# karenyang/GCN-VAE

Measured on AMD Instinct MI355X. Metric: edges/sec R-GCN forward+backward, FB15k-237 emb=200, higher is better.
Workload: dtype f32; 1 GPU; FB15k-237-shaped synthetic full graph (BASELINE configs[1]): 14541 entities, 474 directed relation types, E=544230 directed edges on this rank (544230 in the trained graph), 2-layer R-GCN-VAE bdd num_bases=100 emb_dim=200 dropout 0.2, 0 IAF blocks, DistMult decoder on T=220000 triplets per rank, step = fwd + loss(BCE+reg+KL+MMD) + bwd + clip + Adam; edges_per_gpu=544230, trained_graph_edges=544230, nodes=14541, triplets_per_gpu=220000, n_flows=0, gemm_precision=f32, launch=hipgraph, parallelism=single GPU, optimizer=replicated clip + Adam, k1_operands=f32

## Files before the change

gcn-vae_amd/csrc/common.h:

```cpp
#pragma once
#include <hip/hip_runtime.h>
#include <stdint.h>
#include <stdio.h>

#include "../../include/gcnvae.h"

namespace gv {

constexpr int WAVE = 64;

void set_error(const char* fmt, ...);

inline int launch_status(const char* what) {
    hipError_t e = hipGetLastError();
    if (e != hipSuccess) {
        set_error("%s: %s", what, hipGetErrorString(e));
        return (int)e;
    }
    return GV_OK;
}

#define GV_REQUIRE(cond, code, ...)   \
    do {                              \
        if (!(cond)) {                \
// ... 54 lines not shown
    v += dpp_f<DPP_ROW_HALF_MIRROR>(v);
    v += dpp_f<DPP_ROW_MIRROR>(v);
    return v;
}

__device__ __forceinline__ float wave_sum(float v) {
    v = row16_sum(v);
    return (rl_bcast_f(v, 0) + rl_bcast_f(v, 16)) + (rl_bcast_f(v, 32) + rl_bcast_f(v, 48));
}

__device__ __forceinline__ float wave_max(float v) {
    v = fmaxf(v, dpp_f<DPP_QUAD_1032>(v));
    v = fmaxf(v, dpp_f<DPP_QUAD_2301>(v));
    v = fmaxf(v, dpp_f<DPP_ROW_HALF_MIRROR>(v));
    v = fmaxf(v, dpp_f<DPP_ROW_MIRROR>(v));
    return fmaxf(fmaxf(rl_bcast_f(v, 0), rl_bcast_f(v, 16)), fmaxf(rl_bcast_f(v, 32), rl_bcast_f(v, 48)));
}

template <int N>
__device__ __forceinline__ void load_vec(const float* __restrict__ p, float (&d)[N]) {
    if constexpr (N % 4 == 0) {
#pragma unroll
        for (int i = 0; i < N / 4; ++i) {
            float4 t = reinterpret_cast<const float4*>(p)[i];
            d[4 * i] = t.x; d[4 * i + 1] = t.y; d[4 * i + 2] = t.z; d[4 * i + 3] = t.w;
        }
    } else if constexpr (N % 2 == 0) {
#pragma unroll
        for (int i = 0; i < N / 2; ++i) {
            float2 t = reinterpret_cast<const float2*>(p)[i];
            d[2 * i] = t.x; d[2 * i + 1] = t.y;
        }
    } else {
#pragma unroll
        for (int i = 0; i < N; ++i) d[i] = p[i];
    }
}

template <int N>
__device__ __forceinline__ void store_vec(float* __restrict__ p, const float (&s)[N]) {
    if constexpr (N % 4 == 0) {
#pragma unroll
        for (int i = 0; i < N / 4; ++i)
            reinterpret_cast<float4*>(p)[i] = make_float4(s[4 * i], s[4 * i + 1], s[4 * i + 2], s[4 * i + 3]);
    } else if constexpr (N % 2 == 0) {
#pragma unroll
        for (int i = 0; i < N / 2; ++i) reinterpret_cast<float2*>(p)[i] = make_float2(s[2 * i], s[2 * i + 1]);
    } else {
#pragma unroll
        for (int i = 0; i < N; ++i) p[i] = s[i];
    }
}

__device__ __forceinline__ float sum_slices_16x64(const float* __restrict__ part, int ncols, int nsl, int col, float (*sm)[16]) {
    const int cl = threadIdx.x & 15, grp = threadIdx.x >> 4;
    const int per = (nsl + 63) / 64;
    const int s0 = grp * per, s1 = min(nsl, s0 + per);
    float a0 = 0.f, a1 = 0.f, a2 = 0.f, a3 = 0.f;
    if (col < ncols) {
        int s = s0;
        for (; s + 4 <= s1; s += 4) {
            const float v0 = part[(size_t)s * ncols + col], v1 = part[(size_t)(s + 1) * ncols + col];
            const float v2 = part[(size_t)(s + 2) * ncols + col], v3 = part[(size_t)(s + 3) * ncols + col];
            a0 += v0; a1 += v1; a2 += v2; a3 += v3;
        }
        for (; s < s1; ++s) a0 += part[(size_t)s * ncols + col];
    }
    sm[grp][cl] = (a0 + a1) + (a2 + a3);
    __syncthreads();
    float tot = 0.f;
    if (grp == 0) {
#pragma unroll 8
        for (int g = 0; g < 64; ++g) tot += sm[g][cl];
    }
    return tot;
}

__global__ __launch_bounds__(256) inline void k_fill_u32(unsigned* __restrict__ p, unsigned v, long long n) {
    for (long long i = (long long)blockIdx.x * 256 + threadIdx.x; i < n; i += (long long)gridDim.x * 256) p[i] = v;
}
__global__ __launch_bounds__(256) inline void k_copy_u32(unsigned* __restrict__ d, const unsigned* __restrict__ s, long long n) {
    for (long long i = (long long)blockIdx.x * 256 + threadIdx.x; i < n; i += (long long)gridDim.x * 256) d[i] = s[i];
}
inline hipError_t fill_words(void* p, unsigned word, size_t n_bytes, hipStream_t st) {
    const long long n = (long long)(n_bytes / 4);
    if (n == 0) return hipSuccess;
    const unsigned blocks = (unsigned)((n + 255) / 256 > 4096 ? 4096 : (n + 255) / 256);
    hipLaunchKernelGGL(k_fill_u32, dim3(blocks), dim3(256), 0, st, (unsigned*)p, word, n);
    return hipGetLastError();
}
inline hipError_t copy_words(void* d, const void* s, size_t n_bytes, hipStream_t st) {
    const long long n = (long long)(n_bytes / 4);
    if (n == 0) return hipSuccess;
    const unsigned blocks = (unsigned)((n + 255) / 256 > 4096 ? 4096 : (n + 255) / 256);
    hipLaunchKernelGGL(k_copy_u32, dim3(blocks), dim3(256), 0, st, (unsigned*)d, (const unsigned*)s, n);
    return hipGetLastError();
}

__device__ __forceinline__ float apply_act(float v, int act) { return act == GV_ACT_RELU ? fmaxf(v, 0.f) : v; }

__device__ __forceinline__ uint4 philox4x32_10(uint32_t k0, uint32_t k1, uint32_t c0, uint32_t c1, uint32_t c2, uint32_t c3) {
#pragma unroll
    for (int r = 0; r < 10; ++r) {
        const uint32_t hi0 = __umulhi(0xD2511F53u, c0), lo0 = 0xD2511F53u * c0;
        const uint32_t hi1 = __umulhi(0xCD9E8D57u, c2), lo1 = 0xCD9E8D57u * c2;
        const uint32_t n0 = hi1 ^ c1 ^ k0, n1 = lo1, n2 = hi0 ^ c3 ^ k1, n3 = lo0;
        c0 = n0; c1 = n1; c2 = n2; c3 = n3;
        k0 += 0x9E3779B9u; k1 += 0xBB67AE85u;
    }
    return make_uint4(c0, c1, c2, c3);
}


}
```

gcn-vae_amd/csrc/k_gemm.hip:

```cpp
#include <limits.h>
#include <stdlib.h>
#include <string.h>

#include <algorithm>
#include <type_traits>

#include "common.h"
#include "k_riders.h"
#include "k_mc.h"
#include "k_query_args.h"
#include "k_topk.h"

namespace gv {


typedef float f32x16 __attribute__((ext_vector_type(16)));

struct GemmParams {
    const float* a;
    const float* b;
    float* c;
    const float* bias;
    const float* a_mask;
    float* ws;
// ... 218 lines not shown
        k0 = k1;
    }
#pragma unroll
    for (int u = 0; u < NT; ++u) {
        const int col = n0 + wn + 32 * u + l31;
        if (col >= p.n) continue;
        const float bv = (p.bias && p.split_k == 1) ? p.bias[col] : 0.f;
#pragma unroll
        for (int t = 0; t < MT; ++t) {
            if (p.tmask && MT * NT > 1) {
                const int ti = (m0 + wm + 32 * t) >> 6, tj = (n0 + wn + 32 * u) >> 6;
                const int bit = ti * p.tmask_ld + tj;
                if (ti * 64 < p.m && !((p.tmask[bit >> 6] >> (bit & 63)) & 1ull))
#pragma unroll
                    for (int i = 0; i < 16; ++i) acc[t][u][i] = 0.f;
            }
            float old[16];
            const bool acc_old = p.accumulate && p.split_k == 1;
#pragma unroll
            for (int r = 0; r < 16; ++r) {
                const int row = m0 + wm + t * 32 + (r & 3) + 8 * (r >> 2) + 4 * lhi;
                old[r] = 0.f;
                if (acc_old && row < p.m) old[r] = p.c[(size_t)row * p.ldc + col];
            }
            float val[16];
#pragma unroll
            for (int r = 0; r < 16; ++r) {
                float v = acc[t][u][r];
                if (p.split_k == 1) {
                    v = apply_act(v + bv, p.act);
                    v = acc_old ? old[r] + v : v;
                }
                val[r] = v;
            }
#pragma unroll
            for (int r = 0; r < 16; ++r) {
                const int row = m0 + wm + t * 32 + (r & 3) + 8 * (r >> 2) + 4 * lhi;
                if (row >= p.m) continue;
                if (p.split_k > 1) p.ws[((size_t)bz * p.m + row) * p.n + col] = val[r];
                else p.c[(size_t)row * p.ldc + col] = val[r];
            }
        }
    }
}

template <bool TA, bool TB, int MT, int NT, int BK>
__global__ __launch_bounds__(256) void k_gemm_f32(const GemmParams p) {
    gemm_f32_body<TA, TB, MT, NT, BK>(p, blockIdx.x, blockIdx.y, blockIdx.z, gridDim.x, gridDim.y);
}

template <bool TA, bool TB, int MT, int NT, int BK>
__global__ __launch_bounds__(256) __attribute__((amdgpu_waves_per_eu(MT == 2 ? 5 : 7))) void k_gemm_f32_riders(const GemmParams p, const RiderSet rs, const int ntn, const int ntm,
                                                         const int n_riders, const int riders_front) {
    const int tiles = ntn * ntm;
    int b = blockIdx.x;
    if (riders_front) {
        if (b < n_riders) { rider_body(rs, b, n_riders); return; }
        b -= n_riders;
    } else if (b >= tiles) {
        rider_body(rs, b - tiles, n_riders);
        return;
    }
    const int by = b / ntn;
    gemm_f32_body<TA, TB, MT, NT, BK>(p, b - by * ntn, by, 0, ntn, ntm);
}

constexpr int SC_BM = 64, SC_BN = 64, SC_BK = 16, SC_LDA = SC_BM + 1, SC_LDB = SC_BN + 1;

__device__ __forceinline__ f32x16 score_tile(const GemmParams& p, int m0, int n0, float (&ra)[SC_BM * SC_BK / 256],
                                             float (&rb)[SC_BN * SC_BK / 256], float* As, float* Bs) {
    const int lane = threadIdx.x & 63, wid = threadIdx.x >> 6;
    const int wm = (wid >> 1) * 32, wn = (wid & 1) * 32;
    const int l31 = lane & 31, lhi = lane >> 5;
    f32x16 acc;
#pragma unroll
    for (int i = 0; i < 16; ++i) acc[i] = 0.f;
    for (int k0 = 0; k0 < p.k; k0 += SC_BK) {
        stage_a<false, SC_BM, SC_BK>(As, ra);
        stage_b<true, SC_BN, SC_BK>(Bs, rb);
        __syncthreads();
        if (k0 + SC_BK < p.k) {
            load_a<false, SC_BM, SC_BK>(p, m0, k0 + SC_BK, p.k, ra);
            load_b<true, SC_BN, SC_BK>(p, n0, k0 + SC_BK, p.k, rb);
        }
#pragma unroll
        for (int kk = 0; kk < SC_BK; kk += 2)
            acc = __builtin_amdgcn_mfma_f32_32x32x2f32(As[(kk + lhi) * SC_LDA + wm + l31], Bs[(kk + lhi) * SC_LDB + wn + l31],
                                                       acc, 0, 0, 0);
        __syncthreads();
    }
    return acc;
}

template <class LoadA>
__device__ __forceinline__ f32x16 score_tile_with(const GemmParams& p, LoadA load_a_chunk, int n0, float (&ra)[SC_BM * SC_BK / 256],
                                                  float (&rb)[SC_BN * SC_BK / 256], float* As, float* Bs) {
    const int lane = threadIdx.x & 63, wid = threadIdx.x >> 6;
    const int wm = (wid >> 1) * 32, wn = (wid & 1) * 32;
    const int l31 = lane & 31, lhi = lane >> 5;
    f32x16 acc;
#pragma unroll
    for (int i = 0; i < 16; ++i) acc[i] = 0.f;
    for (int k0 = 0; k0 < p.k; k0 += SC_BK) {
        stage_a<false, SC_BM, SC_BK>(As, ra);
        stage_b<true, SC_BN, SC_BK>(Bs, rb);
        __syncthreads();
        if (k0 + SC_BK < p.k) {
            load_a_chunk(k0 + SC_BK, ra);
            load_b<true, SC_BN, SC_BK>(p, n0, k0 + SC_BK, p.k, rb);
        }
#pragma unroll
        for (int kk = 0; kk < SC_BK; kk += 2)
            acc = __builtin_amdgcn_mfma_f32_32x32x2f32(As[(kk + lhi) * SC_LDA + wm + l31], Bs[(kk + lhi) * SC_LDB + wn + l31],
// ... 843 lines not shown
    }
}

constexpr int COLSUM_SLICES = 64;

__global__ __launch_bounds__(256) void k_colsum_part(const float* x, const float* msk, int64_t m, int n, int ld, float* part) {
    __shared__ float sm[4][64];
    const int lane = threadIdx.x & 63, w = threadIdx.x >> 6;
    const int c = blockIdx.x * 64 + lane;
    const int64_t per = (m + gridDim.y - 1) / gridDim.y;
    const int64_t r0 = blockIdx.y * per, r1 = min(m, r0 + per);
    float a0 = 0.f, a1 = 0.f, a2 = 0.f, a3 = 0.f;
    if (c < n) {
        int64_t r = r0 + w;
        if (msk) {
            for (; r + 12 < r1; r += 16) {
                const float v0 = x[r * ld + c], v1 = x[(r + 4) * ld + c], v2 = x[(r + 8) * ld + c], v3 = x[(r + 12) * ld + c];
                const float m0 = msk[r * ld + c], m1 = msk[(r + 4) * ld + c], m2 = msk[(r + 8) * ld + c], m3 = msk[(r + 12) * ld + c];
                a0 += m0 > 0.f ? v0 : 0.f; a1 += m1 > 0.f ? v1 : 0.f; a2 += m2 > 0.f ? v2 : 0.f; a3 += m3 > 0.f ? v3 : 0.f;
            }
            for (; r < r1; r += 4) a0 += msk[r * ld + c] > 0.f ? x[r * ld + c] : 0.f;
        } else {
            for (; r + 12 < r1; r += 16) {
                const float v0 = x[r * ld + c], v1 = x[(r + 4) * ld + c], v2 = x[(r + 8) * ld + c], v3 = x[(r + 12) * ld + c];
                a0 += v0; a1 += v1; a2 += v2; a3 += v3;
            }
            for (; r < r1; r += 4) a0 += x[r * ld + c];
        }
    }
    sm[w][lane] = (a0 + a1) + (a2 + a3);
    __syncthreads();
    if (w == 0 && c < n) part[(size_t)blockIdx.y * n + c] = (sm[0][lane] + sm[1][lane]) + (sm[2][lane] + sm[3][lane]);
}

__global__ __launch_bounds__(256) void k_colsum_final(const float* part, int n, int nsl, float* out, int accumulate) {
    const int c = blockIdx.x * blockDim.x + threadIdx.x;
    if (c >= n) return;
    float a0 = 0.f, a1 = 0.f, a2 = 0.f, a3 = 0.f;
    int s = 0;
    for (; s + 4 <= nsl; s += 4) {
        const float v0 = part[(size_t)s * n + c], v1 = part[(size_t)(s + 1) * n + c];
        const float v2 = part[(size_t)(s + 2) * n + c], v3 = part[(size_t)(s + 3) * n + c];
        a0 += v0; a1 += v1; a2 += v2; a3 += v3;
    }
    for (; s < nsl; ++s) a0 += part[(size_t)s * n + c];
    const float acc = (a0 + a1) + (a2 + a3);
    out[c] = accumulate ? out[c] + acc : acc;
}

__global__ __launch_bounds__(1024) void k_colsum_final_wide(const float* part, int n, int nsl, float* out, int accumulate) {
    __shared__ float sm[64][16];
    const int c = blockIdx.x * 16 + (threadIdx.x & 15);
    const float acc = sum_slices_16x64(part, n, nsl, c, sm);
    if ((threadIdx.x >> 4) == 0 && c < n) out[c] = accumulate ? out[c] + acc : acc;
}

}

using namespace gv;

static int k_chunk_for(int k, int split_k) {
    int per = (k + split_k - 1) / split_k;
    return ((per + 31) / 32) * 32;
}

extern "C" int64_t gv_gemm_workspace_bytes(int m, int n, int k, int split_k) {
    (void)k;
    return split_k > 1 ? (int64_t)split_k * m * n * (int64_t)sizeof(float) : 0;
}

static int gemm_any(bool bf16, int trans_a, int trans_b, int m, int n, int k, const float* a, int lda, const float* b,
                    int ldb, float* c, int ldc, const float* bias, int act, int accumulate, int split_k,
                    const float* a_relu_mask, void* workspace, int64_t workspace_bytes, void* stream, const int32_t* rows_dev = nullptr,
                    const uint64_t* kmask = nullptr, const uint64_t* tmask = nullptr, int tiles_wanted = 0) {
    GV_REQUIRE(m >= 0 && n >= 0 && k >= 0, GV_ERR_SHAPE, "gv_gemm_f32: negative size");
    if (m == 0 || n == 0) return GV_OK;
    GV_REQUIRE(c && (k == 0 || (a && b)), GV_ERR_NULL, "gv_gemm_f32: NULL matrix");
    GV_REQUIRE(lda >= (trans_a ? m : k) && ldb >= (trans_b ? k : n) && ldc >= n, GV_ERR_SHAPE,
               "gv_gemm_f32: leading dimension too small (lda=%d ldb=%d ldc=%d)", lda, ldb, ldc);
    GV_REQUIRE(act == GV_ACT_NONE || act == GV_ACT_RELU, GV_ERR_SHAPE, "gv_gemm_f32: unknown act %d", act);
    if (split_k < 1) split_k = 1;
    if (k == 0) split_k = 1;
    GemmParams p;
    p.a = a; p.b = b; p.c = c; p.bias = bias; p.a_mask = a_relu_mask; p.ws = (float*)workspace;
    p.m = m; p.n = n; p.k = k; p.lda = lda; p.ldb = ldb; p.ldc = ldc;
    p.act = act; p.accumulate = accumulate;
    p.k_chunk = k_chunk_for(k > 0 ? k : 1, split_k);
    split_k = k > 0 ? (k + p.k_chunk - 1) / p.k_chunk : 1;
    p.split_k = split_k;
    p.vec_a = aligned16(a) && (lda % 4 == 0) && (!a_relu_mask || aligned16(a_relu_mask));
    p.vec_b = aligned16(b) && (ldb % 4 == 0);
    p.rows_dev = bf16 ? nullptr : rows_dev;
    GV_REQUIRE(!kmask || (!bf16 && split_k == 1 && k <= 64 * 16), GV_ERR_SHAPE,
               "gv_gemm_f32_sparse: k-chunk words cover fp32 products of k <= 1024 without split-K (k=%d split_k=%d)", k, split_k);
    GV_REQUIRE(!tmask || !bf16, GV_ERR_SHAPE, "gv_gemm_f32_sparse: fp32 only");
    p.kmask = (const unsigned long long*)kmask;
    p.tmask = (const unsigned long long*)tmask;
    p.tmask_ld = (n + 63) / 64;
    GV_REQUIRE(tiles_wanted >= 0 && tiles_wanted <= ((m + 63) / 64) * ((n + 63) / 64), GV_ERR_SHAPE, "gv_gemm_f32_sparse: c_tiles_wanted=%d", tiles_wanted);
    p.tmask_wanted = (tmask && tiles_wanted > 0 && split_k > 1) ? tiles_wanted : 0;
    if (split_k > 1) {
        GV_REQUIRE(workspace, GV_ERR_NULL, "gv_gemm_f32: split_k needs a workspace");
        GV_REQUIRE(workspace_bytes >= gv_gemm_workspace_bytes(m, n, k, split_k), GV_ERR_WORKSPACE,
                   "gv_gemm_f32: workspace %lld < %lld bytes", (long long)workspace_bytes,
                   (long long)gv_gemm_workspace_bytes(m, n, k, split_k));
    }
    hipStream_t st = (hipStream_t)stream;
// ... 15 lines not shown
    }
    static const int mt_env = getenv("GV_GEMM_MT") ? atoi(getenv("GV_GEMM_MT")) : 0;
    static const int nt_env = getenv("GV_GEMM_NT") ? atoi(getenv("GV_GEMM_NT")) : 0;
    static const int bk_env = getenv("GV_GEMM_BK") ? atoi(getenv("GV_GEMM_BK")) : 0;
    const int nt = (nt_env == 2 && !kmask && !(tmask && tiles_wanted > 0 && split_k > 1)) ? 2 : 1;
    const int bn = 64 * nt;
    const long blocks128 = (long)((n + bn - 1) / bn) * ((m + 127) / 128) * split_k;
    const int mt = p.tmask_wanted ? 1 : (mt_env ? mt_env : (blocks128 >= 1024 ? 2 : 1));
    static const int sparse_bk = getenv("GV_GEMM_SPARSE_BK") ? atoi(getenv("GV_GEMM_SPARSE_BK")) : 16;
    const int bk = kmask ? (sparse_bk == 32 ? 32 : 16) : (bk_env ? (bk_env == 16 ? 16 : 32) : (trans_a ? 32 : 16));
    dim3 grid((n + bn - 1) / bn, (m + 64 * mt - 1) / (64 * mt), split_k), block(256);
    if (p.tmask_wanted) { grid.x = p.tmask_wanted; grid.y = 1; }
#define GV_GEMM_CFG(TA_, TB_, MT_, NT_, BK_) \
    if (mt == MT_ && nt == NT_ && bk == BK_) hipLaunchKernelGGL((k_gemm_f32<TA_, TB_, MT_, NT_, BK_>), grid, block, 0, st, p);
#define GV_GEMM_LAUNCH(TA_, TB_)                                                                       \
    do {                                                                                               \
        GV_GEMM_CFG(TA_, TB_, 1, 1, 16) GV_GEMM_CFG(TA_, TB_, 1, 1, 32) GV_GEMM_CFG(TA_, TB_, 1, 2, 16) \
        GV_GEMM_CFG(TA_, TB_, 1, 2, 32) GV_GEMM_CFG(TA_, TB_, 2, 1, 16) GV_GEMM_CFG(TA_, TB_, 2, 1, 32) \
        GV_GEMM_CFG(TA_, TB_, 2, 2, 16) GV_GEMM_CFG(TA_, TB_, 2, 2, 32)                                 \
    } while (0)
    if (!trans_a && !trans_b) GV_GEMM_LAUNCH(false, false);
    else if (!trans_a && trans_b) GV_GEMM_LAUNCH(false, true);
    else if (trans_a && !trans_b) GV_GEMM_LAUNCH(true, false);
    else GV_GEMM_LAUNCH(true, true);
#undef GV_GEMM_LAUNCH
#undef GV_GEMM_CFG
    int rc = launch_status("gv_gemm_f32");
    if (rc != GV_OK) return rc;
    if (split_k > 1) {
        const size_t total = (size_t)m * n;
        const int blocks = (int)min((size_t)2048, (total + 255) / 256);
        hipLaunchKernelGGL(k_gemm_splitk_reduce, dim3(blocks), dim3(256), 0, st, p);
        return launch_status("gv_gemm_f32(split-k reduce)");
    }
    return GV_OK;
}

extern "C" int gv_gemm_f32(int trans_a, int trans_b, int m, int n, int k, const float* a, int lda, const float* b,
                           int ldb, float* c, int ldc, const float* bias, int act, int accumulate, int split_k,
                           const float* a_relu_mask, void* workspace, int64_t workspace_bytes, void* stream) {
    return gemm_any(false, trans_a, trans_b, m, n, k, a, lda, b, ldb, c, ldc, bias, act, accumulate, split_k, a_relu_mask,
                    workspace, workspace_bytes, stream);
}

namespace {
struct Extent { const char* lo; const char* hi; };
inline Extent extent_of(const void* p, int64_t bytes) {
    return p && bytes > 0 ? Extent{(const char*)p, (const char*)p + bytes} : Extent{nullptr, nullptr};
}
inline bool overlaps(const Extent& a, const Extent& b) { return a.lo && b.lo && a.lo < b.hi && b.lo < a.hi; }
inline int64_t matrix_bytes(int rows, int cols, int ld) { return rows > 0 && cols > 0 ? ((int64_t)(rows - 1) * ld + cols) * 4 : 0; }
}

extern "C" int gv_gemm_f32_riders(int trans_a, int trans_b, int m, int n, int k, const float* a, int lda, const float* b, int ldb,
                                  float* c, int ldc, const float* bias, int act, int accumulate, int split_k,
                                  const float* a_relu_mask, void* workspace, int64_t workspace_bytes, const gv_riders* riders,
                                  void* stream) {
    const bool any = riders && (riders->rng_jobs > 0 || riders->pack_weight || riders->mix_z_pre);
    if (!any)
        return gemm_any(false, trans_a, trans_b, m, n, k, a, lda, b, ldb, c, ldc, bias, act, accumulate, split_k, a_relu_mask,
                        workspace, workspace_bytes, stream);
    GV_REQUIRE(split_k <= 1, GV_ERR_SHAPE, "gv_gemm_f32_riders: riders do not ride on a split-K product (split_k=%d)", split_k);
    GV_REQUIRE(!trans_a && !trans_b, GV_ERR_SHAPE, "gv_gemm_f32_riders: riders ride on A @ B only (the forward self-loop product)");
    GV_REQUIRE(m > 0 && n > 0 && k >= 0, GV_ERR_SHAPE, "gv_gemm_f32_riders: m=%d n=%d k=%d", m, n, k);
    GV_REQUIRE(c && (k == 0 || (a && b)), GV_ERR_NULL, "gv_gemm_f32_riders: NULL matrix");
    GV_REQUIRE(lda >= k && ldb >= n && ldc >= n, GV_ERR_SHAPE, "gv_gemm_f32_riders: leading dimension too small (lda=%d ldb=%d ldc=%d)",
               lda, ldb, ldc);
    GV_REQUIRE(act == GV_ACT_NONE || act == GV_ACT_RELU, GV_ERR_SHAPE, "gv_gemm_f32_riders: unknown act %d", act);
    GemmParams p;
    p.a = a; p.b = b; p.c = c; p.bias = bias; p.a_mask = a_relu_mask; p.ws = nullptr;
    p.m = m; p.n = n; p.k = k; p.lda = lda; p.ldb = ldb; p.ldc = ldc;
    p.act = act; p.accumulate = accumulate;
    p.k_chunk = k_chunk_for(k > 0 ? k : 1, 1);
    p.split_k = 1;
    p.vec_a = aligned16(a) && (lda % 4 == 0) && (!a_relu_mask || aligned16(a_relu_mask));
    p.vec_b = aligned16(b) && (ldb % 4 == 0);
    p.rows_dev = nullptr; p.kmask = nullptr; p.tmask = nullptr; p.tmask_ld = (n + 63) / 64; p.tmask_wanted = 0;
    const int ntn = (n + 63) / 64;
    const int mt = (long)ntn * ((m + 127) / 128) >= 1024 ? 2 : 1;
    const int ntm = (m + 64 * mt - 1) / (64 * mt);
    GV_REQUIRE((int64_t)ntn * ntm < (1ll << 30), GV_ERR_SHAPE, "gv_gemm_f32_riders: %d x %d tiles", ntn, ntm);

    const Extent ea = extent_of(a, matrix_bytes(m, k, lda)), eb = extent_of(b, matrix_bytes(k, n, ldb)),
                 ec = extent_of(c, matrix_bytes(m, n, ldc)), ebias = extent_of(bias, (int64_t)n * 4),
                 emask = extent_of(a_relu_mask, matrix_bytes(m, k, lda));
    auto written_ok = [&](const Extent& w) { return !(overlaps(w, ea) || overlaps(w, eb) || overlaps(w, ec) || overlaps(w, ebias) || overlaps(w, emask)); };
    auto read_ok = [&](const Extent& r) { return !overlaps(r, ec); };

    RiderSet rs;
    memset(&rs, 0, sizeof(rs));
    static const int per_thread = getenv("GV_RIDER_GROUPS") ? std::max(1, atoi(getenv("GV_RIDER_GROUPS"))) : 8;
    static const int front = getenv("GV_RIDERS_FRONT") ? atoi(getenv("GV_RIDERS_FRONT")) : 1;
    int nblk = 0;
    rs.first[0] = 0;
    if (riders->rng_jobs > 0) {
        GV_REQUIRE(riders->rng_state, GV_ERR_NULL, "gv_gemm_f32_riders: NULL rng_state");
        GV_REQUIRE(riders->rng_jobs <= GV_RNG_MAX_JOBS, GV_ERR_SHAPE, "gv_gemm_f32_riders: rng_jobs=%d (1..%d)", riders->rng_jobs,
                   GV_RNG_MAX_JOBS);
        GV_REQUIRE(read_ok(extent_of(riders->rng_state, 16)), GV_ERR_SHAPE, "gv_gemm_f32_riders: rng_state overlaps C");
        rs.rng_state = riders->rng_state;
        long long g = 0;
        for (int j = 0; j < GV_RNG_MAX_JOBS; ++j) {
            rs.rng.group0[j] = g;
            if (j >= riders->rng_jobs) continue;
            void* ptr = riders->rng_ptr[j];
            const int64_t cnt = riders->rng_count[j];
            const int kind = riders->rng_kind[j];
            const float dp = riders->rng_drop_p[j];
            GV_REQUIRE(ptr && cnt > 0 && cnt < (1ll << 34), GV_ERR_SHAPE, "gv_gemm_f32_riders: rng job %d: bad buffer/count", j);
            GV_REQUIRE(kind == GV_RNG_KEEP_MASK || kind == GV_RNG_NORMAL, GV_ERR_SHAPE, "gv_gemm_f32_riders: rng job %d: kind %d", j, kind);
            GV_REQUIRE((reinterpret_cast<uintptr_t>(ptr) & (kind == GV_RNG_NORMAL ? 15u : 3u)) == 0, GV_ERR_ALIGN,
                       "gv_gemm_f32_riders: rng job %d: buffer alignment", j);
            GV_REQUIRE(kind == GV_RNG_NORMAL || (dp >= 0.f && dp < 1.f), GV_ERR_SHAPE, "gv_gemm_f32_riders: rng job %d: p=%f", j, dp);
            GV_REQUIRE(written_ok(extent_of(ptr, cnt * (kind == GV_RNG_NORMAL ? 4 : 1))), GV_ERR_SHAPE,
                       "gv_gemm_f32_riders: rng job %d writes into an operand of the product", j);
            rs.rng.ptr[j] = ptr; rs.rng.n[j] = cnt; rs.rng.kind[j] = kind; rs.rng.stream[j] = riders->rng_stream[j];
            const double th = (double)dp * 4294967296.0;
            rs.rng.thresh[j] = th >= 4294967295.0 ? 4294967295u : (uint32_t)th;
            g += (cnt + 3) / 4;
        }
        rs.rng.group0[GV_RNG_MAX_JOBS] = g;
        for (int j = riders->rng_jobs; j <= GV_RNG_MAX_JOBS; ++j) rs.rng.group0[j] = g;
        rs.rng.n_jobs = riders->rng_jobs;
        const long long want = (g + 256ll * per_thread - 1) / (256ll * per_thread);
        nblk += (int)std::min<long long>(std::max<long long>(want, 1), 1 << 16);
    }
    rs.first[1] = nblk;
    if (riders->pack_weight) {
        const int nb = riders->pack_bases, bi = riders->pack_blk_in, bo = riders->pack_blk_out, r = riders->pack_rels;
        GV_REQUIRE(riders->packed, GV_ERR_NULL, "gv_gemm_f32_riders: NULL packed");
        GV_REQUIRE(r > 0 && nb > 0 && bi > 0 && bo > 0 && (int64_t)r * nb * bi * bo < (1ll << 31), GV_ERR_SHAPE,
                   "gv_gemm_f32_riders: pack shape R=%d nb=%d %dx%d", r, nb, bi, bo);
        GV_REQUIRE(!riders->packed_pair || !riders->pack_transpose, GV_ERR_SHAPE,
                   "gv_gemm_f32_riders: the pair is (blk_in, blk_out, transpose 0) + its backward-x layout");
        PackJob& pj = rs.pack;
        GV_REQUIRE(pack_job_plan(nb, bi, bo, riders->pack_transpose != 0, &pj.bpl, &pj.adj) &&
                       (!riders->packed_pair || pack_job_plan(nb, bo, bi, true, &pj.bpl2, &pj.adj2)),
                   GV_ERR_SHAPE, "gv_gemm_f32_riders: no lane-packed kernel for num_bases=%d blocks %dx%d trans=%d", nb, bi, bo,
                   riders->pack_transpose);
        GV_REQUIRE(aligned16(riders->pack_weight) && aligned16(riders->packed) && aligned16(riders->packed_pair), GV_ERR_ALIGN,
                   "gv_gemm_f32_riders: pack buffers need 16-B alignment");
        const int64_t wbytes = (int64_t)r * nb * bi * bo * 4;
        const Extent ew = extent_of(riders->pack_weight, wbytes), e1 = extent_of(riders->packed, wbytes),
                     e2 = extent_of(riders->packed_pair, wbytes);
        GV_REQUIRE(read_ok(ew) && written_ok(e1) && written_ok(e2) && !overlaps(ew, e1) && !overlaps(ew, e2) && !overlaps(e1, e2),
                   GV_ERR_SHAPE, "gv_gemm_f32_riders: a pack buffer overlaps an operand of the product or another pack buffer");
        pj.w = riders->pack_weight; pj.packed = riders->packed; pj.packed2 = riders->packed_pair;
        pj.num_rels = r; pj.nb = nb; pj.pq = bi * bo;
        const int total = r * nb * bi * bo / 4;
        pj.blocks = std::min(2048, (total + 255) / 256);
        nblk += pj.blocks * (riders->packed_pair ? 2 : 1);
    }
    rs.first[2] = nblk;
    if (riders->mix_z_pre) {
        const int mk = riders->mix_k, mh = riders->mix_h;
        GV_REQUIRE(riders->mix, GV_ERR_NULL, "gv_gemm_f32_riders: NULL mix");
        GV_REQUIRE(mk > 0 && mh > 0 && (int64_t)mk * mh < (1ll << 28), GV_ERR_SHAPE, "gv_gemm_f32_riders: mix k=%d h=%d", mk, mh);
        const Extent ez = extent_of(riders->mix_z_pre, (int64_t)2 * mk * mh * 4), em = extent_of(riders->mix, (int64_t)3 * mk * mh * 4);
        GV_REQUIRE(read_ok(ez) && written_ok(em) && !overlaps(ez, em), GV_ERR_SHAPE,
                   "gv_gemm_f32_riders: a mix buffer overlaps an operand of the product or z_pre");
        rs.mix.z_pre = riders->mix_z_pre; rs.mix.mix = riders->mix; rs.mix.k = mk; rs.mix.h = mh;
        nblk += (mk * mh + 255) / 256;
    }
    rs.first[3] = nblk;
    const int n_riders = front ? (nblk + 7) / 8 * 8 : nblk;
    const dim3 grid((unsigned)(ntn * ntm + n_riders)), block(256);
    hipStream_t st = (hipStream_t)stream;
    if (mt == 2) hipLaunchKernelGGL((k_gemm_f32_riders<false, false, 2, 1, 16>), grid, block, 0, st, p, rs, ntn, ntm, n_riders, front ? 1 : 0);
    else hipLaunchKernelGGL((k_gemm_f32_riders<false, false, 1, 1, 16>), grid, block, 0, st, p, rs, ntn, ntm, n_riders, front ? 1 : 0);
    return launch_status("gv_gemm_f32_riders");
}

extern "C" int gv_gemm_f32_live_rows(int trans_a, int trans_b, int m, int n, int k, const float* a, int lda, const float* b,
                                     int ldb, float* c, int ldc, const float* bias, int act, int accumulate, int split_k,
                                     const float* a_relu_mask, void* workspace, int64_t workspace_bytes, const int32_t* rows_dev,
                                     void* stream) {
    return gemm_any(false, trans_a, trans_b, m, n, k, a, lda, b, ldb, c, ldc, bias, act, accumulate, split_k, a_relu_mask,
                    workspace, workspace_bytes, stream, rows_dev);
}

extern "C" int gv_gemm_f32_sparse(int trans_a, int trans_b, int m, int n, int k, const float* a, int lda, const float* b, int ldb,
                                  float* c, int ldc, const float* bias, int act, int accumulate, int split_k, const float* a_relu_mask,
                                  void* workspace, int64_t workspace_bytes, const int32_t* rows_dev, const uint64_t* b_k_chunks,
                                  const uint64_t* c_tiles, int c_tiles_wanted, void* stream) {
    return gemm_any(false, trans_a, trans_b, m, n, k, a, lda, b, ldb, c, ldc, bias, act, accumulate, split_k, a_relu_mask,
                    workspace, workspace_bytes, stream, rows_dev, b_k_chunks, c_tiles, c_tiles_wanted);
}

extern "C" int gv_gemm_bf16(int trans_a, int trans_b, int m, int n, int k, const float* a, int lda, const float* b,
                            int ldb, float* c, int ldc, const float* bias, int act, int accumulate, int split_k,
                            const float* a_relu_mask, void* workspace, int64_t workspace_bytes, void* stream) {
    return gemm_any(true, trans_a, trans_b, m, n, k, a, lda, b, ldb, c, ldc, bias, act, accumulate, split_k, a_relu_mask,
                    workspace, workspace_bytes, stream);
}

static GemmParams score_gemm_params(const float* q, int ld_q, const float* e, int ld_e, int m, int v, int h) {
    GemmParams p;
    p.a = q; p.b = e; p.c = nullptr; p.bias = nullptr; p.a_mask = nullptr; p.ws = nullptr;
    p.m = m; p.n = v; p.k = h; p.lda = ld_q; p.ldb = ld_e; p.ldc = v;
    p.act = GV_ACT_NONE; p.accumulate = 0; p.split_k = 1; p.k_chunk = h;
    p.vec_a = aligned16(q) && (ld_q % 4 == 0);
    p.vec_b = aligned16(e) && (ld_e % 4 == 0);
    p.rows_dev = nullptr; p.kmask = nullptr; p.tmask = nullptr; p.tmask_ld = 0; p.tmask_wanted = 0;
    return p;
}

static int mc_samples_args(const char* name, const float* q, int ld_q, int64_t q_stride, const float* e, int ld_e, int64_t e_stride,
                           int n_samples, int m, int v, int h, McSamples* mc) {
    GV_REQUIRE(n_samples >= 1, GV_ERR_SHAPE, "%s: n_samples=%d", name, n_samples);
    GV_REQUIRE(ld_q >= h && ld_e >= h, GV_ERR_SHAPE, "%s: leading dimension too small", name);
    GV_REQUIRE(n_samples == 1 || (q_stride >= (int64_t)(m > 0 ? m - 1 : 0) * ld_q + h && e_stride >= (int64_t)(v - 1) * ld_e + h),
               GV_ERR_SHAPE, "%s: sample stride shorter than the rows it spans (q_stride=%lld e_stride=%lld)", name,
               (long long)q_stride, (long long)e_stride);
    mc->q_stride = n_samples > 1 ? q_stride : 0;
    mc->e_stride = n_samples > 1 ? e_stride : 0;
    mc->n_samples = n_samples;
    mc->inv_s = 1.0f / (float)n_samples;
    return GV_OK;
}

static GemmParams mc_gemm_params(const float* q, int ld_q, const float* e, int ld_e, const McSamples& mc, int m, int v, int h) {
    GemmParams p = score_gemm_params(q, ld_q, e, ld_e, m, v, h);
    p.vec_a = p.vec_a && mc.q_stride % 4 == 0;
// ... 694 lines not shown
```

gcn-vae_amd/csrc/k_loss.hip:

```cpp
#include "common.h"
#include "k_riders.h"

namespace gv {

constexpr int RED_BLOCKS = 1024;

__device__ __forceinline__ float block_sum_256(float v, float* sm ) {
    v = wave_sum(v);
    const int lane = threadIdx.x & 63, w = threadIdx.x >> 6;
    __syncthreads();
    if (lane == 0) sm[w] = v;
    __syncthreads();
    return sm[0] + sm[1] + sm[2] + sm[3];
}

__global__ __launch_bounds__(256) void k_final_sum(const float* part, int n, float scale, float* out, int accumulate) {
    __shared__ float sm[4];
    float acc = 0.f;
    for (int i = threadIdx.x; i < n; i += 256) acc += part[i];
    const float tot = block_sum_256(acc, sm);
    if (threadIdx.x == 0) *out = accumulate ? *out + scale * tot : scale * tot;
}

constexpr int LOSS_COMBINE_XSQ_MAX = 65536;
// ... 801 lines not shown
        }
    }
}

__global__ __launch_bounds__(256) void k_kl_bwd_mix_part(const float* z, const float* mix, const float* resp,
                                                         float* part, int64_t n, int h, int k) {
    __shared__ float sm[2][4][64];
    const int j = blockIdx.x, slice = blockIdx.z, nsl = gridDim.z;
    const int lane = threadIdx.x & 63, w = threadIdx.x >> 6;
    const int c = blockIdx.y * 64 + lane;
    const int64_t per = (n + nsl - 1) / nsl;
    const int64_t r0 = slice * per, r1 = min(n, r0 + per);
    const int kh = k * h;
    float gmu0 = 0.f, gmu1 = 0.f, gv0 = 0.f, gv1 = 0.f;
    const bool ok = c < h;
    const float muj = ok ? mix[j * h + c] : 0.f, i2 = ok ? mix[kh + j * h + c] : 0.f;
    if (ok) {
        int64_t r = r0 + w;
        for (; r + 4 < r1; r += 8) {
            const float ra = resp[r * k + j], rb = resp[(r + 4) * k + j];
            const float da = z[r * h + c] - muj, db = z[(r + 4) * h + c] - muj;
            gmu0 += ra * da;
            gmu1 += rb * db;
            gv0 += ra * (da * da * 2.f * i2 * i2 - i2);
            gv1 += rb * (db * db * 2.f * i2 * i2 - i2);
        }
        for (; r < r1; r += 4) {
            const float ra = resp[r * k + j];
            const float da = z[r * h + c] - muj;
            gmu0 += ra * da;
            gv0 += ra * (da * da * 2.f * i2 * i2 - i2);
        }
    }
    sm[0][w][lane] = gmu0 + gmu1;
    sm[1][w][lane] = gv0 + gv1;
    __syncthreads();
    if (w == 0 && ok) {
        const float gmu = (sm[0][0][lane] + sm[0][1][lane]) + (sm[0][2][lane] + sm[0][3][lane]);
        const float gvv = (sm[1][0][lane] + sm[1][1][lane]) + (sm[1][2][lane] + sm[1][3][lane]);
        part[((size_t)slice * 2 * k + j) * h + c] = -gmu * 2.f * i2;
        part[((size_t)slice * 2 * k + k + j) * h + c] = -gvv;
    }
}

__global__ __launch_bounds__(1024) void k_kl_bwd_mix_final(const float* part, const float* z_pre, const float* gkl,
                                                           float gscale, float* g_zpre, int accumulate, int64_t n, int h,
                                                           int k, int nsl, const int* rows_dev, float* g_bias = nullptr,
                                                           int accumulate_bias = 0) {
    __shared__ float sm[64][16];
    const int kh = k * h, total = 2 * kh + (g_bias ? 2 * h : 0);
    const int i = blockIdx.x * 16 + (threadIdx.x & 15);
    float acc = sum_slices_16x64(part, total, nsl, i, sm);
    if ((threadIdx.x >> 4) != 0 || i >= total) return;
    if (i >= 2 * kh) {
        g_bias[i - 2 * kh] = accumulate_bias ? g_bias[i - 2 * kh] + acc : acc;
        return;
    }
    const float cg = gscale * (gkl ? *gkl : 1.f) / (float)(rows_dev ? (int64_t)*rows_dev : n);
    if (i >= kh) {
        const float raw = z_pre[i];
        acc *= raw > 20.f ? 1.f : 1.f / (1.f + expf(-raw));
    }
    g_zpre[i] = accumulate ? g_zpre[i] + cg * acc : cg * acc;
}

constexpr int MMD_WAVES = 16;

template <int CPL>
__device__ __forceinline__ void mmd_load_row(const float* p, int h, int lane, float (&v)[CPL]) {
#pragma unroll
    for (int i = 0; i < CPL; ++i) v[i] = (lane + 64 * i < h) ? p[lane + 64 * i] : 0.f;
}

template <int CPL>
__device__ __forceinline__ float mmd_d2(const float (&a)[CPL], const float (&b)[CPL]) {
    float d2 = 0.f;
#pragma unroll
    for (int i = 0; i < CPL; ++i) { const float d = a[i] - b[i]; d2 = fmaf(d, d, d2); }
    return d2;
}

template <int CPL>
__global__ __launch_bounds__(64 * MMD_WAVES) void k_mmd_fwd(const float* x, const float* y, const int64_t* yidx, int sx, int sy,
                                                             int h, float* part) {
    __shared__ float sm[MMD_WAVES];
    const int lane = threadIdx.x & 63, w = threadIdx.x >> 6;
    const bool is_x = (int)blockIdx.x < sx;
    auto row_of = [&](bool from_y, int j) -> const float* {
        return from_y ? y + (size_t)(yidx ? yidx[j] : j) * h : x + (size_t)j * h;
    };
    float av[CPL];
    mmd_load_row<CPL>(row_of(!is_x, is_x ? (int)blockIdx.x : (int)blockIdx.x - sx), h, lane, av);
    const float inv = 1.f / ((float)h * (float)h);
    float tot = 0.f;
    for (int pass = 0; pass < (is_x ? 2 : 1); ++pass) {
        const bool b_is_y = pass == 0 ? !is_x : true;
        const int nb = pass == 0 ? (is_x ? sx : sy) : sy;
        const float wt = pass == 0 ? 1.f / ((float)nb * (float)nb) : -2.f / ((float)sx * (float)sy);
        for (int j = w; j < nb; j += 4 * MMD_WAVES) {
            float b0[CPL], b1[CPL], b2[CPL], b3[CPL];
            const int j1 = j + MMD_WAVES, j2 = j + 2 * MMD_WAVES, j3 = j + 3 * MMD_WAVES;
            mmd_load_row<CPL>(row_of(b_is_y, j), h, lane, b0);
            mmd_load_row<CPL>(row_of(b_is_y, min(j1, nb - 1)), h, lane, b1);
            mmd_load_row<CPL>(row_of(b_is_y, min(j2, nb - 1)), h, lane, b2);
            mmd_load_row<CPL>(row_of(b_is_y, min(j3, nb - 1)), h, lane, b3);
            const float d0 = wave_sum(mmd_d2<CPL>(av, b0)), d1 = wave_sum(mmd_d2<CPL>(av, b1));
            const float d2 = wave_sum(mmd_d2<CPL>(av, b2)), d3 = wave_sum(mmd_d2<CPL>(av, b3));
            tot += wt * expf(-d0 * inv);
            if (j1 < nb) tot += wt * expf(-d1 * inv);
            if (j2 < nb) tot += wt * expf(-d2 * inv);
            if (j3 < nb) tot += wt * expf(-d3 * inv);
        }
    }
    if (lane == 0) sm[w] = tot;
    __syncthreads();
    if (threadIdx.x == 0) {
// ... 283 lines not shown
    const float* eps;
    float* gz_pre;
    int accumulate, k;
};

__global__ __launch_bounds__(256) void k_mmd_grad_finish(const MmdFinishParams a) {
    const float gg = a.gscale * (a.gmmd ? *a.gmmd : 1.f);
    const int h = a.h;
    if ((int)blockIdx.x < a.sy) {
        const int row = blockIdx.x;
        const float* src = a.gy_u + (size_t)row * h;
        float* o = a.gy + (size_t)(a.yidx ? a.yidx[row] : row) * h;
        for (int c = threadIdx.x; c < h; c += 256) {
            const float v = gg * src[c];
            if (a.yidx) atomicAdd(o + c, v);
            else o[c] = v;
        }
        return;
    }
    const int total = a.k * h;
    const int i = ((int)blockIdx.x - a.sy) * 256 + (int)threadIdx.x;
    if (i >= total) return;
    const int j = i / h, c = i - j * h;
    const float raw = a.z_pre[(size_t)(a.k + j) * h + c];
    const float v = softplus_t(raw) + 1e-8f;
    float gm = 0.f, gs = 0.f;
    constexpr int RU = 8;
    const int last = a.sx - a.k + j;
    for (int r0 = j; r0 < a.sx; r0 += RU * a.k) {
        float gu[RU], ev[RU];
#pragma unroll
        for (int u = 0; u < RU; ++u) {
            const size_t at = (size_t)min(r0 + u * a.k, last) * h + c;
            gu[u] = a.gx_u[at];
            ev[u] = a.eps[at];
        }
#pragma unroll
        for (int u = 0; u < RU; ++u) {
            const int r = r0 + u * a.k;
            if (r < a.sx) {
                const float g = gg * gu[u];
                if (a.g_pri) a.g_pri[(size_t)r * h + c] = g;
                gm += g;
                gs += g * ev[u];
            }
        }
    }
    const float gr = gs * 0.5f / sqrtf(v) * (raw > 20.f ? 1.f : 1.f / (1.f + expf(-raw)));
    a.gz_pre[i] = a.accumulate ? a.gz_pre[i] + gm : gm;
    a.gz_pre[total + i] = a.accumulate ? a.gz_pre[total + i] + gr : gr;
}

__global__ __launch_bounds__(256) void k_prior_sample_fwd(const float* z_pre, const float* eps, float* out, int s, int k, int h) {
    const int total = s * h;
    for (int i = blockIdx.x * 256 + threadIdx.x; i < total; i += gridDim.x * 256) {
        const int r = i / h, c = i - r * h, j = r % k;
        const float v = softplus_t(z_pre[(size_t)(k + j) * h + c]) + 1e-8f;
        out[i] = z_pre[(size_t)j * h + c] + eps[i] * sqrtf(v);
    }
}

__global__ __launch_bounds__(256) void k_prior_sample_bwd(const float* z_pre, const float* eps, const float* g, float* gz_pre,
                                                          int accumulate, int s, int k, int h) {
    const int total = k * h;
    for (int i = blockIdx.x * 256 + threadIdx.x; i < total; i += gridDim.x * 256) {
        const int j = i / h, c = i - j * h;
        const float raw = z_pre[(size_t)(k + j) * h + c];
        const float v = softplus_t(raw) + 1e-8f;
        float gm = 0.f, gs = 0.f;
        for (int r = j; r < s; r += k) {
            gm += g[(size_t)r * h + c];
            gs += g[(size_t)r * h + c] * eps[(size_t)r * h + c];
        }
        const float gr = gs * 0.5f / sqrtf(v) * (raw > 20.f ? 1.f : 1.f / (1.f + expf(-raw)));
        gz_pre[i] = accumulate ? gz_pre[i] + gm : gm;
        gz_pre[total + i] = accumulate ? gz_pre[total + i] + gr : gr;
    }
}

struct DmFusedParams {
    const int4* items;
    int n_items;
    const int* rel_s;
    const int* rel_o;
    const int* rel_tid;
    const float* e;
    int ld_e;
    const float* w;
    int ld_w;
    const float* labels;
    const float* bias;
    const int* pos3;
    float* score;
    float* delta;
    float* u;
    float* partial;
    float* part;
    int h;
};

constexpr int DM_PART = RED_BLOCKS;

__device__ __forceinline__ float dm_perm_f(int src_lane, float v) {
    return __int_as_float(__builtin_amdgcn_ds_bpermute(src_lane << 2, __float_as_int(v)));
}
__device__ __forceinline__ float dm_delta(float x, float y) { return 1.f / (1.f + expf(-x)) - y; }

constexpr int DM_U = 2;

__device__ __forceinline__ void dm_fused_body(const DmFusedParams& a, const int bid, const int nblk, float* sm, int4 (*tb)[64],
                                              float (*sums)[256]) {
    constexpr int U = DM_U;
// ... 418 lines not shown

extern "C" int gv_reparam_kl_fwd_mix(const float* h2, const float* eps, const float* z_pre, float* z, float* v, float* m_out,
                                     float* resp, float* workspace, int mix_ready, int64_t n, int h, int k, void* stream) {
    GV_REQUIRE(h2 && eps && z_pre && z && v && resp && workspace, GV_ERR_NULL, "gv_reparam_kl_fwd: NULL pointer");
    GV_REQUIRE(n > 0 && h > 0 && h <= 1024 && k > 0 && k <= KL_KMAX, GV_ERR_SHAPE, "gv_reparam_kl_fwd: n=%lld h=%d k=%d", (long long)n,
               h, k);
    const size_t lds = (size_t)2 * k * h * sizeof(float);
    GV_REQUIRE(lds <= 64 * 1024, GV_ERR_SHAPE, "gv_reparam_kl_fwd: mixture table %zu B exceeds the 64 KiB LDS budget", lds);
    float* mix = workspace;
    float* part = workspace + 3 * (size_t)k * h;
    float* zsq_part = workspace + kl_zsq_offset(h, k);
    if (!mix_ready) hipLaunchKernelGGL(k_kl_mix, dim3((k * h + 255) / 256), dim3(256), 0, GV_ST, z_pre, k, h, mix);
    const int nb = kl_blocks(n);
    const float* none = nullptr;
    const int* no_rows = nullptr;
#define GV_RKL_FWD(CPL_)                                                                                                       \
    hipLaunchKernelGGL(k_kl_fwd<CPL_>, dim3(nb), dim3(256), lds, GV_ST, none, none, h, none, (const float*)mix, none, resp, part, n, h, \
                       k, no_rows, h2, eps, z, v, m_out, zsq_part)
    if (kl_fwd_v4(nb, lds, GV_ST, none, none, h, none, mix, none, resp, part, n, h, k, no_rows, h2, eps, z, v, m_out, zsq_part)) {}
    else if (h <= 64) GV_RKL_FWD(1);
    else if (h <= 128) GV_RKL_FWD(2);
    else if (h <= 256) GV_RKL_FWD(4);
    else if (h <= 512) GV_RKL_FWD(8);
    else GV_RKL_FWD(16);
#undef GV_RKL_FWD
    return launch_status("gv_reparam_kl_fwd");
}

extern "C" int gv_reparam_kl_fwd(const float* h2, const float* eps, const float* z_pre, float* z, float* v, float* m_out,
                                 float* resp, float* workspace, int64_t n, int h, int k, void* stream) {
    return gv_reparam_kl_fwd_mix(h2, eps, z_pre, z, v, m_out, resp, workspace, 0, n, h, k, stream);
}

extern "C" int gv_reparam_kl_bwd(const float* z, const float* h2, const float* v, const float* eps, const float* z_pre,
                                 const float* resp, const float* gkl, float gscale, float z_extra, const float* gz_up,
                                 float* gh2, float* g_zpre, int accumulate_zpre, float* workspace, int64_t n, int h, int k,
                                 void* stream) {
    GV_REQUIRE(z && h2 && v && eps && z_pre && resp && gh2 && g_zpre && workspace, GV_ERR_NULL, "gv_reparam_kl_bwd: NULL pointer");
    GV_REQUIRE(n > 0 && h > 0 && k > 0 && k <= KL_FUSED_KT, GV_ERR_SHAPE, "gv_reparam_kl_bwd: n=%lld h=%d k=%d (k <= %d)", (long long)n,
               h, k, KL_FUSED_KT);
    float* mix = workspace;
    float* part = workspace + 3 * (size_t)k * h + RED_BLOCKS;
    float* none = nullptr;
    const int* no_rows = nullptr;
    if (!kl_bwd_cols4(GV_ST, z, h2, 2 * h, v, mix, resp, gkl, gscale, z_extra, none, none, none, part, n, h, k, no_rows, h2, eps, gz_up,
                      gh2))
        hipLaunchKernelGGL(k_kl_bwd_fused<KL_FUSED_KT>, dim3((h + 63) / 64, KL_SLICES), dim3(256), 0, GV_ST, z, h2, 2 * h, v,
                           (const float*)mix, resp, gkl, gscale, z_extra, none, none, none, part, n, h, k, no_rows, h2, eps, gz_up, gh2);
    hipLaunchKernelGGL(k_kl_bwd_mix_final, dim3((2 * k * h + 15) / 16), dim3(1024), 0, GV_ST, (const float*)part, z_pre, gkl, gscale,
                       g_zpre, accumulate_zpre, n, h, k, KL_SLICES, no_rows);
    return launch_status("gv_reparam_kl_bwd");
}

extern "C" int gv_reparam_kl_bwd_fold(const float* z, const float* h2, const float* v, const float* eps, const float* z_pre,
                                      const float* resp, const float* gkl, float gscale, float z_extra, const float* gz_up,
                                      float* gh2, float* g_zpre, int accumulate_zpre, const uint8_t* keep, float keep_scale,
                                      float* g_bias, int accumulate_bias, float* workspace, int64_t n, int h, int k,
                                      void* stream) {
    GV_REQUIRE(z && h2 && v && eps && z_pre && resp && gh2 && g_zpre && workspace, GV_ERR_NULL,
               "gv_reparam_kl_bwd_fold: NULL pointer");
    GV_REQUIRE(n > 0 && h > 0 && k > 0 && k <= KL_FUSED_KT, GV_ERR_SHAPE, "gv_reparam_kl_bwd_fold: n=%lld h=%d k=%d (k <= %d)",
               (long long)n, h, k, KL_FUSED_KT);
    float* mix = workspace;
    float* part = workspace + 3 * (size_t)k * h + RED_BLOCKS;
    float* none = nullptr;
    const int* no_rows = nullptr;
    const int cols = (2 * k + (g_bias ? 2 : 0)) * h;
    GV_REQUIRE(kl_bwd_cols4(GV_ST, z, h2, 2 * h, v, mix, resp, gkl, gscale, z_extra, none, none, none, part, n, h, k, no_rows, h2, eps,
                            gz_up, gh2, keep, keep_scale, g_bias != nullptr),
               GV_ERR_SHAPE, "gv_reparam_kl_bwd_fold: h=%d k=%d or an unaligned operand: only the float4-column backward "
               "(h %% 4 == 0, k <= 10, 16-B rows) folds the epilogue gradient", h, k);
    hipLaunchKernelGGL(k_kl_bwd_mix_final, dim3((cols + 15) / 16), dim3(1024), 0, GV_ST, (const float*)part, z_pre, gkl, gscale,
                       g_zpre, accumulate_zpre, n, h, k, KL_SLICES, no_rows, g_bias, accumulate_bias);
    return launch_status("gv_reparam_kl_bwd_fold");
}

__global__ void k_lincomb(const float* a0, float c0, const float* a1, float c1, const float* a2, float c2, const float* a3,
                          float c3, float* out) {
    if (threadIdx.x == 0 && blockIdx.x == 0) {
        float v = 0.f;
        if (a0) v += c0 * *a0;
        if (a1) v += c1 * *a1;
        if (a2) v += c2 * *a2;
        if (a3) v += c3 * *a3;
        *out = v;
    }
}

extern "C" int gv_lincomb4(const float* a0, float c0, const float* a1, float c1, const float* a2, float c2,
                           const float* a3, float c3, float* out, void* stream) {
    GV_REQUIRE(out, GV_ERR_NULL, "gv_lincomb4: NULL output");
    hipLaunchKernelGGL(k_lincomb, dim3(1), dim3(64), 0, GV_ST, a0, c0, a1, c1, a2, c2, a3, c3, out);
    return launch_status("gv_lincomb4");
}

extern "C" int gv_mmd_fwd(const float* x, const float* y, const int64_t* y_index, int sx, int sy, int h, float* mmd,
                          float* workspace, void* stream) {
    GV_REQUIRE(x && y && workspace, GV_ERR_NULL, "gv_mmd_fwd: NULL pointer");
    GV_REQUIRE(sx > 0 && sy > 0 && h > 0 && h <= 1024 && sx + sy <= RED_BLOCKS, GV_ERR_SHAPE,
               "gv_mmd_fwd: sx=%d sy=%d h=%d (need h <= 1024, sx+sy <= %d)", sx, sy, h, RED_BLOCKS);
    static const int v2 = getenv("GV_MMD_ROWS16") ? atoi(getenv("GV_MMD_ROWS16")) : 1;
    const bool al = h % 4 == 0 && aligned16(x) && aligned16(y);
    if (v2 && al && h <= 256) hipLaunchKernelGGL(k_mmd_fwd_g<4>, dim3(sx + sy), dim3(64 * MMD_WAVES), 0, GV_ST, x, y, y_index, sx, sy, h, workspace);
    else if (v2 && al && h <= 512) hipLaunchKernelGGL(k_mmd_fwd_g<8>, dim3(sx + sy), dim3(64 * MMD_WAVES), 0, GV_ST, x, y, y_index, sx, sy, h, workspace);
    else if (h <= 256) hipLaunchKernelGGL(k_mmd_fwd<4>, dim3(sx + sy), dim3(64 * MMD_WAVES), 0, GV_ST, x, y, y_index, sx, sy, h, workspace);
    else hipLaunchKernelGGL(k_mmd_fwd<16>, dim3(sx + sy), dim3(64 * MMD_WAVES), 0, GV_ST, x, y, y_index, sx, sy, h, workspace);
    if (mmd) hipLaunchKernelGGL(k_final_sum, dim3(1), dim3(256), 0, GV_ST, workspace, sx + sy, 1.f, mmd, 0);
    return launch_status("gv_mmd_fwd");
}

extern "C" int gv_loss_combine(const float* ws_pred, int64_t t, const float* ws_reg, int64_t n_embed, int64_t n_wrel,
                               const float* ws_kl, int64_t n_nodes, int h, int k, const float* ws_mmd, int sx, int sy,
                               float reg_w, float kl_w, float mmd_w, float* scal, float* loss, const int32_t* rows_dev,
                               void* stream) {
    GV_REQUIRE(ws_pred && loss, GV_ERR_NULL, "gv_loss_combine: NULL pointer");
    GV_REQUIRE(t > 0, GV_ERR_SHAPE, "gv_loss_combine: t=%lld", (long long)t);
    const int n0 = red_blocks(t, 16);
    const int n1 = ws_reg ? sq2_blocks(n_embed, 768) + sq2_blocks(n_wrel, 255) : 0;
    const int n2 = ws_kl ? kl_blocks(n_nodes) : 0;
    const int n3 = ws_mmd ? sx + sy : 0;
    const float* kl_part = ws_kl ? ws_kl + 3 * (size_t)k * h : nullptr;
    hipLaunchKernelGGL(k_loss_combine, dim3(1), dim3(256), 0, GV_ST, ws_pred, n0, 1.f / (float)t, ws_reg, n1, 1.f, kl_part,
                       n2, ws_kl ? 1.f / (float)n_nodes : 0.f, ws_mmd, n3, 1.f, reg_w, kl_w, mmd_w, scal, loss, rows_dev,
                       (float)n_nodes);
    return launch_status("gv_loss_combine");
}

// ... 139 lines not shown
```

gcn-vae_amd/csrc/k_riders.h:

```cpp
#pragma once

#include "common.h"

namespace gv {

struct RngJobs {
    void* ptr[GV_RNG_MAX_JOBS];
    long long n[GV_RNG_MAX_JOBS];
    long long group0[GV_RNG_MAX_JOBS + 1];
    int kind[GV_RNG_MAX_JOBS];
    uint32_t thresh[GV_RNG_MAX_JOBS];
    uint32_t stream[GV_RNG_MAX_JOBS];
    int n_jobs;
};

__device__ __forceinline__ void rng_fill_body(const uint64_t* state, const RngJobs& jobs, long long bid, long long nblk) {
    const uint64_t seed = state[0], tick = state[1];
    const uint32_t k0 = (uint32_t)seed, k1 = (uint32_t)(seed >> 32), t0 = (uint32_t)tick, t1 = (uint32_t)(tick >> 32);
    const long long total = jobs.group0[jobs.n_jobs];
    for (long long gg = bid * 256 + threadIdx.x; gg < total; gg += nblk * 256) {
        int j = 0;
#pragma unroll
        for (int q = 1; q < GV_RNG_MAX_JOBS; ++q)
            if (q < jobs.n_jobs && gg >= jobs.group0[q]) j = q;
// ... 11 lines not shown
                if (left > 1) o[1] = b.y;
                if (left > 2) o[2] = b.z;
            }
        } else {
            const float s = 2.3283064365386963e-10f;
            const float r0 = sqrtf(-1.3862943611198906f * __log2f(((float)x.x + 1.f) * s));
            const float r1 = sqrtf(-1.3862943611198906f * __log2f(((float)x.z + 1.f) * s));
            const float a0 = (float)x.y * s, a1 = (float)x.w * s;
            const float s0 = __builtin_amdgcn_sinf(a0), c0 = __builtin_amdgcn_cosf(a0);
            const float s1 = __builtin_amdgcn_sinf(a1), c1 = __builtin_amdgcn_cosf(a1);
            const float4 nrm = make_float4(r0 * c0, r0 * s0, r1 * c1, r1 * s1);
            float* o = (float*)jobs.ptr[j] + e0;
            if (left >= 4) {
                *reinterpret_cast<float4*>(o) = nrm;
            } else {
                o[0] = nrm.x;
                if (left > 1) o[1] = nrm.y;
                if (left > 2) o[2] = nrm.z;
            }
        }
    }
}

__device__ __forceinline__ void pack_weight_body(const float* w, float* packed, int num_rels, int nb, int pq, int bpl, int adj,
                                                 int bid, int nblk) {
    const int L = nb / bpl, nq = bpl * pq / 4, quads = L * nq;
    const int total = num_rels * quads;
    for (int i = bid * 256 + threadIdx.x; i < total; i += nblk * 256) {
        const int r = i / quads, rem = i - r * quads;
        const int l = rem % L, jq = rem / L;
        const int f = 4 * jq, sb = f / pq, within = f - sb * pq;
        const int block = adj ? l * bpl + sb : l + sb * L;
        reinterpret_cast<float4*>(packed)[i] =
            *reinterpret_cast<const float4*>(w + (size_t)r * nb * pq + (size_t)block * pq + within);
    }
}

bool pack_job_plan(int num_bases, int blk_in, int blk_out, bool transpose_w, int* bpl, int* adj);

constexpr float LOG_SQRT_2PI = 0.9189385332046727f;

__device__ __forceinline__ float softplus_t(float x) { return x > 20.f ? x : log1pf(expf(x)); }

__device__ __forceinline__ void kl_mix_body(const float* z_pre, int k, int h, float* mix, int bid, int nblk) {
    const int total = k * h;
    for (int i = bid * 256 + threadIdx.x; i < total; i += nblk * 256) {
        const float v = softplus_t(z_pre[total + i]) + 1e-8f;
        mix[i] = z_pre[i];
        mix[total + i] = 1.f / (2.f * v);
        mix[2 * total + i] = logf(sqrtf(v)) + LOG_SQRT_2PI;
    }
}

struct PackJob {
    const float* w;
    float* packed;
    float* packed2;
    int num_rels, nb, pq, bpl, adj, bpl2, adj2;
    int blocks;
};

struct MixJob {
    const float* z_pre;
    float* mix;
    int k, h;
};

struct RiderSet {
    const uint64_t* rng_state;
    RngJobs rng;
    PackJob pack;
    MixJob mix;
    int first[4];
};

__device__ __forceinline__ void rider_body(const RiderSet& rs, int b, int n) {
    (void)n;
    if (b < rs.first[1]) {
        rng_fill_body(rs.rng_state, rs.rng, b, rs.first[1]);
    } else if (b < rs.first[2]) {
        const int i = b - rs.first[1], second = i >= rs.pack.blocks;
        const PackJob& pj = rs.pack;
        pack_weight_body(pj.w, second ? pj.packed2 : pj.packed, pj.num_rels, pj.nb, pj.pq, second ? pj.bpl2 : pj.bpl,
                         second ? pj.adj2 : pj.adj, second ? i - pj.blocks : i, pj.blocks);
    } else if (b < rs.first[3]) {
        kl_mix_body(rs.mix.z_pre, rs.mix.k, rs.mix.h, rs.mix.mix, b - rs.first[2], rs.first[3] - rs.first[2]);
    }
}

}
```

gcn-vae_amd/encoders.py:

```python
import random

import numpy as np
import torch
import torch.nn as nn
import torch.nn.functional as F

from . import ops, prob
from .flows import MADE, PermuteLayer
from .layers import RelGraphConv


class EmbeddingLayer(ops.StayOnDevice, nn.Module):
    def __init__(self, num_nodes, h_dim):
        super().__init__()
        self.embedding = nn.Embedding(num_nodes, h_dim)

    def forward(self, g, h, r, norm):
        h = ops.to_module_device(self.embedding.weight, h)
        return ops.embedding(self.embedding.weight, h.squeeze(), ops.device_rng(self.embedding.weight.device),
                             sole_consumer=True)


class DistLayer(ops.StayOnDevice, nn.Module):

# ... 19 lines not shown
            print(f"Mixture of {self.k} Gaussians.")
        self.flow_log_prob = None
        self.build_encoder()
        self.z_pre = nn.Parameter(torch.randn(1, 2 * self.k, self.h_dim) / np.sqrt(self.k * self.h_dim))
        self.pi = nn.Parameter(torch.ones(k) / k, requires_grad=False)
        self.n_flows = n_flows
        if self.n_flows > 0:
            if verbose:
                print(f"Sequence of {self.n_flows} Flow transforms.")
            self.build_iaf()
        self.eps_override = None
        self.mmd_eps_override = None
        self.mmd_index_override = None
        self.rng_stream_eps, self.rng_stream_prior = ops.new_rng_stream(), ops.new_rng_stream()
        self._prior_eps_next = None
        self.batch_mmd_prior_with_forward = False
        self.rows_dev = None
        self.fuse_kl_with_reparam = False
        self.grad_reducer = None
        self._z_pri_flowed = None
        self.row_part = None

    def build_iaf(self):
        blocks = []
        for _ in range(self.n_flows):
            blocks.append(MADE(self.h_dim, self.h_dim, self.n_flows))
            blocks.append(PermuteLayer(self.h_dim))
        self.nf = nn.Sequential(*blocks)

    def build_encoder(self):
        self.input_layer = EmbeddingLayer(self.num_nodes, self.h_dim)
        self.rconv_layer_1 = RelGraphConv(self.h_dim, self.h_dim, self.num_rels, "bdd", self.num_bases,
                                          activation=nn.ReLU(), self_loop=True, dropout=self.dropout)
        self.rconv_layer_2 = RelGraphConv(self.h_dim, self.h_dim * 2, self.num_rels, "bdd", self.num_bases,
                                          activation=None, self_loop=True, dropout=self.dropout)

    def sample_z(self, batch):
        m, v = prob.gaussian_parameters(self.z_pre.squeeze(0), dim=0)
        idx = torch.distributions.categorical.Categorical(self.pi).sample((batch,))
        x = prob.sample_gaussian(m[idx], v[idx])
        if self.n_flows > 0:
            for flow in self.nf[::-1]:
                x, _ = flow.inverse(x)
        return x

    def compute_kernel(self, x, y):
        dim = x.size(1)
        d2 = (x.unsqueeze(1) - y.unsqueeze(0)).pow(2).mean(2) / float(dim)
        return torch.exp(-d2)

    def get_kl(self, z):
        return ops.kl_to_mixture(z, self.z_mean, self.z_sigma, self.z_pre.squeeze(0), self.flow_log_prob)

    def _prior_draw(self, device, dtype):
        num_sample = 200
        rows = (num_sample // self.k) * self.k if num_sample // self.k > 1 else self.k
        if self.mmd_eps_override is not None:
            eps = self.mmd_eps_override
        elif self._prior_eps_next is not None:
            eps, self._prior_eps_next = self._prior_eps_next, None
        else:
            eps = torch.empty(rows, self.h_dim, device=device, dtype=dtype)
            ops.device_rng(device).fill([(eps, ops.RNG_NORMAL, 0.0, self.rng_stream_prior)])
        return ops.prior_sample(self.z_pre.squeeze(0), eps)

    def _prior_rows(self):
        num_sample = 200
        return (num_sample // self.k) * self.k if num_sample // self.k > 1 else self.k

    def _draw_noise(self, n, device, riders=None):
        jobs, eps = [], self.eps_override
        for layer in (self.rconv_layer_1, self.rconv_layer_2):
            if layer.wants_keep_mask():
                layer._keep_next = torch.empty(n, layer.out_feat, dtype=torch.uint8, device=device)
                jobs.append(layer.keep_job(layer._keep_next))
        if eps is None:
            eps = torch.empty(n, self.h_dim, dtype=torch.float32, device=device)
            jobs.append((eps, ops.RNG_NORMAL, 0.0, self.rng_stream_eps))
        if self.batch_mmd_prior_with_forward and self.training and self.mmd_eps_override is None:
            self._prior_eps_next = torch.empty(self._prior_rows(), self.h_dim, dtype=torch.float32, device=device)
            jobs.append((self._prior_eps_next, ops.RNG_NORMAL, 0.0, self.rng_stream_prior))
        if jobs and riders is not None:
            rng = ops.device_rng(device)
            rng.claim(jobs)
            riders.rng = (rng, jobs)
        elif jobs:
            ops.device_rng(device).fill(jobs)
        return eps

    def mmd_inputs(self, z):
        num_sample = 200
        if self._z_pri_flowed is not None:
            z_pri, self._z_pri_flowed = self._z_pri_flowed, None
        else:
            z_pri = self._prior_draw(z.device, z.dtype)
            if self.n_flows > 0:
                for flow in self.nf:
                    z_pri, _ = flow.forward(z_pri)
        if self.mmd_index_override is not None:
            pick = self.mmd_index_override
        elif self.row_part is not None and getattr(self.row_part, 'real_positions', None) is not None:
            real = self.row_part.real_positions
            pick = torch.as_tensor(real[random.sample(range(len(real)), num_sample)], device=z.device)
        else:
            pick = torch.tensor(random.sample(range(z.shape[0]), num_sample), device=z.device)
        return z_pri, pick

    def get_mmd(self, z):
        z_pri, pick = self.mmd_inputs(z)
        return ops.mmd(z_pri, ops.embedding(z, pick))

    def get_flow_log_prob(self):
        return self.flow_log_prob

    def _forward_rows(self, g, h, r, norm):
        from .distributed import AllGatherRows
        from .distributed import AllReduceSum
# ... 18 lines not shown
        self.z_own = z
        return AllGatherRows.apply(ops.pad_rows(z, part.slot_rows), part)

    def _apply_flows(self, z, want_mean=False):
        n = z.shape[0]
        ride_along = self.batch_mmd_prior_with_forward and self.training
        if ride_along:
            z = ops.cat_rows(z, self._prior_draw(z.device, z.dtype))
        log_dets, flows, i = [], list(self.nf), 0
        with ops.made.keep_row_blocks_forked(z.shape[0]):
            while i < len(flows):
                flow = flows[i]
                if isinstance(flow, MADE):
                    fold = i + 1 < len(flows) and type(flows[i + 1]) is PermuteLayer
                    z, log_det = flow.forward(z, reverse_out=fold)
                    log_dets.append(log_det)
                    i += 2 if fold else 1
                else:
                    ops.made.fork_sync()
                    z, log_det = flow.forward(z)
                    i += 1
        if ride_along:
            z, self._z_pri_flowed = ops.split_rows(z, n)
        if want_mean and 1 <= len(log_dets) <= 8:
            return z, ops.mean_rows_multi(log_dets, n=n, rows_dev=self.rows_dev)
        log_det_sum = None
        for log_det in log_dets:
            log_det_sum = log_det if log_det_sum is None else log_det_sum + log_det
        if ride_along:
            log_det_sum = ops.split_rows(log_det_sum, n)[0]
        return z, log_det_sum

    def forward(self, g, h, r, norm):
        h, r, norm = ops.to_module_device(self.z_pre, h, r, norm)
        self.node_id = h.squeeze()
        if self.row_part is not None:
            return self._forward_rows(g, h, r, norm)
        if self.n_flows > 0:
            ops.made_prepare([f.call_arguments() for f in self.nf if isinstance(f, MADE)])
        h = self.input_layer(g, h, r, norm)
        ride = ops.LIVE_ROWS is None
        box1, box2 = self._rider_boxes = (ops.RiderBox(), ops.RiderBox()) if ride else (None, None)
        eps = self._draw_noise(h.shape[0], h.device, box1)
        h = self.rconv_layer_1(g, h, r, norm, riders=box1)
        if box1 is not None and not box1.done:
            raise RuntimeError('KGVAE.forward: layer 1 dropped its RiderBox (the random draws were never launched)')
        if self.grad_reducer is not None:
            h = self.grad_reducer.milestone(h, next(self.rconv_layer_2.parameters()))
        fuse_kl = self.training and self.n_flows == 0 and self.fuse_kl_with_reparam
        kl_ws = None
        if box2 is not None and fuse_kl and ops.FUSE_REPARAM_KL:
            kl_ws = ops.KLWorkspace(self.z_pre.squeeze(0), h.shape[0])
            box2.mix = (kl_ws.z_pre, kl_ws.ws)
        h = self.rconv_layer_2(g, h, r, norm, sole_consumer=fuse_kl, riders=box2)
        if box2 is not None and not box2.done:
            raise RuntimeError('KGVAE.forward: layer 2 dropped its RiderBox (weight packing / KL mixture table never launched)')
        z, self.z_mean, self.z_sigma = ops.reparam(h, eps, self.z_pre.squeeze(0) if fuse_kl else None,
                                                   getattr(h, '_gv_epi_link', None) if fuse_kl else None, kl_ws)
        self._z_pri_flowed = None
        if self.n_flows > 0:
            z, self.flow_log_prob = self._apply_flows(z, want_mean=True)
            ops.made_prepare_finish()
            if self.flow_log_prob.dim() != 0:
                log_det_sum = self.flow_log_prob
                if self.rows_dev is None:
                    self.flow_log_prob = torch.mean(log_det_sum.view(-1, 1))
                else:
                    rows = self.rows_dev.reshape(()).to(log_det_sum.dtype)
                    live = torch.arange(log_det_sum.numel(), device=log_det_sum.device) < self.rows_dev.reshape(())
                    self.flow_log_prob = (log_det_sum.reshape(-1) * live).sum() / rows
        return z

    def posterior_samples(self, g, h, r, norm, n_samples, seed=None):
        n_samples = int(n_samples)
        if n_samples < 1:
            raise ValueError(f'posterior_samples: n_samples must be >= 1, got {n_samples}')
        if self.training:
            raise RuntimeError('posterior_samples needs eval mode (the layers\' dropout would differ between the samples\' one '
                               'shared pass and a forward): call .eval() first')
        if self.row_part is not None:
            raise NotImplementedError('posterior_samples under a destination-row partition (multi-GPU) is not supported')
        h, r, norm = ops.to_module_device(self.z_pre, h, r, norm)
        self.node_id = h.squeeze()
        dev = self.z_pre.device
        gen = torch.Generator(device=dev)
        if seed is None:
            gen.seed()
        else:
            gen.manual_seed(int(seed))
        with torch.no_grad():
            x = self.input_layer(g, h, r, norm)
            x = self.rconv_layer_1(g, x, r, norm)
            h2 = self.rconv_layer_2(g, x, r, norm)
            n = h2.shape[0]
            z = torch.empty(n_samples, n, self.h_dim, dtype=torch.float32, device=dev)
            flps = torch.empty(n_samples, dtype=torch.float32, device=dev) if self.n_flows > 0 else None
            self.flow_log_prob = None
            self._z_pri_flowed = None
            for s in range(n_samples):
                eps = torch.randn(n, self.h_dim, generator=gen, dtype=torch.float32, device=dev)
                zs, self.z_mean, self.z_sigma = ops.reparam(h2, eps)
                if self.n_flows > 0:
                    zs, flp = self._apply_flows(zs, want_mean=True)
                    if flp.dim() != 0:
                        flp = torch.mean(flp.view(-1, 1))
                    self.flow_log_prob = flp
                    flps[s] = flp
                z[s].copy_(zs)
        return z, flps


class BaseRGCN(ops.StayOnDevice, nn.Module):
# ... 50 lines not shown
```

gcn-vae_amd/lib.py:

```python
import ctypes
import os

import torch

_HERE = os.path.dirname(os.path.abspath(__file__))
LIB_PATH = os.path.join(_HERE, 'libgcnvae_hip.so')

_P, _I, _L, _F = ctypes.c_void_p, ctypes.c_int, ctypes.c_int64, ctypes.c_float

SIGNATURES = {
    'gv_version': (_I, []),
    'gv_last_error_string': (ctypes.c_char_p, []),
    'gv_index_caps': (None, [_L, _I, _I, _P, _P, _P]),
    'gv_index_workspace_bytes': (_L, [_L, _I]),
    'gv_build_csr': (_I, [_P, _L, _I, _I, _P, _P, _P, _I, _P, _I, _P, _L, _P]),
    'gv_build_csr_batch_workspace_bytes': (_L, [_P, _I]),
    'gv_build_csr_batch': (_I, [_P, _I, _P, _L, _P]),
    'gv_triplet_lists': (_I, [_P, _I, _L, _P, _P, _P, _P, _P, _P, _P, _P, _P]),
    'gv_widen2_i32': (_I, [_P, _P, _L, _P, _P, _L, _P]),
    'gv_graph_index_build': (_I, [_P, _P, _L, _I, _I, _I, _I, _P, _P, _P, _P, _I, _P, _I, _P, _P, _P, _P, _I, _P, _I, _P, _L, _P]),
    'gv_relation_index_build': (_I, [_P, _P, _P, _P, _P, _L, _I, _I, _P, _P, _P, _P, _P, _P, _P, _I, _P, _I, _P, _L, _P]),
    'gv_triplet_index_build': (_I, [_P, _L, _I, _I, _I, _I, _P, _P, _P, _P, _P, _I, _P, _I, _P, _P, _P, _P, _P, _I, _P, _I,
                                    _P, _L, _P]),
    'gv_perm_sample': (_I, [_L, _L, ctypes.c_uint64, ctypes.c_uint64, _P, _P, ctypes.c_uint32, _P, _P]),
    'gv_neighborhood_sample_workspace_bytes': (_L, [_I, _L]),
    'gv_neighborhood_sample': (_I, [_P, _P, _P, _P, _I, _L, _I, ctypes.c_uint64, ctypes.c_uint64, _P, ctypes.c_uint32, _P, _P, _L, _P]),
    'gv_relabel_workspace_bytes': (_L, [_I]),
    'gv_relabel_pairs': (_I, [_P, _P, _L, _I, _P, _I, _P, _P, _P, _P, _L, _P]),
    'gv_negative_sampling': (_I, [_P, _P, _P, _L, _I, _P, _P, _P, ctypes.c_uint64, ctypes.c_uint64, _P, ctypes.c_uint32, _P, _P, _P]),
    'gv_graph_from_triplets_workspace_bytes': (_L, [_L, _I, _I]),
    'gv_graph_from_triplets': (_I, [_P, _P, _P, _P, _L, _I, _I, _P, _P, _P, _P, _P, _L, _P]),
    'gv_segment_items_count': (_I, [_P, _I, _I, _P, _P, _P, _P]),
    'gv_segment_items_fill': (_I, [_P, _I, _I, _P, _P, _P, _P, _P, _P]),
    'gv_rgcn_bdd_aggregate': (_I, [_P, _I, _P, _I, _P, _P, _P, _P, _P, _I, _P, _I, _I, _I, _I, _I, _I,
                                   _P, _I, _I, _P, _F, _P, _I, _P, _P]),
    'gv_rgcn_bdd_phase_plan': (_I, [_I, _I, _I, _I, _I, _I, _I, _I, _I, _P]),
    'gv_rgcn_bdd_pack_weight_phase': (_I, [_P, _I, _I, _I, _I, _I, _P, _P]),
    'gv_rgcn_bdd_aggregate_phases': (_I, [_P, _P, _P, _P, _P, _I, _P, _I, _P, _I, _P, _I, _I, _I, _I, _I, _I, _I, _I, _I,
                                          _P, _I, _I, _P, _F, _P, _I, _P, _P]),
    'gv_rgcn_bdd_lds_plan': (_I, [_I, _I, _I, _I, _I, _P]),
    'gv_rgcn_bdd_pack_weight_lds': (_I, [_P, _I, _I, _I, _I, _I, _I, _P, _P]),
    'gv_rgcn_bdd_aggregate_lds': (_I, [_P, _I, _P, _P, _I, _P, _I, _P, _P, _P, _P, _P, _I, _P, _I, _I, _I, _I, _I, _P, _I, _I,
                                       _P, _F, _P, _I, _P, _I, _P]),
    'gv_rgcn_bdd_pack_supported': (_I, [_I, _I, _I, _I]),
    'gv_rgcn_bdd_pack_weight': (_I, [_P, _I, _I, _I, _I, _I, _P, _P]),
    'gv_rgcn_bdd_pack_weight_pair': (_I, [_P, _I, _I, _I, _I, _P, _P, _P]),
    'gv_rgcn_bdd_fixup': (_I, [_P, _I, _P, _I, _P, _I, _I, _P, _F, _P, _I, _P]),
    'gv_rgcn_bdd_grad_weight': (_I, [_P, _I, _P, _I, _P, _P, _P, _P, _P, _I, _P, _I, _I, _I, _I, _P, _P, _I, _P]),
    'gv_rgcn_epilogue_fwd': (_I, [_P, _P, _I, _P, _F, _P, _L, _I, _P]),
    'gv_rgcn_epilogue_bwd': (_I, [_P, _P, _I, _P, _F, _P, _L, _I, _P, _P]),
    'gv_colsum_finish': (_I, [_P, _I, _I, _P, _I, _P]),
    'gv_gemm_workspace_bytes': (_L, [_I, _I, _I, _I]),
    'gv_gemm_f32': (_I, [_I, _I, _I, _I, _I, _P, _I, _P, _I, _P, _I, _P, _I, _I, _I, _P, _P, _L, _P]),
    'gv_gemm_f32_riders': (_I, [_I, _I, _I, _I, _I, _P, _I, _P, _I, _P, _I, _P, _I, _I, _I, _P, _P, _L, _P, _P]),
    'gv_gemm_f32_live_rows': (_I, [_I, _I, _I, _I, _I, _P, _I, _P, _I, _P, _I, _P, _I, _I, _I, _P, _P, _L, _P, _P]),
    'gv_gemm_f32_sparse': (_I, [_I, _I, _I, _I, _I, _P, _I, _P, _I, _P, _I, _P, _I, _I, _I, _P, _P, _L, _P, _P, _P, _I, _P]),
    'gv_gemm_bf16': (_I, [_I, _I, _I, _I, _I, _P, _I, _P, _I, _P, _I, _P, _I, _I, _I, _P, _P, _L, _P]),
    'gv_gemm_bf16_nt_workspace_bytes': (_L, [_I, _I, _I]),
    'gv_gemm_bf16_gradw_fits': (_I, [_I, _I, _I, _I]),
    'gv_gemm_bf16_gradw_workspace_bytes': (_L, [_I, _I, _I]),
    'gv_gemm_bf16_gradw': (_I, [_P, _I, _P, _I, _I, _I, _I, _P, _I, _P, _I, _P, _L, _P]),
    'gv_gemm_bf16_gradw_tiles': (_I, [_P, _L, _P, _L, _I, _I, _I, _P, _I, _P, _I, _P, _L, _P]),
    'gv_gemm_bf16_nt': (_I, [_P, _I, _I, _P, _I, _I, _I, _I, _P, _I, _P, _I, _P, _I, _I, _P, _I, _P, _I, _I, _P, _L, _P]),
    'gv_cast_bf16': (_I, [_P, _I, _I, _I, _P, _I, _P, _I, _P]),
    'gv_rowsum_bf16_workspace_floats': (_L, [_I, _I]),
    'gv_iaf_update_fwd_bf16': (_I, [_P, _P, _I, _P, _P, _P, _P, _I, _P, _I, _L, _I, _P]),
    'gv_iaf_update_fwd_bf16_tiles': (_I, [_P, _P, _I, _P, _P, _P, _P, _I, _P, _L, _L, _I, _P]),
    'gv_iaf_update_bwd_bf16': (_I, [_P, _P, _I, _P, _P, _P, _P, _P, _I, _P, _I, _P, _L, _I, _P]),
    'gv_gather3_i32': (_I, [_P, _L, _P, _P, _P, _P, _P, _P, _P]),
    'gv_iaf_update_bwd_row0_workspace_floats': (_L, [_I]),
    'gv_iaf_update_bwd_row0': (_I, [_P, _P, _P, _P, _P, _P, _P, _P, _L, _I, _P]),
    'gv_iaf_update_bwd_bf16_ex': (_I, [_P, _P, _I, _P, _P, _P, _P, _P, _I, _P, _I, _P, _I, _L, _I, _P]),
    'gv_rowsum_bf16': (_I, [_P, _I, _I, _I, _P, _I, _P, _P]),
    'gv_rowsum_bf16_segments': (_I, [_P, _I, _I, _I, _I, _P, _P, _I, _P, _P]),
    'gv_made_pack_weight_elems': (_L, [_I, _I]),
    'gv_made_pack_weight': (_I, [_P, _I, _I, _I, _P, _P, _P]),
    'gv_made_pack_weight_multi': (_I, [_I, _P, _P, _P, _P, _P, _P, _P]),
    'gv_made_pack_weight_multi_iaf': (_I, [_I, _P, _P, _P, _P, _P, _P, _P]),
    'gv_made_pack_weight_iaf': (_I, [_P, _I, _I, _I, _P, _P]),
    'gv_made_chain_fits': (_I, [_I, _P, _P, _I]),
    'gv_made_chain': (_I, [_P, _I, _I, _I, _P, _P]),
    'gv_made_chain_iafb': (_I, [_P, _I, _I, _P, _P]),
    'gv_made_chain_fwd': (_I, [_P, _I, _I, _I, _P, _I, _P, _P]),
    'gv_made_chain_fwd_row0': (_I, [_P, _I, _I, _P, _I, _P, _P]),
    'gv_made_chain_debug_stamps': (_I, [_P]),
    'gv_made_pack_weight_f32_elems': (_L, [_I, _I]),
    'gv_made_pack_weight_f32_multi': (_I, [_I, _P, _P, _P, _P, _P, _P, _P]),
    'gv_made_chain_f32_fits': (_I, [_I, _P, _P]),
    'gv_made_chain_f32_plan': (_I, [_I, _P, _P, _P, _P, _P, _P, _P]),
    'gv_made_chain_f32': (_I, [_P, _I, _I, _I, _P, _P, _P, _P]),
    'gv_made_passes_f32': (_I, [_P, _I, _I, _I, _P, _P, _P, _P, _P]),
    'gv_made_gradw_f32_plan_words': (_L, [_I, _I]),
    'gv_made_gradw_f32_plan': (_I, [_P, _I, _I, _I, _P, _P]),
    'gv_made_gradw_f32_workspace_floats': (_L, [_I, _I, _L]),
    'gv_made_gradw_f32': (_I, [_P, _I, _P, _I, _I, _I, _L, _P, _P, _I, _P, _P, _P, _P, _I, _I, _P, _I, _P, _L, _P]),
    'gv_made_gradw_f32_multi_workspace_floats': (_L, [_I, _P]),
    'gv_made_gradw_f32_multi': (_I, [_I, _P, _P, _L, _P]),
    'gv_made_row_fwd': (_I, [_P, _I, _P, _P]),
    'gv_made_row_bwd': (_I, [_P, _I, _P, _P, _P]),
    'gv_rel_rows_gemm': (_I, [_P, _I, _P, _P, _I, _I, _I, _I, _P, _I, _P, _P]),
    'gv_rel_gradw_gemm': (_I, [_P, _I, _P, _P, _I, _P, _P, _P, _I, _I, _I, _P, _P]),
    'gv_rank_scores': (_I, [_P, _I, _P, _I, _P, _P, _P, _P, _I, _I, _I, _P]),
    'gv_rank_scores_filtered': (_I, [_P, _I, _P, _I, _P, _P, _P, _P, _P, _I, _P, _P, _P, _I, _I, _I, _P]),
    'gv_topk_scores_workspace_bytes': (_L, [_I, _I, _I]),
    'gv_topk_scores': (_I, [_P, _I, _P, _I, _P, _P, _P, _P, _I, _I, _P, _P, _P, _I, _I, _I, _P]),
    'gv_rank_scores_constrained': (_I, [_P, _I, _P, _I, _P, _P, _P, _P, _P, _I, _P, _I, _I, _P, _P, _P, _P, _P, _P, _I, _I, _I, _P]),
    'gv_topk_scores_constrained': (_I, [_P, _I, _P, _I, _P, _P, _P, _P, _I, _P, _I, _I, _P, _I, _P, _P, _P, _I, _I, _I, _P]),
# ... 173 lines not shown
```

gcn-vae_amd/ops.py:

```python
import contextlib
import ctypes as _ct
import itertools as _it
import os as _os
from dataclasses import dataclass
from typing import Optional

import numpy as np
import torch

from . import lib
from .lib import ptr

ACT_NONE, ACT_RELU = 0, 1

DIRECT_GRAD = {}
GRAD_FRESH = set()
DIRECT_EPOCH = [0]


def _stamp_direct(ctx):
    ctx._gv_direct_epoch = DIRECT_EPOCH[0]


def _verify_direct(ctx):
# ... 277 lines not shown
        out = torch.empty(n_seg, w_row, dtype=torch.float32, device=x.device)
        accumulate = False
    if coef is not None:
        coef = _chk(coef.reshape(-1), name='coef')
    partial = None
    if seg.n_fix > 0:
        partial = torch.empty(seg.n_slots, w_row, dtype=torch.float32, device=x.device)
    lib.call('gv_rgcn_bdd_grad_weight', ptr(seg.items), seg.n_items, ptr(seg.fix), seg.n_fix, ptr(src), ptr(dst),
             ptr(coef), ptr(coef_idx), ptr(x), ld_x, ptr(g), ld_g, num_bases, blk_in, blk_out, ptr(out), ptr(partial),
             1 if accumulate else 0, lib.stream(), tag=f'gradw_{blk_in}x{blk_out}_nb{num_bases}')
    return out


GEMM_PRECISION = 'f32'


def set_gemm_precision(precision):
    global GEMM_PRECISION
    if precision not in ('f32', 'bf16'):
        raise ValueError("precision must be 'f32' or 'bf16'")
    GEMM_PRECISION = precision


@contextlib.contextmanager
def gemm_precision(precision):
    old = GEMM_PRECISION
    set_gemm_precision(precision)
    try:
        yield
    finally:
        set_gemm_precision(old)


LIVE_ROWS = None


class live_rows:

    def __init__(self, rows_dev, cap):
        self.val = (rows_dev, int(cap)) if rows_dev is not None else None

    def __enter__(self):
        global LIVE_ROWS
        self.saved, LIVE_ROWS = LIVE_ROWS, self.val
        return self

    def __exit__(self, *exc):
        global LIVE_ROWS
        LIVE_ROWS = self.saved
        return False


GEMM_RIDERS = _os.environ.get('GV_GEMM_RIDERS', '1') == '1'
GEMM_RIDER_KINDS = set(_os.environ.get('GV_GEMM_RIDER_KINDS', 'rng,pack,mix').split(','))


class _Riders(_ct.Structure):
    _fields_ = [('rng_state', _ct.c_void_p), ('rng_ptr', _ct.c_void_p * 8), ('rng_count', _ct.c_int64 * 8),
                ('rng_kind', _ct.c_int32 * 8), ('rng_drop_p', _ct.c_float * 8), ('rng_stream', _ct.c_uint32 * 8),
                ('rng_jobs', _ct.c_int32), ('pack_rels', _ct.c_int32), ('pack_bases', _ct.c_int32), ('pack_blk_in', _ct.c_int32),
                ('pack_blk_out', _ct.c_int32), ('pack_transpose', _ct.c_int32), ('pack_weight', _ct.c_void_p),
                ('packed', _ct.c_void_p), ('packed_pair', _ct.c_void_p), ('mix_z_pre', _ct.c_void_p), ('mix', _ct.c_void_p),
                ('mix_k', _ct.c_int32), ('mix_h', _ct.c_int32)]


class RiderBox:
    __slots__ = ('rng', 'pack', 'mix', 'done', 'rode')

    def __init__(self):
        self.rng = self.pack = self.mix = None
        self.done = False
        self.rode = ()

    def empty(self):
        return self.rng is None and self.pack is None and self.mix is None

    def _launch_alone(self, kinds):
        if 'rng' in kinds and self.rng is not None:
            self.rng[0].launch(self.rng[1])
        if 'pack' in kinds and self.pack is not None:
            w, nb, bi, bo, trans, packed, pair = self.pack
            if pair is not None:
                lib.call('gv_rgcn_bdd_pack_weight_pair', ptr(w), w.shape[0], nb, bi, bo, ptr(packed), ptr(pair), lib.stream())
            else:
                lib.call('gv_rgcn_bdd_pack_weight', ptr(w), w.shape[0], nb, bi, bo, 1 if trans else 0, ptr(packed), lib.stream())
        if 'mix' in kinds and self.mix is not None:
            z_pre, ws = self.mix
            lib.call('gv_kl_mix', ptr(z_pre), z_pre.shape[0] // 2, z_pre.shape[1], ptr(ws), lib.stream())

    def flush(self):
        if self.done:
            raise RuntimeError('RiderBox: its jobs were already launched')
        self._launch_alone(('rng', 'pack', 'mix'))
        self.done = True

    def ride(self, gemm_args):
        if self.done:
            raise RuntimeError('RiderBox: its jobs were already launched')
        ride = {k for k in ('rng', 'pack', 'mix') if getattr(self, k) is not None and k in GEMM_RIDER_KINDS}
        if 'rng' in ride and len(self.rng[1]) > 8:
            ride.discard('rng')
        self._launch_alone({'rng', 'pack', 'mix'} - ride)
        d = _Riders()
        if 'rng' in ride:
            rng, jobs = self.rng
            d.rng_state, d.rng_jobs = rng.state.data_ptr(), len(jobs)
            for i, (t, kind, p, st) in enumerate(jobs):
                d.rng_ptr[i], d.rng_count[i], d.rng_kind[i], d.rng_drop_p[i], d.rng_stream[i] = t.data_ptr(), t.numel(), kind, float(p), st
        if 'pack' in ride:
            w, nb, bi, bo, trans, packed, pair = self.pack
            d.pack_weight, d.packed, d.packed_pair = w.data_ptr(), packed.data_ptr(), (pair.data_ptr() if pair is not None else None)
            d.pack_rels, d.pack_bases, d.pack_blk_in, d.pack_blk_out, d.pack_transpose = w.shape[0], nb, bi, bo, 1 if trans else 0
        if 'mix' in ride:
            z_pre, ws = self.mix
            d.mix_z_pre, d.mix, d.mix_k, d.mix_h = z_pre.data_ptr(), ws.data_ptr(), z_pre.shape[0] // 2, z_pre.shape[1]
        lib.call('gv_gemm_f32_riders', *gemm_args, _ct.addressof(d), lib.stream())
        self.rode = tuple(sorted(ride))
        self.done = True


def gemm(a, b, trans_a=False, trans_b=False, bias=None, act=ACT_NONE, out=None, accumulate=False, split_k=1,
         a_relu_mask=None, precision=None, b_k_chunks=None, c_tiles=None, riders=None):
    a, lda = _row_major(a, 'a')
    b, ldb = _row_major(b, 'b')
    m, k = (a.shape[1], a.shape[0]) if trans_a else a.shape
    kb, n = (b.shape[1], b.shape[0]) if trans_b else b.shape
    if k != kb:
        raise ValueError(f'gemm inner dimensions differ: {k} vs {kb}')
    if out is None:
        out = torch.empty(m, n, dtype=torch.float32, device=a.device)
        accumulate = False
    else:
        if not isinstance(out, torch.Tensor) or out.dtype != torch.float32 or out.dim() != 2:
            raise TypeError(f'out: expected a 2-D float32 tensor, got {getattr(out, "dtype", type(out).__name__)} '
                            f'{tuple(getattr(out, "shape", ()))}')
        if out.device != a.device or b.device != a.device:
            raise ValueError(f'out / b must be on the device of a ({a.device}), got {out.device} / {b.device}')
        if tuple(out.shape) != (m, n):
            raise ValueError(f'out: expected shape {(m, n)}, got {tuple(out.shape)}')
        if m * n and ((n > 1 and out.stride(1) != 1) or (m > 1 and out.stride(0) < n)):
            raise ValueError(f'out: needs unit inner stride and a leading dimension >= {n}, got strides {out.stride()}')
    if bias is not None:
        _chk(bias, name='bias')
        if bias.numel() != n or bias.device != a.device:
            raise ValueError(f'bias: expected {n} values on {a.device}, got {bias.numel()} on {bias.device}')
    ws, ws_bytes = None, 0
    if split_k > 1:
        ws_bytes = int(lib.load().gv_gemm_workspace_bytes(m, n, k, split_k))
        ws = torch.empty(ws_bytes // 4, dtype=torch.float32, device=a.device)
    if a_relu_mask is not None:
        a_relu_mask, ld_mask = _row_major(a_relu_mask, 'a_relu_mask')
        if tuple(a_relu_mask.shape) != tuple(a.shape) or ld_mask != lda:
            raise ValueError('a_relu_mask must have the shape and leading dimension of a')
    entry = 'gv_gemm_bf16' if (precision or GEMM_PRECISION) == 'bf16' else 'gv_gemm_f32'
    live = LIVE_ROWS
    if riders is not None:
        plain = (entry == 'gv_gemm_f32' and b_k_chunks is None and c_tiles is None and not trans_a and not trans_b and split_k <= 1
                 and m > 0 and n > 0 and not (live is not None and a.shape[0] == live[1] and a.device == live[0].device))
        if GEMM_RIDERS and plain and not riders.empty():
            riders.ride((0, 0, m, n, k, ptr(a), lda, ptr(b), ldb, ptr(out), out.stride(0) if m > 1 else n, ptr(bias), act,
                         1 if accumulate else 0, 1, ptr(a_relu_mask), None, 0))
            return out
        riders.flush()
    if (b_k_chunks is not None or c_tiles is not None) and entry == 'gv_gemm_f32':
        if b_k_chunks is not None and (b_k_chunks.dtype != torch.int64 or b_k_chunks.numel() < (n + 63) // 64 or k > 1024 or split_k != 1):
            raise ValueError('b_k_chunks: one int64 word per 64-column tile, k <= 1024, no split-K')
        if c_tiles is not None and (c_tiles.dtype != torch.int64 or c_tiles.numel() * 64 < ((m + 63) // 64) * ((n + 63) // 64)):
            raise ValueError('c_tiles: one bit per 64 x 64 tile of the result')
        rows = live[0] if (live is not None and a.shape[0] == live[1] and a.device == live[0].device) else None
        lib.call('gv_gemm_f32_sparse', 1 if trans_a else 0, 1 if trans_b else 0, m, n, k, ptr(a), lda, ptr(b), ldb, ptr(out),
                 out.stride(0) if m > 1 else n, ptr(bias), act, 1 if accumulate else 0, split_k, ptr(a_relu_mask), ptr(ws),
                 ws_bytes, ptr(rows), ptr(b_k_chunks), ptr(c_tiles), int(getattr(c_tiles, '_gv_wanted', 0)) if c_tiles is not None else 0,
                 lib.stream())
        return out
    if live is not None and entry == 'gv_gemm_f32' and a.shape[0] == live[1] and a.device == live[0].device:
        lib.call('gv_gemm_f32_live_rows', 1 if trans_a else 0, 1 if trans_b else 0, m, n, k, ptr(a), lda, ptr(b), ldb, ptr(out),
                 out.stride(0) if m > 1 else n, ptr(bias), act, 1 if accumulate else 0, split_k, ptr(a_relu_mask), ptr(ws),
                 ws_bytes, ptr(live[0]), lib.stream())
        return out
    lib.call(entry, 1 if trans_a else 0, 1 if trans_b else 0, m, n, k, ptr(a), lda, ptr(b), ldb, ptr(out),
             out.stride(0) if m > 1 else n, ptr(bias), act, 1 if accumulate else 0, split_k, ptr(a_relu_mask), ptr(ws),
             ws_bytes, lib.stream())
    return out


def block_words(mask, kind):
    import numpy as np
    m = (mask.detach().to('cpu').numpy() != 0)
    o, i = m.shape

    def pad(x, r, c):
        y = np.zeros((-(-x.shape[0] // r) * r, -(-x.shape[1] // c) * c), dtype=bool)
        y[:x.shape[0], :x.shape[1]] = x
        return y
    if kind in ('fwd', 'bwd'):
        mm = m if kind == 'fwd' else m.T
        if mm.shape[1] > 1024:
            return None
        y = pad(mm, 64, 16)
        blk = y.reshape(y.shape[0] // 64, 64, y.shape[1] // 16, 16).any(axis=(1, 3))
        words = np.zeros(blk.shape[0], dtype=np.uint64)
        for c in range(blk.shape[1]):
            words |= blk[:, c].astype(np.uint64) << np.uint64(c)
    elif kind == 'tiles':
        y = pad(m, 64, 64)
        blk = y.reshape(y.shape[0] // 64, 64, y.shape[1] // 64, 64).any(axis=(1, 3)).reshape(-1)
        words = np.zeros((blk.size + 63) // 64, dtype=np.uint64)
        for b in np.nonzero(blk)[0]:
            words[b >> 6] |= np.uint64(1) << np.uint64(b & 63)
    else:
        raise ValueError(kind)
    out = torch.from_numpy(words.view(np.int64).copy()).to(mask.device)
    if kind == 'tiles':
# ... 977 lines not shown

def relation_typed_plan(set_ptr, num_rels, rels, span=None):
    sizes = (set_ptr[1:] - set_ptr[:-1]).to(torch.int64)
    chosen = torch.zeros(num_rels, dtype=torch.bool, device=set_ptr.device)
    chosen[rels.to(set_ptr.device)] = True
    sizes = sizes * torch.cat([chosen, chosen])
    units = mine_typed_plan(torch.cat([sizes.new_zeros(1), torch.cumsum(sizes, 0)]), num_rels, span)
    slot_of = torch.full((num_rels,), -1, dtype=torch.int32, device=set_ptr.device)
    slot_of[rels.to(set_ptr.device)] = torch.arange(rels.numel(), dtype=torch.int32, device=set_ptr.device)
    units[:, 0] = slot_of[units[:, 0].long()]
    return units.contiguous()


def relation_topk_scores_typed(emb, w, k, set_ptr, set_ids, *, relations=None, bias=None, filt_lo=None, filt_hi=None, filt_ent=None,
                               exclude_self=True, max_results=MINE_MAX_RESULTS, span=None):
    return _relation_topk('gv_mine_scores_typed_by_relation', MINE_RELATION_TYPED_LEVELS, emb, w, k, relations,
                          (set_ptr, set_ids, span), bias, filt_lo, filt_hi, filt_ent, exclude_self, max_results)


def pick_split_k(m_out, n_out, k):
    tiles = ((m_out + 63) // 64) * ((n_out + 63) // 64)
    if tiles >= 256 or k < 2048:
        return 1
    if k >= 65536:
        return 64
    return max(1, min(64, 1024 // tiles, k // 256))


def colsum(x, out=None, accumulate=False, relu_mask=None):
    x, ld = _row_major(x, 'x')
    if relu_mask is not None:
        relu_mask, ldm = _row_major(relu_mask, 'relu_mask')
        if tuple(relu_mask.shape) != tuple(x.shape) or ldm != ld:
            raise ValueError('relu_mask must have the shape and leading dimension of x')
    m, n = x.shape
    if out is None:
        out = torch.empty(n, dtype=torch.float32, device=x.device)
        accumulate = False
    ws = torch.empty(64 * n, dtype=torch.float32, device=x.device)
    lib.call('gv_colsum', ptr(x), ptr(relu_mask), m, n, ld, ptr(out), ptr(ws), 1 if accumulate else 0, lib.stream())
    return out


def epilogue_fwd(agg, addend, act, keep, keep_scale):
    agg = _chk(agg, name='agg')
    out = torch.empty_like(agg)
    if addend is not None:
        addend = _chk(addend, name='addend')
    lib.call('gv_rgcn_epilogue_fwd', ptr(agg), ptr(addend), act, ptr(keep), float(keep_scale), ptr(out),
             agg.shape[0], agg.shape[1], lib.stream())
    return out


def epilogue_bwd(out, grad_out, act, keep, keep_scale, colsum_out=None, colsum_accumulate=False):
    grad_out = _chk(grad_out.contiguous(), name='grad_out')
    g = torch.empty_like(grad_out)
    m, n = grad_out.shape
    fused = colsum_out is not None and n % 4 == 0 and n <= 1024
    part = torch.empty(EPILOGUE_COLSUM_SLICES * n, dtype=torch.float32, device=g.device) if fused else None
    lib.call('gv_rgcn_epilogue_bwd', ptr(out), ptr(grad_out), act, ptr(keep), float(keep_scale), ptr(g), m, n, ptr(part),
             lib.stream())
    if fused:
        lib.call('gv_colsum_finish', ptr(part), n, EPILOGUE_COLSUM_SLICES, ptr(colsum_out), 1 if colsum_accumulate else 0,
                 lib.stream())
    elif colsum_out is not None:
        colsum(g, out=colsum_out, accumulate=colsum_accumulate)
    return g


def axpby(alpha, x, beta=0.0, y=None, a=None):
    x = _chk(x.contiguous(), name='x')
    if y is None:
        y = torch.empty_like(x)
        beta = 0.0
    lib.call('gv_axpby', x.numel(), ptr(a), float(alpha), ptr(x), float(beta), ptr(y), lib.stream())
    return y


def copy_into(dst, src):
    src = _chk(src.contiguous(), name='src')
    if dst.numel() != src.numel() or not dst.is_contiguous():
        raise ValueError('copy_into: same size, contiguous destination')
    lib.call('gv_axpby', src.numel(), None, 1.0, ptr(src), 0.0, ptr(dst), lib.stream())
    return dst


def copy_of(x):
    return copy_into(torch.empty_like(x, memory_format=torch.contiguous_format), x)


class _CatRows(torch.autograd.Function):

    @staticmethod
    def forward(ctx, a, b):
        out = torch.empty(a.shape[0] + b.shape[0], a.shape[1], dtype=torch.float32, device=a.device)
        copy_into(out[:a.shape[0]], a)
        copy_into(out[a.shape[0]:], b)
        ctx.na = a.shape[0]
        return out

    @staticmethod
    def backward(ctx, g):
        return g[:ctx.na], g[ctx.na:]


def cat_rows(a, b):
    return _CatRows.apply(a, b)


class _SplitRows(torch.autograd.Function):

    @staticmethod
    def forward(ctx, x, n):
        ctx.n, ctx.shape = int(n), tuple(x.shape)
        ctx.set_materialize_grads(False)
# ... 145 lines not shown
    @staticmethod
    def forward(ctx, table, tick_rng):
        ctx.set_materialize_grads(False)
        if tick_rng is not None:
            tick_rng.tick()
        ctx.direct = _direct(table)
        _stamp_direct(ctx)
        return table.detach().view(table.shape)

    @staticmethod
    def backward(ctx, g):
        if g is None:
            return None, None
        g = _chk(g.contiguous(), name='grad')
        _verify_direct(ctx)
        tgt = ctx.direct
        if tgt is None:
            return g, None
        lib.call('gv_axpby', g.numel(), None, 1.0, ptr(g), 1.0, ptr(tgt), lib.stream())
        GRAD_FRESH.discard(tgt.data_ptr())
        return None, None


_identity_ids = {}


def _ids_are_identity(table, ids):
    if ids.numel() != table.shape[0]:
        return False
    key = (ids.data_ptr(), ids._version, ids.numel())
    hit = _identity_ids.get(key)
    if hit is None:
        if len(_identity_ids) > 64:
            _identity_ids.clear()
        hit = _identity_ids[key] = (bool((ids.reshape(-1) == torch.arange(ids.numel(), device=ids.device)).all()), ids)
    return hit[0]


def embedding(table, ids, tick_rng=None, sole_consumer=False):
    identity = False
    if table.is_cuda and isinstance(ids, torch.Tensor) and ids.is_cuda and ids.dtype == torch.int64:
        if torch.cuda.is_current_stream_capturing():
            hit = _identity_ids.get((ids.data_ptr(), ids._version, ids.numel()))
            identity = bool(hit and hit[0]) and ids.numel() == table.shape[0]
        else:
            identity = _ids_are_identity(table, ids)
    if identity and sole_consumer:
        out = _EmbeddingIdentity.apply(table, tick_rng)
        out._gv_grad_target = _direct(table)
        return out
    return _Embedding.apply(table, ids, tick_rng)


def _epilogue_grad(out, grad_out, act, keep, keep_scale, want_bias, d_b):
    if not want_bias:
        return epilogue_bwd(out, grad_out, act, keep, keep_scale), None
    grad_bias = d_b if d_b is not None else torch.empty(grad_out.shape[1], dtype=torch.float32, device=grad_out.device)
    g = epilogue_bwd(out, grad_out, act, keep, keep_scale, colsum_out=grad_bias, colsum_accumulate=d_b is not None)
    return g, (None if d_b is not None else grad_bias)


def _gemm_addend(x, loop_weight, h_bias, out_feat, loop_bf=None, riders=None):
    if riders is not None and (loop_weight is None or loop_bf is not None):
        riders.flush()
        riders = None
    if loop_weight is not None and loop_bf is not None:
        return dense_bf16(x, loop_bf[0], loop_weight.shape[1], loop_weight.shape[0], bias=h_bias)
    if loop_weight is not None:
        return gemm(x, loop_weight, bias=h_bias, riders=riders)
    if h_bias is not None:
        return h_bias.unsqueeze(0).expand(x.shape[0], out_feat).contiguous()
    return None


def _row_addend(h_bias, loop_rows, n, out_feat):
    if h_bias is None:
        return loop_rows
    addend = h_bias.unsqueeze(0).expand(n, out_feat).contiguous()
    if loop_rows is not None:
        lib.call('gv_axpby', addend.numel(), None, 1.0, ptr(loop_rows), 1.0, ptr(addend), lib.stream())
    return addend


def _loop_grads(x, g, loop_weight, d_l, want_loop, want_x, loop_bf=None):
    if loop_weight is None:
        return None, None
    grad_loop = gx_loop = None
    if want_loop:
        grad_loop = gemm(x, g, trans_a=True, split_k=pick_split_k(x.shape[1], g.shape[1], x.shape[0]), out=d_l,
                         accumulate=d_l is not None)
        if d_l is not None:
            grad_loop = None
    if want_x:
        if loop_bf is not None:
            gx_loop = dense_bf16(g, loop_bf[1], loop_weight.shape[0], loop_weight.shape[1])
        else:
            gx_loop = gemm(g, loop_weight, trans_b=True)
    return grad_loop, gx_loop


def _coef_order(gidx, ridx, coef, side):
    if gidx.sync_free or coef is None:
        return coef, (gidx.by_src.perm if side == 'src' else ridx.by_rel.perm)
    return (gidx.coef_in_src_order(coef) if side == 'src' else ridx.coef_in_rel_order(coef)), None


def _relation_weight_grad(gidx, ridx, coef, x, g, nb, si, so, d_w):
    coef_r, idx_r = _coef_order(gidx, ridx, coef, 'rel')
    grad_w = bdd_grad_weight(ridx.by_rel.seg, ridx.src_by_rel, ridx.dst_by_rel, coef_r, idx_r, x, g, nb, si, so, out=d_w,
                             accumulate=d_w is not None)
    return None if d_w is not None else grad_w


def _bdd_weight_fwd(ctx, weight, nb, si, so, pk, pk_bwd, riders=None):
    ctx.w_bwd_packed = None
    ctx.w_version = weight._version
    if pk and riders is not None:
        w_fwd = torch.empty_like(weight)
        if pk_bwd:
            ctx.w_bwd_packed = torch.empty_like(weight)
        riders.pack = (weight, nb, si, so, False, w_fwd, ctx.w_bwd_packed)
        return w_fwd
    if pk and pk_bwd:
        w_fwd, ctx.w_bwd_packed = torch.empty_like(weight), torch.empty_like(weight)
        lib.call('gv_rgcn_bdd_pack_weight_pair', ptr(weight), weight.shape[0], nb, si, so, ptr(w_fwd), ptr(ctx.w_bwd_packed),
                 lib.stream())
        return w_fwd
    return pack_weight(weight, nb, si, so, False) if pk else weight


def _bdd_weight_bwd(ctx, weight, nb, so, si):
    pk = si * so >= 8 and pack_supported(nb, so, si, True)
    if ctx.w_bwd_packed is not None and weight._version == ctx.w_version:
        return ctx.w_bwd_packed, pk
    return (pack_weight(weight, nb, so, si, True) if pk else weight), pk


def _bdd_k1(ctx, side, tl, gidx, ridx, coef, feat, weight, nb, bi, bo, plain_weight, addend, act=ACT_NONE, keep=None,
            keep_scale=1.0, out=None, sharded=False):
    trans, r = side == 'src', weight.shape[0]
    if tl is not None:
        return bdd_aggregate_phases(tl, None if coef is None else tl.coef(coef), feat, pack_weight_phase(tl, weight, nb, bi, bo),
                                    r, nb, bi, bo, addend(), act, keep, keep_scale, out=out)
    seg = gidx.by_src.seg if trans else gidx.by_dst.seg
    nbr, ety = (gidx.nbr_by_src, ridx.et_by_src) if trans else (gidx.nbr_by_dst, ridx.et_by_dst)

    def coef_operands():
        return _coef_order(gidx, ridx, coef, 'src') if trans else (coef, gidx.by_dst.perm)
    lp = None if (ctx.grouped or sharded) else lds_plan(r, nb, bi, bo, bf=ctx.k1_bf if trans else None)
    if lp is not None and lds_graph(gidx, side, lp[2]):
        if not trans:
            ctx.k1_bf = bool(lp[3])
            if not torch.cuda.is_current_stream_capturing():
                lp_b = lds_plan(r, nb, bo, bi, bf=ctx.k1_bf)
                if lp_b is not None:
                    gidx.lds_order('src', lp_b[2])
        c, c_idx = coef_operands()
        return bdd_aggregate_lds(gidx.lds_order(side, lp[2]), nbr, ety, c, c_idx, feat,
                                 pack_weight_lds(weight, nb, bi, bo, trans, lp), r, nb, bi, bo, trans, addend(), act, keep,
                                 keep_scale, out=out, plan=lp)
    w, pk = plain_weight()
    if ctx.grouped:
        seg_g, nbr_g, ety_g, perm = ridx.grouped_order(gidx, side)
        coef_g = None if coef is None else ridx.grouped_coef(coef, side, perm)
        return bdd_aggregate(seg_g, nbr_g, ety_g, coef_g, None, feat, w, nb, bi, bo, trans, addend(), act, keep, keep_scale,
                             out=out, packed=pk)
    if K1_REL_RUNS and not gidx.sync_free and not sharded:
        nbr_r, et_r, _, coef_r = ridx.rel_sorted(gidx, side, coef)
        return bdd_aggregate(_k1_items(gidx, seg), nbr_r, et_r, coef_r, None, feat, w, nb, bi, bo, trans, addend(), act, keep,
                             keep_scale, out=out, packed=pk)
    c, c_idx = coef_operands()
    return bdd_aggregate(_k1_items(gidx, seg), nbr, ety, c, c_idx, feat, w, nb, bi, bo, trans, addend(), act, keep, keep_scale,
                         out=out, packed=pk)


class _RelGraphConvBdd(torch.autograd.Function):

    @staticmethod
    def forward(ctx, x, weight, h_bias, loop_weight, norm, gidx, ridx, num_bases, act, keep, keep_scale,
                reduce_hook, link_box=None, riders=None):
        x, _ = _row_major(x, 'x')
        n, in_feat = x.shape
        if riders is not None and (reduce_hook is not None or loop_weight is None):
            riders.flush()
            riders = None
        si = in_feat // num_bases
        so = weight.shape[1] // (num_bases * si)
        out_feat = num_bases * so
        coef = None if norm is None else norm.reshape(-1)
        tl = None
        if reduce_hook is None and use_phases(gidx, si, so, False, x.shape[0], in_feat):
            tl = ridx.phase_order(gidx, 'dst', num_bases, si, so)
        pk = tl is None and si * so >= 8 and pack_supported(num_bases, si, so, False)
        bwd_phases = reduce_hook is None and use_phases(gidx, so, si, True, n, out_feat)
        pk_bwd = not bwd_phases and si * so >= 8 and pack_supported(num_bases, so, si, True)
        w_fwd = _bdd_weight_fwd(ctx, weight, num_bases, si, so, pk, pk_bwd and ctx.needs_input_grad[0], riders)
        ctx.loop_bf = dense_bf16_forms(loop_weight) if (loop_weight is not None and x.shape[0] >= 4096) else None

        def addend():
            return _gemm_addend(x, loop_weight, h_bias, out_feat, ctx.loop_bf, riders)

        ctx.grouped = tl is None and reduce_hook is None and use_relation_groups(weight, gidx)
        ctx.k1_bf = False
        if reduce_hook is None:
            out = _bdd_k1(ctx, 'dst', tl, gidx, ridx, coef, x, weight, num_bases, si, so, lambda: (w_fwd, pk), addend, act, keep,
                          keep_scale)
        else:
            agg = torch.empty(n, out_feat, dtype=torch.float32, device=x.device)
            pending = []
            for r0, r1, sub in gidx.dst_chunks(DIST_FWD_CHUNKS):
                bdd_aggregate(sub, gidx.nbr_by_dst, ridx.et_by_dst, coef, gidx.by_dst.perm, x, w_fwd, num_bases, si, so,
                              packed=pk, out=agg)
                pending.append(reduce_hook(agg[r0:r1]))
            add = addend()
            for h in pending:
                h.wait()
            out = epilogue_fwd(agg, add, act, keep, keep_scale)
        ctx.save_for_backward(x, weight, loop_weight, coef, out if act == ACT_RELU else None, keep)
        ctx.meta = (gidx, ridx, num_bases, si, so, act, keep_scale, h_bias is not None, reduce_hook)
        ctx.direct = (_direct(weight), _direct(h_bias), _direct(loop_weight))
        _stamp_direct(ctx)
        tgt = getattr(x, '_gv_grad_target', None)
        ctx.x_grad_target = tgt if (tgt is not None and reduce_hook is None and tuple(tgt.shape) == tuple(x.shape)) else None
        ctx.epi_link = None
        if link_box is not None and act == ACT_NONE and reduce_hook is None:
            ctx.epi_link = link_box[0] = EpilogueLink(keep, keep_scale, h_bias is not None and ctx.needs_input_grad[2],
                                                      ctx.direct[1], out_feat)
        return out

    @staticmethod
    def backward(ctx, grad_out):
        x, weight, loop_weight, coef, out, keep = ctx.saved_tensors
        gidx, ridx, nb, si, so, act, keep_scale, has_bias, reduce_hook = ctx.meta
        _verify_direct(ctx)
        d_w, d_b, d_l = ctx.direct
        folded = ctx.epi_link.take(grad_out) if ctx.epi_link is not None else None
        if folded is not None:
            g, grad_bias = folded
        else:
            g, grad_bias = _epilogue_grad(out, grad_out, act, keep, keep_scale, has_bias and ctx.needs_input_grad[2], d_b)
        pending = None
        g_agg = g
        if reduce_hook is not None:
            g_agg = copy_of(g)
            pending = reduce_hook(g_agg)
        side_w = reduce_hook is None and d_l is not None and d_w is not None and loop_weight is not None \
            and ctx.needs_input_grad[3] and ctx.needs_input_grad[1] and rgcn_bwd_side(gidx.num_edges, max(x.shape[1], g.shape[1]))
        if side_w:
            with backward_side(True, x, g, g_agg, weight, coef, rgcn=True):
                gw_first = rgcn_side_gradw_first(gidx.num_edges, x.shape[1])
                if not gw_first:
                    _loop_grads(x, g, loop_weight, d_l, True, False)
                _relation_weight_grad(gidx, ridx, coef, x, g_agg, nb, si, so, d_w)
                if gw_first:
                    _loop_grads(x, g, loop_weight, d_l, True, False)
        grad_loop, gx_loop = _loop_grads(x, g, loop_weight, d_l, ctx.needs_input_grad[3] and not side_w, ctx.needs_input_grad[0],
                                         ctx.loop_bf)
        if pending is not None:
            pending.wait()
        grad_x = None
        if ctx.needs_input_grad[0]:
            x_tgt = x_add = ctx.x_grad_target
            if x_tgt is not None:
                if x_tgt.data_ptr() in GRAD_FRESH:
                    GRAD_FRESH.discard(x_tgt.data_ptr())
                    x_add = None
                else:
                    x_tgt = None
            tl = None
            if reduce_hook is None and use_phases(gidx, so, si, True, g_agg.shape[0], g_agg.shape[1]):
                tl = ridx.phase_order(gidx, 'src', nb, so, si)
            grad_x = _bdd_k1(ctx, 'src', tl, gidx, ridx, coef, g_agg, weight, nb, so, si,
                             lambda: _bdd_weight_bwd(ctx, weight, nb, so, si), lambda: gx_loop, out=x_tgt,
                             sharded=reduce_hook is not None)
            if x_tgt is not None:
                grad_x = None
            elif x_add is not None:
                lib.call('gv_axpby', grad_x.numel(), None, 1.0, ptr(grad_x), 1.0, ptr(x_add), lib.stream())
                grad_x = None
        grad_w = None
        if ctx.needs_input_grad[1] and not side_w:
            grad_w = _relation_weight_grad(gidx, ridx, coef, x, g_agg, nb, si, so, d_w)
        return grad_x, grad_w, grad_bias, grad_loop, None, None, None, None, None, None, None, None, None, None


K1_REL_RUNS = _os.environ.get('GV_K1_REL_RUNS', '1') == '1'
REL_GROUPS = _os.environ.get('GV_REL_GROUPS', '0')
L2_WEIGHT_BUDGET = 3 << 20


def use_relation_groups(weight, gidx):
    if REL_GROUPS == '0' or gidx.sync_free or gidx.num_edges == 0:
        return False
    return REL_GROUPS == '1' or weight.numel() * 4 > L2_WEIGHT_BUDGET


def rel_graph_conv_bdd(x, weight, h_bias, loop_weight, norm, gidx, ridx, num_bases, act=ACT_NONE, keep=None,
                       keep_scale=1.0, reduce_hook=None, sole_consumer=False, riders=None):
    if not (sole_consumer and KL_SEAM_FOLD):
        return _RelGraphConvBdd.apply(x, weight, h_bias, loop_weight, norm, gidx, ridx, num_bases, act, keep,
                                      float(keep_scale), reduce_hook, None, riders)
    box = [None]
    out = _RelGraphConvBdd.apply(x, weight, h_bias, loop_weight, norm, gidx, ridx, num_bases, act, keep, float(keep_scale),
                                 reduce_hook, box, riders)
    out._gv_epi_link = box[0]
    return out


def rel_rows_gemm(feat, rows, w3, transpose_w, tiles, n_tiles, n_edges):
    feat, ld = _row_major(feat, 'feat')
# ... 570 lines not shown


def linear(x, w, b=None, act=ACT_NONE):
    return _Linear.apply(x, w, b, act)


class _Mul(torch.autograd.Function):

    @staticmethod
    def forward(ctx, mask, w):
        ctx.save_for_backward(mask)
        ctx.direct = _direct(w)
        _stamp_direct(ctx)
        return mul(mask, w)

    @staticmethod
    def backward(ctx, g):
        (mask,) = ctx.saved_tensors
        _verify_direct(ctx)
        tgt = ctx.direct
        if tgt is not None and tgt.data_ptr() in GRAD_FRESH and tgt.is_contiguous():
            g = _chk(g.contiguous(), name='grad')
            lib.call('gv_mul', g.numel(), ptr(mask), ptr(g), ptr(tgt), lib.stream())
            GRAD_FRESH.discard(tgt.data_ptr())
            return None, None
        return None, mul(mask, g)


def masked_weight(mask, w):
    return _Mul.apply(mask, w)


class KLLink:
    __slots__ = ('resp', 'ws', 'z_pre_ptr', 'z_pre_version', 'gkl', 'gscale', 'z_extra', 'claimed')

    def __init__(self, resp, ws, z_pre):
        self.resp, self.ws = resp, ws
        self.z_pre_ptr, self.z_pre_version = z_pre.data_ptr(), z_pre._version
        self.gkl = None
        self.gscale = self.z_extra = 0.0
        self.claimed = False

    def matches(self, z_pre):
        return z_pre is not None and z_pre.data_ptr() == self.z_pre_ptr and z_pre._version == self.z_pre_version


FUSE_REPARAM_KL = _os.environ.get('GV_FUSE_REPARAM_KL', '1') == '1'
KL_SEAM_FOLD = _os.environ.get('GV_KL_SEAM_FOLD', '1') == '1'
LOSS_COMBINE_WREL_MAX = 65536
KL_BWD_COLS4_KMAX = 10


class EpilogueLink:
    __slots__ = ('keep', 'keep_scale', 'want_bias', 'bias_target', 'n_bias', '_gv_direct_epoch', 'buf', 'buf_version', 'grad_bias')

    def __init__(self, keep, keep_scale, want_bias, bias_target, n_bias):
        self.keep, self.keep_scale = keep, float(keep_scale)
        self.want_bias, self.bias_target, self.n_bias = bool(want_bias), bias_target, int(n_bias)
        _stamp_direct(self)
        self.buf = self.grad_bias = None
        self.buf_version = 0

    def record(self, buf, grad_bias):
        self.buf, self.buf_version, self.grad_bias = buf, buf._version, grad_bias

    def take(self, grad_out):
        buf, version, grad_bias = self.buf, self.buf_version, self.grad_bias
        self.buf = self.grad_bias = None
        if buf is None:
            return None
        if (grad_out is None or grad_out.data_ptr() != buf.data_ptr() or tuple(grad_out.shape) != tuple(buf.shape)
                or grad_out.dtype != buf.dtype or not grad_out.is_contiguous() or grad_out._version != version):
            raise RuntimeError('the layer-2 epilogue gradient was folded into the KL backward (ops.EpilogueLink), but the gradient '
                               'arriving at the layer is not that buffer: something else consumed the layer output as well and '
                               'its gradient was added unmasked.  Only hand an EpilogueLink to ops.reparam when it is the sole '
                               'consumer (GV_KL_SEAM_FOLD=0 turns the fold off)')
        return grad_out, grad_bias


def kl_seam_fold_ok(epi, gm, gv, h, k, tensors=()):
    if epi is None or not KL_SEAM_FOLD or gm is not None or gv is not None:
        return False
    if _os.environ.get('GV_KL_BWD_V4', '1') == '0' or h % 4 != 0 or h > 1024 or not 1 <= k <= KL_BWD_COLS4_KMAX:
        return False
    if epi.keep is not None and (epi.keep.data_ptr() % 4 != 0 or not epi.keep.is_contiguous()
                                 or tuple(epi.keep.shape)[-1] != 2 * h or epi.keep.dtype != torch.uint8):
        return False
    if epi.want_bias and epi.n_bias != 2 * h:
        return False
    return all(t is None or t.data_ptr() % 16 == 0 for t in tensors)


class _Reparam(torch.autograd.Function):

    @staticmethod
    def forward(ctx, h2, eps, z_pre, link_box, epi_link=None, kl_ws=None):
        ctx.set_materialize_grads(False)
        h2 = _chk(h2.contiguous(), name='h2')
        n, h = h2.shape[0], h2.shape[1] // 2
        eps = _chk(eps.contiguous(), name='eps')
        z = torch.empty(n, h, dtype=torch.float32, device=h2.device)
        v = torch.empty_like(z)
        m = torch.empty_like(z)
        ctx.link = None
        ctx.epi_link = epi_link if z_pre is not None else None
        if z_pre is not None:
            z_pre = _chk(z_pre.contiguous(), name='z_pre')
            k = z_pre.shape[0] // 2
            resp = torch.empty(n, k, dtype=torch.float32, device=h2.device)
            if kl_ws is not None and kl_ws.matches(z_pre, n, h, k):
                ws = kl_ws.ws
                lib.call('gv_reparam_kl_fwd_mix', ptr(h2), ptr(eps), ptr(z_pre), ptr(z), ptr(v), ptr(m), ptr(resp), ptr(ws), 1, n, h,
                         k, lib.stream())
            else:
                ws = torch.empty(kl_workspace_floats(n, h, k), dtype=torch.float32, device=h2.device)
                lib.call('gv_reparam_kl_fwd', ptr(h2), ptr(eps), ptr(z_pre), ptr(z), ptr(v), ptr(m), ptr(resp), ptr(ws), n, h, k,
                         lib.stream())
            ctx.link = link_box[0] = KLLink(resp, ws, z_pre)
            ctx.save_for_backward(h2, eps, v, z, z_pre)
        else:
            lib.call('gv_reparam_fwd', ptr(h2), ptr(eps), ptr(z), ptr(v), ptr(m), n, h, lib.stream())
            ctx.save_for_backward(h2, eps, v)
        return z, m, v

    @staticmethod
    def backward(ctx, gz, gm, gv):
        link, epi = ctx.link, ctx.epi_link
        if epi is not None:
            epi.buf = epi.grad_bias = None
        if link is not None and link.gkl is not None:
            h2, eps, v, z, z_pre = ctx.saved_tensors
            n, h = v.shape
            k = z_pre.shape[0] // 2
            gz = None if gz is None else _chk(gz.contiguous(), name='gz')
            d_zp = _direct_flat(z_pre)
            gzp = d_zp if d_zp is not None else torch.empty_like(z_pre)
            gh2 = torch.empty_like(h2)
            if kl_seam_fold_ok(epi, gm, gv, h, k, (z, h2, v, eps, link.resp, link.ws, gz, gh2)):
                g_bias = d_b = None
                if epi.want_bias:
                    d_b = epi.bias_target
                    if d_b is not None:
                        _verify_direct(epi)
                    g_bias = d_b if d_b is not None else torch.empty(2 * h, dtype=torch.float32, device=h2.device)
                lib.call('gv_reparam_kl_bwd_fold', ptr(z), ptr(h2), ptr(v), ptr(eps), ptr(z_pre), ptr(link.resp), ptr(link.gkl),
                         float(link.gscale), float(link.z_extra), ptr(gz), ptr(gh2), ptr(gzp), 1 if d_zp is not None else 0,
                         ptr(epi.keep), epi.keep_scale, ptr(g_bias), 1 if d_b is not None else 0, ptr(link.ws), n, h, k,
                         lib.stream())
                link.gkl = None
                epi.record(gh2, None if d_b is not None else g_bias)
                return gh2, None, (None if d_zp is not None else gzp), None, None, None
            lib.call('gv_reparam_kl_bwd', ptr(z), ptr(h2), ptr(v), ptr(eps), ptr(z_pre), ptr(link.resp), ptr(link.gkl),
                     float(link.gscale), float(link.z_extra), ptr(gz), ptr(gh2), ptr(gzp), 1 if d_zp is not None else 0,
                     ptr(link.ws), n, h, k, lib.stream())
            link.gkl = None
            if gm is not None or gv is not None:
                extra = torch.empty_like(h2)
                gm = None if gm is None else _chk(gm.contiguous(), name='gm')
                gv = None if gv is None else _chk(gv.contiguous(), name='gv')
                lib.call('gv_reparam_bwd', ptr(h2), ptr(eps), ptr(v), None, ptr(gm), ptr(gv), ptr(extra), n, h, lib.stream())
                gh2 += extra
            return gh2, None, (None if d_zp is not None else gzp), None, None, None
        h2, eps, v = ctx.saved_tensors[:3]
        n, h = v.shape
        gz = None if gz is None else _chk(gz.contiguous(), name='gz')
        gm = None if gm is None else _chk(gm.contiguous(), name='gm')
        gv = None if gv is None else _chk(gv.contiguous(), name='gv')
        gh2 = torch.empty_like(h2)
        lib.call('gv_reparam_bwd', ptr(h2), ptr(eps), ptr(v), ptr(gz), ptr(gm), ptr(gv), ptr(gh2), n, h, lib.stream())
        return gh2, None, None, None, None, None


def kl_workspace_floats(n, h, k):
    return int(lib.load().gv_kl_workspace_bytes(n, h, k)) // 4


class KLWorkspace:
    __slots__ = ('ws', 'z_pre', 'key')

    def __init__(self, z_pre, n):
        z_pre = _chk(z_pre.detach().contiguous(), name='z_pre')
        k, h = z_pre.shape[0] // 2, z_pre.shape[1]
        self.z_pre = z_pre
        self.ws = torch.empty(kl_workspace_floats(n, h, k), dtype=torch.float32, device=z_pre.device)
        self.key = (z_pre.data_ptr(), z_pre._version, int(n), h, k)

    def matches(self, z_pre, n, h, k):
        return (z_pre.data_ptr(), z_pre._version, int(n), h, k) == self.key


def reparam(h2, eps, z_pre=None, epi_link=None, kl_ws=None):
    if z_pre is None or not FUSE_REPARAM_KL:
        return _Reparam.apply(h2, eps, None, None, None, None)
    box = [None]
    z, m, v = _Reparam.apply(h2, eps, z_pre, box, epi_link if KL_SEAM_FOLD else None, kl_ws)
    z._gv_kl_link = box[0]
    return z, m, v


DISTMULT_FUSED = _os.environ.get('GV_DISTMULT_FUSED', '1') == '1'

# ... 343 lines not shown
        gx, gy = torch.empty_like(x), torch.empty_like(y)
        lib.call('gv_mmd_bwd', ptr(x), ptr(y), None, x.shape[0], y.shape[0], x.shape[1], ptr(g), 1.0, ptr(gx), ptr(gy),
                 lib.stream())
        return gx, gy


def mmd(x, y):
    return _MMD.apply(x, y)


MMD_FUSED = _os.environ.get('GV_MMD_FUSED', '1') == '1'


def mmd_sweep_ok(z_pri, z, h_max=256):
    h = z_pri.shape[1]
    return (MMD_FUSED and h % 4 == 0 and h <= h_max and z.shape[1] == h and z_pri.data_ptr() % 16 == 0
            and z.data_ptr() % 16 == 0)


class PriorLink:
    __slots__ = ('z_pre', 'eps', 'out_ptr', 'out_version', 'out_shape', 'claimed', 'buf', 'buf_version', 'gz')

    def __init__(self, z_pre, eps, out):
        self.z_pre, self.eps = z_pre, eps
        self.out_ptr, self.out_version, self.out_shape = out.data_ptr(), out._version, tuple(out.shape)
        self.claimed = False
        self.buf = self.gz = None
        self.buf_version = 0

    def matches(self, z_pri):
        return (z_pri is not None and z_pri.data_ptr() == self.out_ptr and z_pri._version == self.out_version
                and tuple(z_pri.shape) == self.out_shape and z_pri.is_contiguous())

    def record(self, buf, gz):
        self.buf, self.buf_version, self.gz = buf, buf._version, gz

    def take(self, grad_out):
        buf, version, gz = self.buf, self.buf_version, self.gz
        self.buf = self.gz = None
        if buf is None:
            return None
        if (grad_out is None or grad_out.data_ptr() != buf.data_ptr() or tuple(grad_out.shape) != tuple(buf.shape)
                or grad_out.dtype != buf.dtype or not grad_out.is_contiguous() or grad_out._version != version):
            raise RuntimeError('the prior sampler\'s backward was folded into the loss head\'s MMD finishing launch (ops.PriorLink), '
                               'but the gradient arriving at the sampler is not that buffer: something else consumed z_pri as well.  '
                               'Only hand a linked z_pri to ops.loss_head when the head is its sole consumer (GV_MMD_FUSED=0 turns '
                               'the fold off)')
        return (gz,)


class _PriorSample(torch.autograd.Function):

    @staticmethod
    def forward(ctx, z_pre, eps, link_box=None):
        z_pre, eps = _chk(z_pre.contiguous(), name='z_pre'), _chk(eps.contiguous(), name='eps')
        k, h = z_pre.shape[0] // 2, z_pre.shape[1]
        out = torch.empty_like(eps)
        ctx.set_materialize_grads(False)
        lib.call('gv_prior_sample_fwd', ptr(z_pre), ptr(eps), ptr(out), eps.shape[0], k, h, lib.stream())
        ctx.save_for_backward(z_pre, eps)
        ctx.link = None
        if link_box is not None and eps.shape[0] % k == 0:
            ctx.link = link_box[0] = PriorLink(z_pre, eps, out)
        return out

    @staticmethod
    def backward(ctx, g):
        z_pre, eps = ctx.saved_tensors
        link = ctx.link
        if link is not None and link.claimed:
            folded = link.take(g)
            if folded is not None:
                return folded[0], None, None
        if g is None:
            return None, None, None
        g = _chk(g.contiguous(), name='g')
        d_zp = _direct_flat(z_pre)
        gz = d_zp if d_zp is not None else torch.empty_like(z_pre)
        lib.call('gv_prior_sample_bwd', ptr(z_pre), ptr(eps), ptr(g), ptr(gz), 1 if d_zp is not None else 0, eps.shape[0],
                 z_pre.shape[0] // 2, z_pre.shape[1], lib.stream())
        return (None if d_zp is not None else gz), None, None


def prior_sample(z_pre, eps):
    if not MMD_FUSED:
        return _PriorSample.apply(z_pre, eps)
    box = [None]
    out = _PriorSample.apply(z_pre, eps, box)
    out._gv_prior_link = box[0]
    return out


class _LossHead(torch.autograd.Function):

    @staticmethod
    def forward(ctx, z, z_mean, z_sigma, w_rel, z_pre, flp, z_pri, pick, labels, tidx, reg_w, kl_w, mmd_w, score_bias,
                embed_rows=None, rows_dev=None, kl_link=None, grad_mode=True, prior_link=None):
        z, ld_z = _row_major(z, 'embed')
        if rows_dev is not None:
            rows_dev = _chk(rows_dev.reshape(-1), torch.int32, 'rows_dev')
            if kl_w <= 0 or embed_rows is not None:
                raise NotImplementedError('rows_dev needs kl_w > 0 (the padding rows are masked in the KL pass) and no embed_rows')
        w_rel, ld_w = _row_major(w_rel, 'w_relation')
        labels = _chk(labels.reshape(-1), name='labels')
        dev, (n, h), T = z.device, z.shape, tidx.T
        if labels.numel() != T:
            raise ValueError('labels / triplets length mismatch')
        f32 = dict(dtype=torch.float32, device=dev)
        ctx.set_materialize_grads(False)
        scal = torch.empty(4, **f32)
        pred, reg, kl, mmd = scal[0:1], scal[1:2], scal[2:3], scal[3:4]
        ws, ws2 = torch.empty(2048, **f32), torch.empty(1024, **f32)
        score = torch.empty(T, **f32)
        loss = torch.empty((), **f32)
        bias = flp if (score_bias and flp is not None) else None
        resp = wsk = z_post = wsm = None
        link = kl_link if (kl_link is not None and not kl_link.claimed and kl_w > 0 and flp is None and rows_dev is None
                           and embed_rows is None and kl_link.matches(z_pre) and kl_link.resp.shape[0] == n) else None
        if link is not None:
            link.claimed = True
        if kl_w > 0:
            z_mean, z_sigma = _chk(z_mean.contiguous(), name='z_mean'), _chk(z_sigma.contiguous(), name='z_sigma')
            z_pre = _chk(z_pre.contiguous(), name='z_pre')
            k = z_pre.shape[0] // 2
            if link is None:
                wsk = torch.empty(int(lib.load().gv_kl_workspace_bytes(n, h, k)) // 4, **f32)
                resp = torch.empty(n, k, **f32)
        if mmd_w > 0:
            z_pri = _chk(z_pri.contiguous(), name='z_pri')
            pick = _chk(pick.reshape(-1), torch.int64, 'pick')
            wsm = torch.empty(z_pri.shape[0] + pick.numel(), **f32)
        if ld_z != h or ld_w != h:
            raise ValueError('loss_head needs contiguous embeddings and relation table')
        dm_fused = grad_mode and (ctx.needs_input_grad[0] or ctx.needs_input_grad[3]) and distmult_fused_ok(z, ld_z, w_rel, ld_w)
        plink = prior_link if (mmd_w > 0 and dm_fused and prior_link is not None and not prior_link.claimed
                               and prior_link.matches(z_pri) and mmd_sweep_ok(z_pri, z)
                               and z_pri.shape[0] + pick.numel() <= 1024) else None
        if plink is not None:
            plink.claimed = True
        ctx.prior_link = plink
        st = lib.stream()
# ... 559 lines not shown
```

include/gcnvae.h:

```cpp
#ifndef GCNVAE_H
#define GCNVAE_H

#include <stdint.h>

#ifdef __cplusplus
extern "C" {
#endif

typedef enum {
    GV_OK = 0,
    GV_ERR_NULL = -1,
    GV_ERR_SHAPE = -2,
    GV_ERR_ALIGN = -3,
    GV_ERR_WORKSPACE = -4
} gv_status;

enum { GV_ACT_NONE = 0, GV_ACT_RELU = 1 };

int gv_version(void);
const char* gv_last_error_string(void);

int gv_segment_items_count(const int32_t* rowptr, int n_seg, int chunk, int32_t* n_chunks, int32_t* n_slots,
                           int32_t* is_split, void* stream);
int gv_segment_items_fill(const int32_t* rowptr, int n_seg, int chunk, const int32_t* item_off,
// ... 381 lines not shown
int64_t gv_transe_entity_topk_typed_workspace_bytes(int m, int n_tiles, int k, int span_tiles);
int gv_transe_entity_topk_typed(const int32_t* ents, int m, const float* en, const float* rn, int n, int num_rels, int dim, int head,
                                int p_norm, const int32_t* filt_lo, const int32_t* filt_hi, const int32_t* filt_ent, int n_filt_ent,
                                const int64_t* set_ptr, const int32_t* set_ids, const int32_t* tile_ptr, int n_tiles, int cand_base,
                                int exclude_self, int k, int span_tiles, int64_t* out_rel, int64_t* out_ent, float* out_dist,
                                void* workspace, int64_t workspace_bytes, void* stream);

int gv_transe_pair_rel(const float* en, const float* rn, int n, int num_rels, int dim, int p_norm, const int32_t* s, const int32_t* o,
                       const int32_t* target, const int32_t* filt_lo, const int32_t* filt_hi, const int32_t* filt_rel, int n_filt_rel,
                       int k, float* tgt, int32_t* count_raw, int32_t* count_filt, int64_t* out_ids, float* out_dist, int m,
                       void* stream);

int gv_transe_pair_rel_constrained(const float* en, const float* rn, int n, int num_rels, int dim, int p_norm, const int32_t* s,
                                   const int32_t* o, const int32_t* target, const int32_t* filt_lo, const int32_t* filt_hi,
                                   const int32_t* filt_rel, int n_filt_rel, const uint32_t* cand, int ld_cand, int n_sets, int k,
                                   float* tgt, int32_t* count_raw, int32_t* count_filt, int32_t* count_raw_c, int32_t* count_filt_c,
                                   int64_t* out_ids, float* out_dist, int m, void* stream);

int64_t gv_transe_mine_workspace_bytes(int n, int num_rels, int n_filt_ent);
int gv_transe_mine(const float* en, const float* rn, int n, int num_rels, int dim, int p_norm, const int32_t* filt_lo,
                   const int32_t* filt_hi, const int32_t* filt_ent, int n_filt_ent, int exclude_self, int mode, uint32_t key_min,
                   int prefix_bits, uint32_t prefix, int bin_bits, int32_t* out, int64_t capacity, uint64_t* counter, uint64_t* hist,
                   void* workspace, int64_t workspace_bytes, void* stream);

int gv_transe_mine_typed(const float* en, const float* rn, int n, int num_rels, int dim, int p_norm, const int64_t* set_ptr,
                         const int32_t* set_ids, const int32_t* units, int64_t n_units, const int32_t* filt_lo,
                         const int32_t* filt_hi, const int32_t* filt_ent, int n_filt_ent, int exclude_self, int mode,
                         uint32_t key_min, int prefix_bits, uint32_t prefix, int bin_bits, int32_t* out, int64_t capacity,
                         uint64_t* counter, uint64_t* hist, void* stream);

int64_t gv_gemm_workspace_bytes(int m, int n, int k, int split_k);
int gv_gemm_f32(int trans_a, int trans_b, int m, int n, int k, const float* a, int lda, const float* b, int ldb,
                float* c, int ldc, const float* bias, int act, int accumulate, int split_k, const float* a_relu_mask,
                void* workspace, int64_t workspace_bytes, void* stream);
typedef struct gv_riders {
    const uint64_t* rng_state;
    void* rng_ptr[8];
    int64_t rng_count[8];
    int32_t rng_kind[8];
    float rng_drop_p[8];
    uint32_t rng_stream[8];
    int32_t rng_jobs;
    int32_t pack_rels, pack_bases, pack_blk_in, pack_blk_out, pack_transpose;
    const float* pack_weight;
    float* packed;
    float* packed_pair;
    const float* mix_z_pre;
    float* mix;
    int32_t mix_k, mix_h;
} gv_riders;
int gv_gemm_f32_riders(int trans_a, int trans_b, int m, int n, int k, const float* a, int lda, const float* b, int ldb, float* c,
                       int ldc, const float* bias, int act, int accumulate, int split_k, const float* a_relu_mask, void* workspace,
                       int64_t workspace_bytes, const gv_riders* riders, void* stream);
int gv_gemm_f32_live_rows(int trans_a, int trans_b, int m, int n, int k, const float* a, int lda, const float* b, int ldb, float* c,
                          int ldc, const float* bias, int act, int accumulate, int split_k, const float* a_relu_mask, void* workspace,
                          int64_t workspace_bytes, const int32_t* rows_dev, void* stream);
int gv_gemm_f32_sparse(int trans_a, int trans_b, int m, int n, int k, const float* a, int lda, const float* b, int ldb, float* c,
                       int ldc, const float* bias, int act, int accumulate, int split_k, const float* a_relu_mask, void* workspace,
                       int64_t workspace_bytes, const int32_t* rows_dev , const uint64_t* b_k_chunks,
                       const uint64_t* c_tiles, int c_tiles_wanted, void* stream);
int gv_gemm_bf16(int trans_a, int trans_b, int m, int n, int k, const float* a, int lda, const float* b, int ldb,
                float* c, int ldc, const float* bias, int act, int accumulate, int split_k, const float* a_relu_mask,
                void* workspace, int64_t workspace_bytes, void* stream);

int gv_colsum(const float* x, const float* relu_mask, int64_t m, int n, int ld, float* out, float* workspace,
              int accumulate, void* stream);

int gv_gather_rows(const float* table, const int64_t* ids, float* out, int64_t n, int h, void* stream);
int gv_gather_rows_rng_tick(const float* table, const int64_t* ids, float* out, int64_t n, int h, uint64_t* rng_state,
                            void* stream);
int gv_scatter_add_rows(const float* grad_out, const int64_t* ids, float* grad_table, int64_t n, int h, void* stream);

#define GV_RNG_MAX_JOBS 8
#define GV_RNG_KEEP_MASK 0
#define GV_RNG_NORMAL 1
int gv_rng_fill(const uint64_t* rng_state, int n_jobs, void* const* ptrs, const int64_t* counts, const int32_t* kinds,
                const float* drop_p, const uint32_t* streams, void* stream);
int gv_rng_tick(uint64_t* rng_state, void* stream);

int gv_reparam_fwd(const float* h2, const float* eps, float* z, float* v, float* m_out ,
                   int64_t n, int h, void* stream);
int gv_reparam_bwd(const float* h2, const float* eps, const float* v, const float* gz, const float* gm,
                   const float* gv, float* grad_h2, int64_t n, int h, void* stream);

int gv_distmult_bce_fwd(const float* embed, int ld_e, const float* w_rel, int ld_w, const int32_t* triplets,
                        const int32_t* order ,
                        const float* labels, const float* bias, float* score, float* loss, float* workspace,
                        int64_t t, int h, void* stream);
int gv_bce_grad(const float* score, const float* labels, const float* gloss, float* dscore,
                const int32_t* pos3 , float* dscore_inc , float* dscore_rel ,
                float* dbias, float* workspace, int64_t t, void* stream);

int gv_distmult_bce_fwd_grad(const int32_t* items, int n_items, const int32_t* rel_s, const int32_t* rel_o,
                             const int32_t* rel_tid, const float* embed, int ld_e, const float* w_rel, int ld_w,
                             const float* labels, const float* bias, const int32_t* pos3, float* score, float* delta,
                             float* u, float* partial, float* workspace, int64_t t, int h, void* stream);
int gv_distmult_grad_finish(const float* gloss, const float* u, const float* partial, const int32_t* fix, int n_fix,
                            const int32_t* rowptr, int chunk, int num_rels, int h, const float* w_rel, int ld_w,
                            float reg_scale, float* grad_w, int ld_gw, int accumulate, const float* delta, float* d_out,
                            int64_t n_coef, const float* workspace, float* dbias, int64_t t, void* stream);

int gv_mean_sq(const float* x, int64_t n, float scale, float* out, float* workspace, int accumulate, void* stream);
int gv_mean_sq2(const float* x1, int64_t n1, float scale1, const float* x2, int64_t n2, float scale2, float* out,
                float* workspace, const int32_t* rows_dev, int64_t rows_host, void* stream);
int gv_axpby(int64_t n, const float* a, float alpha, const float* x, float beta, float* y, void* stream);
int gv_mul(int64_t n, const float* a, const float* b, float* out, void* stream);
#define GV_MUL_MULTI_MAX 8
int gv_mul_multi(int count, const float* const* a, const float* const* b, float* const* out, const int64_t* n, void* stream);
int64_t gv_kl_workspace_bytes(int64_t n, int h, int k);
int gv_kl_fwd(const float* z, const float* m, int ld_m, const float* v, const float* z_pre, const float* flp,
              float* resp, float* kl, float* workspace, int64_t n, int h, int k, const int32_t* rows_dev, void* stream);
int gv_kl_bwd(const float* z, const float* m, int ld_m, const float* v, const float* z_pre, const float* resp,
              const float* gkl, float gscale, float z_extra, float* gz, float* gm, float* gv, float* g_zpre,
              int accumulate_zpre, float* workspace, int mix_ready, int64_t n, int h, int k, const int32_t* rows_dev,
              void* stream);
int gv_reparam_kl_fwd(const float* h2, const float* eps, const float* z_pre, float* z, float* v, float* m_out, float* resp,
                      float* workspace, int64_t n, int h, int k, void* stream);
int gv_reparam_kl_fwd_mix(const float* h2, const float* eps, const float* z_pre, float* z, float* v, float* m_out, float* resp,
                          float* workspace, int mix_ready, int64_t n, int h, int k, void* stream);
int gv_kl_mix(const float* z_pre, int k, int h, float* mix, void* stream);
int gv_reparam_kl_bwd(const float* z, const float* h2, const float* v, const float* eps, const float* z_pre, const float* resp,
                      const float* gkl, float gscale, float z_extra, const float* gz_up, float* gh2, float* g_zpre,
                      int accumulate_zpre, float* workspace, int64_t n, int h, int k, void* stream);
#define GV_LOSS_COMBINE_WREL_MAX 65536
int gv_reparam_kl_bwd_fold(const float* z, const float* h2, const float* v, const float* eps, const float* z_pre,
                           const float* resp, const float* gkl, float gscale, float z_extra, const float* gz_up, float* gh2,
                           float* g_zpre, int accumulate_zpre, const uint8_t* keep, float keep_scale, float* g_bias,
                           int accumulate_bias, float* workspace, int64_t n, int h, int k, void* stream);
int gv_loss_combine_fold(const float* ws_pred, int64_t t, const float* w_rel, int64_t n_embed, int64_t n_wrel,
                         const float* ws_kl, int64_t n_nodes, int h, int k, const float* ws_mmd, int sx, int sy, float reg_w,
                         float kl_w, float mmd_w, float* scal , float* loss, void* stream);

int gv_loss_combine(const float* ws_pred, int64_t t, const float* ws_reg, int64_t n_embed, int64_t n_wrel,
                    const float* ws_kl, int64_t n_nodes, int h, int k, const float* ws_mmd, int sx, int sy, float reg_w,
                    float kl_w, float mmd_w, float* scal , float* loss, const int32_t* rows_dev,
                    void* stream);
int gv_lincomb4(const float* a0, float c0, const float* a1, float c1, const float* a2, float c2, const float* a3,
                float c3, float* out, void* stream);
int gv_mmd_fwd(const float* x, const float* y, const int64_t* y_index, int sx, int sy, int h, float* mmd, float* workspace,
               void* stream);
int gv_mmd_bwd(const float* x, const float* y, const int64_t* y_index, int sx, int sy, int h, const float* gmmd, float gscale,
               float* gx, float* gy, void* stream);
int gv_prior_sample_fwd(const float* z_pre, const float* eps, float* out, int s, int k, int h, void* stream);
int gv_prior_sample_bwd(const float* z_pre, const float* eps, const float* g, float* gz_pre, int accumulate, int s, int k,
                        int h, void* stream);
int gv_mmd_fwd_grad(const float* x, const float* y, const int64_t* y_index, int sx, int sy, int h, float* part, float* gx_u,
                    float* gy_u, void* stream);
int gv_distmult_bce_fwd_grad_mmd(const int32_t* items, int n_items, const int32_t* rel_s, const int32_t* rel_o,
                                 const int32_t* rel_tid, const float* embed, int ld_e, const float* w_rel, int ld_w,
                                 const float* labels, const float* bias, const int32_t* pos3, float* score, float* delta,
                                 float* u, float* partial, float* workspace, int64_t t, int h, const float* mmd_x,
                                 const float* mmd_y, const int64_t* mmd_y_index, int sx, int sy, int mmd_h, float* mmd_part,
                                 float* gx_u, float* gy_u, void* stream);
int gv_mmd_grad_finish(const float* gx_u, const float* gy_u, const int64_t* y_index, int sx, int sy, int h, const float* gmmd,
                       float gscale, float* gy, float* g_pri, const float* z_pre, const float* eps, float* gz_pre,
                       int accumulate, int k, void* stream);

int gv_iaf_update_fwd(const float* z, const float* net, int ld_net, const float* x_old, const int32_t* colcount,
                      float* x_new, int64_t n, int d, void* stream);
int gv_iaf_update_bwd(const float* z, const float* net, int ld_net, const int32_t* colcount, const float* g_xnew,
                      const float* g_logdet , float* g_z, float* g_net, float* g_xold, int64_t n, int d,
                      void* stream);
int gv_iaf_update_bwd_acc(const float* z, const float* net, int ld_net, const int32_t* colcount, const float* g_xnew,
                          const float* g_logdet, float* g_z, int gz_accumulate, float* g_net, float* g_xold, int64_t n, int d,
                          void* stream);
int gv_rowsum(const float* x, int ld, int col0, int ncols, float* out, int64_t n, void* stream);
int gv_reverse_cols(const float* x, float* out, int64_t n, int d, void* stream);
int gv_mean_rows_multi(int count, const float* const* x, int64_t n, const int32_t* rows_dev, float* out, float* workspace,
                       void* stream);
int gv_mean_rows_bwd(const float* g, int64_t len, int64_t n, const int32_t* rows_dev, float* out, void* stream);

int gv_adam_step(float* p, const float* g, float* exp_avg, float* exp_avg_sq, int64_t n, const float* sumsq,
                 float max_norm, float lr, float beta1, float beta2, float eps, const float* step, void* stream);
int gv_clip_adam_step(float* p, float* g, float* exp_avg, float* exp_avg_sq, int64_t n, float* workspace,
                      float* sumsq_out, float max_norm, float lr, float beta1, float beta2, float eps, float* step,
                      int zero_grad, void* stream);

void gv_index_caps(int64_t n_entries, int n_seg, int chunk, int* items_cap, int* fix_cap, int* slots_cap);
int64_t gv_index_workspace_bytes(int64_t n_entries, int n_seg_max);
int gv_build_csr(const int32_t* keys, int64_t n, int n_seg, int chunk, int32_t* perm, int32_t* rowptr, int32_t* items,
                 int items_cap, int32_t* fix, int fix_cap, void* workspace, int64_t workspace_bytes, void* stream);
// ... 61 lines not shown
```

Before: 611.6 million edges/s.

## Ride prior sampling, KL-mix and column-sum finishers on GEMM launches

Adds a finisher rider set (prior sampler, KL-mixture gradient finalisation, column-sum reduction) that executes as extra blocks inside an existing riders GEMM launch, including a new A @ B^T backward variant. The KL backward fold can now skip its own final reduction and hand the partials to a rider, and prior sampling can be deferred into a rider box. The aim is to remove several small separate kernel launches and the serial gaps between them. In exchange it adds ordering and aliasing checks, and Python bookkeeping that raises an error if a deferred finisher is never run.

```diff
diff --git a/gcn-vae_amd/csrc/common.h b/gcn-vae_amd/csrc/common.h
--- a/gcn-vae_amd/csrc/common.h
+++ b/gcn-vae_amd/csrc/common.h
@@ -130,8 +130,7 @@
     }
 }
 
-__device__ __forceinline__ float sum_slices_16x64(const float* __restrict__ part, int ncols, int nsl, int col, float (*sm)[16]) {
-    const int cl = threadIdx.x & 15, grp = threadIdx.x >> 4;
+__device__ __forceinline__ float slice_group_sum(const float* __restrict__ part, int ncols, int nsl, int col, int grp) {
     const int per = (nsl + 63) / 64;
     const int s0 = grp * per, s1 = min(nsl, s0 + per);
     float a0 = 0.f, a1 = 0.f, a2 = 0.f, a3 = 0.f;
@@ -144,13 +143,37 @@
         }
         for (; s < s1; ++s) a0 += part[(size_t)s * ncols + col];
     }
-    sm[grp][cl] = (a0 + a1) + (a2 + a3);
-    __syncthreads();
+    return (a0 + a1) + (a2 + a3);
+}
+
+__device__ __forceinline__ float slice_groups_total(const float (*sm)[16]) {
+    const int cl = threadIdx.x & 15;
     float tot = 0.f;
-    if (grp == 0) {
+    if ((threadIdx.x >> 4) == 0) {
 #pragma unroll 8
         for (int g = 0; g < 64; ++g) tot += sm[g][cl];
     }
+    return tot;
+}
+
+__device__ __forceinline__ float sum_slices_16x64(const float* __restrict__ part, int ncols, int nsl, int col, float (*sm)[16]) {
+    const int cl = threadIdx.x & 15, grp = threadIdx.x >> 4;
+    sm[grp][cl] = slice_group_sum(part, ncols, nsl, col, grp);
+    __syncthreads();
+    return slice_groups_total(sm);
+}
+
+__device__ __forceinline__ float sum_slices_16x64_wg256(const float* __restrict__ part, int ncols, int nsl, int col, float (*sm)[16]) {
+    const int cl = threadIdx.x & 15, t = threadIdx.x >> 4;
+    float g4[4];
+#pragma unroll
+    for (int q = 0; q < 4; ++q) g4[q] = slice_group_sum(part, ncols, nsl, col, t + 16 * q);
+    __syncthreads();
+#pragma unroll
+    for (int q = 0; q < 4; ++q) sm[t + 16 * q][cl] = g4[q];
+    __syncthreads();
+    const float tot = slice_groups_total(sm);
+    __syncthreads();
     return tot;
 }
 
diff --git a/gcn-vae_amd/csrc/k_gemm.hip b/gcn-vae_amd/csrc/k_gemm.hip
--- a/gcn-vae_amd/csrc/k_gemm.hip
+++ b/gcn-vae_amd/csrc/k_gemm.hip
@@ -294,13 +294,14 @@
 template <bool TA, bool TB, int MT, int NT, int BK>
 __global__ __launch_bounds__(256) __attribute__((amdgpu_waves_per_eu(MT == 2 ? 5 : 7))) void k_gemm_f32_riders(const GemmParams p, const RiderSet rs, const int ntn, const int ntm,
                                                          const int n_riders, const int riders_front) {
+    __shared__ float rider_sm[64][16];
     const int tiles = ntn * ntm;
     int b = blockIdx.x;
     if (riders_front) {
-        if (b < n_riders) { rider_body(rs, b, n_riders); return; }
+        if (b < n_riders) { rider_body(rs, b, n_riders, rider_sm); return; }
         b -= n_riders;
     } else if (b >= tiles) {
-        rider_body(rs, b - tiles, n_riders);
+        rider_body(rs, b - tiles, n_riders, rider_sm);
         return;
     }
     const int by = b / ntn;
@@ -1250,7 +1251,7 @@
     __shared__ float sm[64][16];
     const int c = blockIdx.x * 16 + (threadIdx.x & 15);
     const float acc = sum_slices_16x64(part, n, nsl, c, sm);
-    if ((threadIdx.x >> 4) == 0 && c < n) out[c] = accumulate ? out[c] + acc : acc;
+    if ((threadIdx.x >> 4) == 0 && c < n) colsum_final_store(acc, c, out, accumulate);
 }
 
 }
@@ -1372,20 +1373,26 @@
 inline int64_t matrix_bytes(int rows, int cols, int ld) { return rows > 0 && cols > 0 ? ((int64_t)(rows - 1) * ld + cols) * 4 : 0; }
 }
 
-extern "C" int gv_gemm_f32_riders(int trans_a, int trans_b, int m, int n, int k, const float* a, int lda, const float* b, int ldb,
-                                  float* c, int ldc, const float* bias, int act, int accumulate, int split_k,
-                                  const float* a_relu_mask, void* workspace, int64_t workspace_bytes, const gv_riders* riders,
-                                  void* stream) {
-    const bool any = riders && (riders->rng_jobs > 0 || riders->pack_weight || riders->mix_z_pre);
+static const gv_riders NO_RIDERS = {};
+
+static int gemm_riders(int trans_a, int trans_b, int m, int n, int k, const float* a, int lda, const float* b, int ldb,
+                       float* c, int ldc, const float* bias, int act, int accumulate, int split_k,
+                       const float* a_relu_mask, void* workspace, int64_t workspace_bytes, const gv_riders* riders,
+                       const gv_riders_fin* fin, void* stream) {
+    const bool any_fin = fin && (fin->prior_z_pre || fin->kl_part || fin->cs_part);
+    const bool any = (riders && (riders->rng_jobs > 0 || riders->pack_weight || riders->mix_z_pre)) || any_fin;
     if (!any)
         return gemm_any(false, trans_a, trans_b, m, n, k, a, lda, b, ldb, c, ldc, bias, act, accumulate, split_k, a_relu_mask,
                         workspace, workspace_bytes, stream);
+    if (!riders) riders = &NO_RIDERS;
     GV_REQUIRE(split_k <= 1, GV_ERR_SHAPE, "gv_gemm_f32_riders: riders do not ride on a split-K product (split_k=%d)", split_k);
-    GV_REQUIRE(!trans_a && !trans_b, GV_ERR_SHAPE, "gv_gemm_f32_riders: riders ride on A @ B only (the forward self-loop product)");
+    GV_REQUIRE(!trans_a && (!trans_b || fin), GV_ERR_SHAPE,
+               "gv_gemm_f32_riders: riders ride on A @ B (the forward self-loop product) and, through gv_gemm_f32_riders_fin, on "
+               "A @ B^T (the backward's) only");
     GV_REQUIRE(m > 0 && n > 0 && k >= 0, GV_ERR_SHAPE, "gv_gemm_f32_riders: m=%d n=%d k=%d", m, n, k);
     GV_REQUIRE(c && (k == 0 || (a && b)), GV_ERR_NULL, "gv_gemm_f32_riders: NULL matrix");
-    GV_REQUIRE(lda >= k && ldb >= n && ldc >= n, GV_ERR_SHAPE, "gv_gemm_f32_riders: leading dimension too small (lda=%d ldb=%d ldc=%d)",
-               lda, ldb, ldc);
+    GV_REQUIRE(lda >= k && ldb >= (trans_b ? k : n) && ldc >= n, GV_ERR_SHAPE,
+               "gv_gemm_f32_riders: leading dimension too small (lda=%d ldb=%d ldc=%d)", lda, ldb, ldc);
     GV_REQUIRE(act == GV_ACT_NONE || act == GV_ACT_RELU, GV_ERR_SHAPE, "gv_gemm_f32_riders: unknown act %d", act);
     GemmParams p;
     p.a = a; p.b = b; p.c = c; p.bias = bias; p.a_mask = a_relu_mask; p.ws = nullptr;
@@ -1401,7 +1408,7 @@
     const int ntm = (m + 64 * mt - 1) / (64 * mt);
     GV_REQUIRE((int64_t)ntn * ntm < (1ll << 30), GV_ERR_SHAPE, "gv_gemm_f32_riders: %d x %d tiles", ntn, ntm);
 
-    const Extent ea = extent_of(a, matrix_bytes(m, k, lda)), eb = extent_of(b, matrix_bytes(k, n, ldb)),
+    const Extent ea = extent_of(a, matrix_bytes(m, k, lda)), eb = extent_of(b, trans_b ? matrix_bytes(n, k, ldb) : matrix_bytes(k, n, ldb)),
                  ec = extent_of(c, matrix_bytes(m, n, ldc)), ebias = extent_of(bias, (int64_t)n * 4),
                  emask = extent_of(a_relu_mask, matrix_bytes(m, k, lda));
     auto written_ok = [&](const Extent& w) { return !(overlaps(w, ea) || overlaps(w, eb) || overlaps(w, ec) || overlaps(w, ebias) || overlaps(w, emask)); };
@@ -1483,12 +1490,90 @@
         nblk += (mk * mh + 255) / 256;
     }
     rs.first[3] = nblk;
+    Extent fin_out[3] = {{nullptr, nullptr}, {nullptr, nullptr}, {nullptr, nullptr}};
+    if (any_fin && fin->prior_z_pre) {
+        const int s = fin->prior_s, pk = fin->prior_k, ph = fin->prior_h;
+        GV_REQUIRE(fin->prior_eps && fin->prior_out, GV_ERR_NULL, "gv_gemm_f32_riders_fin: NULL prior buffer");
+        GV_REQUIRE(s > 0 && pk > 0 && ph > 0 && (int64_t)s * ph < (1ll << 28) && (int64_t)pk * ph < (1ll << 28), GV_ERR_SHAPE,
+                   "gv_gemm_f32_riders_fin: prior s=%d k=%d h=%d", s, pk, ph);
+        const Extent ez = extent_of(fin->prior_z_pre, (int64_t)2 * pk * ph * 4), ee = extent_of(fin->prior_eps, (int64_t)s * ph * 4),
+                     eo = extent_of(fin->prior_out, (int64_t)s * ph * 4);
+        GV_REQUIRE(read_ok(ez) && read_ok(ee) && written_ok(eo) && !overlaps(eo, ez) && !overlaps(eo, ee), GV_ERR_SHAPE,
+                   "gv_gemm_f32_riders_fin: a prior sampler buffer overlaps an operand of the product or its own input");
+        for (int j = 0; j < riders->rng_jobs; ++j) {
+            const Extent ej = extent_of(riders->rng_ptr[j], riders->rng_count[j] * (riders->rng_kind[j] == GV_RNG_NORMAL ? 4 : 1));
+            GV_REQUIRE(!overlaps(ej, ee) && !overlaps(ej, ez) && !overlaps(ej, eo), GV_ERR_SHAPE,
+                       "gv_gemm_f32_riders_fin: the prior sampler reads or writes what rng job %d of the same launch writes", j);
+        }
+        GV_REQUIRE(!overlaps(eo, extent_of(riders->mix, (int64_t)3 * riders->mix_k * riders->mix_h * 4)), GV_ERR_SHAPE,
+                   "gv_gemm_f32_riders_fin: the prior samples overlap the mixture table");
+        rs.prior.z_pre = fin->prior_z_pre; rs.prior.eps = fin->prior_eps; rs.prior.out = fin->prior_out;
+        rs.prior.s = s; rs.prior.k = pk; rs.prior.h = ph;
+        fin_out[0] = eo;
+        nblk += (s * ph + 255) / 256;
+    }
+    rs.first[4] = nblk;
+    if (any_fin && fin->kl_part) {
+        const int kh_ = fin->kl_h, kk = fin->kl_k, nsl = fin->kl_slices;
+        GV_REQUIRE(fin->kl_z_pre && fin->kl_g_zpre, GV_ERR_NULL, "gv_gemm_f32_riders_fin: NULL KL finisher buffer");
+        GV_REQUIRE(kh_ > 0 && kk > 0 && nsl > 0 && fin->kl_n > 0 && (int64_t)(2 * kk + 2) * kh_ < (1ll << 28), GV_ERR_SHAPE,
+                   "gv_gemm_f32_riders_fin: KL finisher n=%lld h=%d k=%d slices=%d", (long long)fin->kl_n, kh_, kk, nsl);
+        const int cols = (2 * kk + (fin->kl_g_bias ? 2 : 0)) * kh_;
+        const Extent ep = extent_of(fin->kl_part, (int64_t)nsl * cols * 4), ez = extent_of(fin->kl_z_pre, (int64_t)2 * kk * kh_ * 4),
+                     eg = extent_of(fin->kl_gkl, 4), eo = extent_of(fin->kl_g_zpre, (int64_t)2 * kk * kh_ * 4),
+                     ebo = extent_of(fin->kl_g_bias, (int64_t)2 * kh_ * 4);
+        GV_REQUIRE(read_ok(ep) && read_ok(ez) && read_ok(eg) && written_ok(eo) && written_ok(ebo) && !overlaps(eo, ebo) &&
+                       !overlaps(eo, ep) && !overlaps(eo, ez) && !overlaps(eo, eg) && !overlaps(ebo, ep) && !overlaps(ebo, ez) &&
+                       !overlaps(ebo, eg) && !overlaps(eo, fin_out[0]) && !overlaps(ebo, fin_out[0]),
+                   GV_ERR_SHAPE, "gv_gemm_f32_riders_fin: a KL finisher buffer overlaps an operand of the product or another rider buffer");
+        KlFinJob& kj = rs.klfin;
+        kj.part = fin->kl_part; kj.z_pre = fin->kl_z_pre; kj.gkl = fin->kl_gkl; kj.gscale = fin->kl_gscale;
+        kj.g_zpre = fin->kl_g_zpre; kj.g_bias = fin->kl_g_bias; kj.n = fin->kl_n; kj.accumulate = fin->kl_accumulate;
+        kj.accumulate_bias = fin->kl_accumulate_bias; kj.h = kh_; kj.k = kk; kj.nsl = nsl;
+        fin_out[1] = eo; fin_out[2] = ebo;
+        nblk += (cols + 15) / 16;
+    }
+    rs.first[5] = nblk;
+    if (any_fin && fin->cs_part) {
+        const int cn = fin->cs_n, nsl = fin->cs_slices;
+        GV_REQUIRE(fin->cs_out, GV_ERR_NULL, "gv_gemm_f32_riders_fin: NULL column-sum target");
+        GV_REQUIRE(cn > 0 && nsl > 0 && (int64_t)cn * nsl < (1ll << 28), GV_ERR_SHAPE, "gv_gemm_f32_riders_fin: column sums n=%d slices=%d",
+                   cn, nsl);
+        const Extent ep = extent_of(fin->cs_part, (int64_t)nsl * cn * 4), eo = extent_of(fin->cs_out, (int64_t)cn * 4);
+        GV_REQUIRE(read_ok(ep) && written_ok(eo) && !overlaps(eo, ep) && !overlaps(eo, fin_out[0]) && !overlaps(eo, fin_out[1]) &&
+                       !overlaps(eo, fin_out[2]) && !overlaps(ep, fin_out[0]) && !overlaps(ep, fin_out[1]) && !overlaps(ep, fin_out[2]),
+                   GV_ERR_SHAPE, "gv_gemm_f32_riders_fin: a column-sum buffer overlaps an operand of the product or another rider buffer");
+        rs.colsum.part = fin->cs_part; rs.colsum.out = fin->cs_out; rs.colsum.n = cn; rs.colsum.nsl = nsl;
+        rs.colsum.accumulate = fin->cs_accumulate;
+        nblk += (cn + 15) / 16;
+    }
+    rs.first[6] = nblk;
     const int n_riders = front ? (nblk + 7) / 8 * 8 : nblk;
     const dim3 grid((unsigned)(ntn * ntm + n_riders)), block(256);
     hipStream_t st = (hipStream_t)stream;
-    if (mt == 2) hipLaunchKernelGGL((k_gemm_f32_riders<false, false, 2, 1, 16>), grid, block, 0, st, p, rs, ntn, ntm, n_riders, front ? 1 : 0);
-    else hipLaunchKernelGGL((k_gemm_f32_riders<false, false, 1, 1, 16>), grid, block, 0, st, p, rs, ntn, ntm, n_riders, front ? 1 : 0);
+#define GV_RIDERS_LAUNCH(TB_, MT_) \
+    hipLaunchKernelGGL((k_gemm_f32_riders<false, TB_, MT_, 1, 16>), grid, block, 0, st, p, rs, ntn, ntm, n_riders, front ? 1 : 0)
+    if (trans_b) { if (mt == 2) GV_RIDERS_LAUNCH(true, 2); else GV_RIDERS_LAUNCH(true, 1); }
+    else { if (mt == 2) GV_RIDERS_LAUNCH(false, 2); else GV_RIDERS_LAUNCH(false, 1); }
+#undef GV_RIDERS_LAUNCH
     return launch_status("gv_gemm_f32_riders");
+}
+
+extern "C" int gv_gemm_f32_riders(int trans_a, int trans_b, int m, int n, int k, const float* a, int lda, const float* b, int ldb,
+                                  float* c, int ldc, const float* bias, int act, int accumulate, int split_k,
+                                  const float* a_relu_mask, void* workspace, int64_t workspace_bytes, const gv_riders* riders,
+                                  void* stream) {
+    return gemm_riders(trans_a, trans_b, m, n, k, a, lda, b, ldb, c, ldc, bias, act, accumulate, split_k, a_relu_mask, workspace,
+                       workspace_bytes, riders, nullptr, stream);
+}
+
+extern "C" int gv_gemm_f32_riders_fin(int trans_a, int trans_b, int m, int n, int k, const float* a, int lda, const float* b, int ldb,
+                                      float* c, int ldc, const float* bias, int act, int accumulate, int split_k,
+                                      const float* a_relu_mask, void* workspace, int64_t workspace_bytes, const gv_riders* riders,
+                                      const gv_riders_fin* fin, void* stream) {
+    static const gv_riders_fin none = {};
+    return gemm_riders(trans_a, trans_b, m, n, k, a, lda, b, ldb, c, ldc, bias, act, accumulate, split_k, a_relu_mask, workspace,
+                       workspace_bytes, riders, fin ? fin : &none, stream);
 }
 
 extern "C" int gv_gemm_f32_live_rows(int trans_a, int trans_b, int m, int n, int k, const float* a, int lda, const float* b,
diff --git a/gcn-vae_amd/csrc/k_loss.hip b/gcn-vae_amd/csrc/k_loss.hip
--- a/gcn-vae_amd/csrc/k_loss.hip
+++ b/gcn-vae_amd/csrc/k_loss.hip
@@ -877,16 +877,7 @@
     const int i = blockIdx.x * 16 + (threadIdx.x & 15);
     float acc = sum_slices_16x64(part, total, nsl, i, sm);
     if ((threadIdx.x >> 4) != 0 || i >= total) return;
-    if (i >= 2 * kh) {
-        g_bias[i - 2 * kh] = accumulate_bias ? g_bias[i - 2 * kh] + acc : acc;
-        return;
-    }
-    const float cg = gscale * (gkl ? *gkl : 1.f) / (float)(rows_dev ? (int64_t)*rows_dev : n);
-    if (i >= kh) {
-        const float raw = z_pre[i];
-        acc *= raw > 20.f ? 1.f : 1.f / (1.f + expf(-raw));
-    }
-    g_zpre[i] = accumulate ? g_zpre[i] + cg * acc : cg * acc;
+    kl_mix_final_store(acc, i, kh, z_pre, gkl, gscale, g_zpre, accumulate, n, rows_dev, g_bias, accumulate_bias);
 }
 
 constexpr int MMD_WAVES = 16;
@@ -1276,12 +1267,7 @@
 }
 
 __global__ __launch_bounds__(256) void k_prior_sample_fwd(const float* z_pre, const float* eps, float* out, int s, int k, int h) {
-    const int total = s * h;
-    for (int i = blockIdx.x * 256 + threadIdx.x; i < total; i += gridDim.x * 256) {
-        const int r = i / h, c = i - r * h, j = r % k;
-        const float v = softplus_t(z_pre[(size_t)(k + j) * h + c]) + 1e-8f;
-        out[i] = z_pre[(size_t)j * h + c] + eps[i] * sqrtf(v);
-    }
+    prior_sample_body(z_pre, eps, out, s, k, h, (int)blockIdx.x, (int)gridDim.x);
 }
 
 __global__ __launch_bounds__(256) void k_prior_sample_bwd(const float* z_pre, const float* eps, const float* g, float* gz_pre,
@@ -1806,11 +1792,11 @@
     return launch_status("gv_reparam_kl_bwd");
 }
 
-extern "C" int gv_reparam_kl_bwd_fold(const float* z, const float* h2, const float* v, const float* eps, const float* z_pre,
-                                      const float* resp, const float* gkl, float gscale, float z_extra, const float* gz_up,
-                                      float* gh2, float* g_zpre, int accumulate_zpre, const uint8_t* keep, float keep_scale,
-                                      float* g_bias, int accumulate_bias, float* workspace, int64_t n, int h, int k,
-                                      void* stream) {
+static int reparam_kl_bwd_fold(const float* z, const float* h2, const float* v, const float* eps, const float* z_pre,
+                               const float* resp, const float* gkl, float gscale, float z_extra, const float* gz_up,
+                               float* gh2, float* g_zpre, int accumulate_zpre, const uint8_t* keep, float keep_scale,
+                               float* g_bias, int accumulate_bias, float* workspace, int64_t n, int h, int k,
+                               void* stream, bool finish) {
     GV_REQUIRE(z && h2 && v && eps && z_pre && resp && gh2 && g_zpre && workspace, GV_ERR_NULL,
                "gv_reparam_kl_bwd_fold: NULL pointer");
     GV_REQUIRE(n > 0 && h > 0 && k > 0 && k <= KL_FUSED_KT, GV_ERR_SHAPE, "gv_reparam_kl_bwd_fold: n=%lld h=%d k=%d (k <= %d)",
@@ -1824,9 +1810,42 @@
                             gz_up, gh2, keep, keep_scale, g_bias != nullptr),
                GV_ERR_SHAPE, "gv_reparam_kl_bwd_fold: h=%d k=%d or an unaligned operand: only the float4-column backward "
                "(h %% 4 == 0, k <= 10, 16-B rows) folds the epilogue gradient", h, k);
-    hipLaunchKernelGGL(k_kl_bwd_mix_final, dim3((cols + 15) / 16), dim3(1024), 0, GV_ST, (const float*)part, z_pre, gkl, gscale,
-                       g_zpre, accumulate_zpre, n, h, k, KL_SLICES, no_rows, g_bias, accumulate_bias);
+    if (finish)
+        hipLaunchKernelGGL(k_kl_bwd_mix_final, dim3((cols + 15) / 16), dim3(1024), 0, GV_ST, (const float*)part, z_pre, gkl, gscale,
+                           g_zpre, accumulate_zpre, n, h, k, KL_SLICES, no_rows, g_bias, accumulate_bias);
     return launch_status("gv_reparam_kl_bwd_fold");
+}
+
+extern "C" int gv_reparam_kl_bwd_fold(const float* z, const float* h2, const float* v, const float* eps, const float* z_pre,
+                                      const float* resp, const float* gkl, float gscale, float z_extra, const float* gz_up,
+                                      float* gh2, float* g_zpre, int accumulate_zpre, const uint8_t* keep, float keep_scale,
+                                      float* g_bias, int accumulate_bias, float* workspace, int64_t n, int h, int k,
+                                      void* stream) {
+    return reparam_kl_bwd_fold(z, h2, v, eps, z_pre, resp, gkl, gscale, z_extra, gz_up, gh2, g_zpre, accumulate_zpre, keep, keep_scale,
+                               g_bias, accumulate_bias, workspace, n, h, k, stream, true);
+}
+
+extern "C" int gv_reparam_kl_bwd_fold_sweep(const float* z, const float* h2, const float* v, const float* eps, const float* z_pre,
+                                            const float* resp, const float* gkl, float gscale, float z_extra, const float* gz_up,
+                                            float* gh2, float* g_zpre, const uint8_t* keep, float keep_scale, float* g_bias,
+                                            float* workspace, int64_t n, int h, int k, void* stream) {
+    return reparam_kl_bwd_fold(z, h2, v, eps, z_pre, resp, gkl, gscale, z_extra, gz_up, gh2, g_zpre, 0, keep, keep_scale, g_bias, 0,
+                               workspace, n, h, k, stream, false);
+}
+
+extern "C" int64_t gv_kl_bwd_part_offset(int h, int k) { return 3 * (int64_t)k * h + RED_BLOCKS; }
+extern "C" int gv_kl_bwd_slices(void) { return KL_SLICES; }
+
+extern "C" int gv_kl_bwd_mix_final(const float* part, int n_slices, const float* z_pre, const float* gkl, float gscale, float* g_zpre,
+                                   int accumulate_zpre, float* g_bias, int accumulate_bias, int64_t n, int h, int k, void* stream) {
+    GV_REQUIRE(part && z_pre && g_zpre, GV_ERR_NULL, "gv_kl_bwd_mix_final: NULL pointer");
+    GV_REQUIRE(n > 0 && h > 0 && k > 0 && n_slices > 0 && (int64_t)(2 * k + 2) * h < (1ll << 28), GV_ERR_SHAPE,
+               "gv_kl_bwd_mix_final: n=%lld h=%d k=%d n_slices=%d", (long long)n, h, k, n_slices);
+    const int cols = (2 * k + (g_bias ? 2 : 0)) * h;
+    const int* no_rows = nullptr;
+    hipLaunchKernelGGL(k_kl_bwd_mix_final, dim3((cols + 15) / 16), dim3(1024), 0, GV_ST, part, z_pre, gkl, gscale, g_zpre,
+                       accumulate_zpre, n, h, k, n_slices, no_rows, g_bias, accumulate_bias);
+    return launch_status("gv_kl_bwd_mix_final");
 }
 
 __global__ void k_lincomb(const float* a0, float c0, const float* a1, float c1, const float* a2, float c2, const float* a3,
diff --git a/gcn-vae_amd/csrc/k_riders.h b/gcn-vae_amd/csrc/k_riders.h
--- a/gcn-vae_amd/csrc/k_riders.h
+++ b/gcn-vae_amd/csrc/k_riders.h
@@ -87,6 +87,65 @@
     }
 }
 
+__device__ __forceinline__ void prior_sample_body(const float* z_pre, const float* eps, float* out, int s, int k, int h, int bid, int nblk) {
+    const int total = s * h;
+    for (int i = bid * 256 + threadIdx.x; i < total; i += nblk * 256) {
+        const int r = i / h, c = i - r * h, j = r % k;
+        const float v = softplus_t(z_pre[(size_t)(k + j) * h + c]) + 1e-8f;
+        out[i] = z_pre[(size_t)j * h + c] + eps[i] * sqrtf(v);
+    }
+}
+
+__device__ __forceinline__ void kl_mix_final_store(float acc, int i, int kh, const float* z_pre, const float* gkl, float gscale,
+                                                   float* g_zpre, int accumulate, int64_t n, const int* rows_dev, float* g_bias,
+                                                   int accumulate_bias) {
+    if (i >= 2 * kh) {
+        g_bias[i - 2 * kh] = accumulate_bias ? g_bias[i - 2 * kh] + acc : acc;
+        return;
+    }
+    const float cg = gscale * (gkl ? *gkl : 1.f) / (float)(rows_dev ? (int64_t)*rows_dev : n);
+    if (i >= kh) {
+        const float raw = z_pre[i];
+        acc *= raw > 20.f ? 1.f : 1.f / (1.f + expf(-raw));
+    }
+    g_zpre[i] = accumulate ? g_zpre[i] + cg * acc : cg * acc;
+}
+
+struct KlFinJob {
+    const float* part;
+    const float* z_pre;
+    const float* gkl;
+    float gscale;
+    float* g_zpre;
+    float* g_bias;
+    long long n;
+    int accumulate, accumulate_bias, h, k, nsl;
+};
+
+__device__ __forceinline__ void kl_mix_final_body(const KlFinJob& j, int bid, float (*sm)[16]) {
+    const int kh = j.k * j.h, total = 2 * kh + (j.g_bias ? 2 * j.h : 0);
+    const int i = bid * 16 + (threadIdx.x & 15);
+    const float acc = sum_slices_16x64_wg256(j.part, total, j.nsl, i, sm);
+    if ((threadIdx.x >> 4) != 0 || i >= total) return;
+    kl_mix_final_store(acc, i, kh, j.z_pre, j.gkl, j.gscale, j.g_zpre, j.accumulate, j.n, nullptr, j.g_bias, j.accumulate_bias);
+}
+
+struct ColsumJob {
+    const float* part;
+    float* out;
+    int n, nsl, accumulate;
+};
+
+__device__ __forceinline__ void colsum_final_store(float acc, int c, float* out, int accumulate) {
+    out[c] = accumulate ? out[c] + acc : acc;
+}
+
+__device__ __forceinline__ void colsum_final_body(const ColsumJob& j, int bid, float (*sm)[16]) {
+    const int c = bid * 16 + (threadIdx.x & 15);
+    const float acc = sum_slices_16x64_wg256(j.part, j.n, j.nsl, c, sm);
+    if ((threadIdx.x >> 4) == 0 && c < j.n) colsum_final_store(acc, c, j.out, j.accumulate);
+}
+
 struct PackJob {
     const float* w;
     float* packed;
@@ -101,15 +160,25 @@
     int k, h;
 };
 
+struct PriorJob {
+    const float* z_pre;
+    const float* eps;
+    float* out;
+    int s, k, h;
+};
+
 struct RiderSet {
     const uint64_t* rng_state;
     RngJobs rng;
     PackJob pack;
     MixJob mix;
-    int first[4];
-};
-
-__device__ __forceinline__ void rider_body(const RiderSet& rs, int b, int n) {
+    PriorJob prior;
+    KlFinJob klfin;
+    ColsumJob colsum;
+    int first[7];
+};
+
+__device__ __forceinline__ void rider_body(const RiderSet& rs, int b, int n, float (*sm)[16]) {
     (void)n;
     if (b < rs.first[1]) {
         rng_fill_body(rs.rng_state, rs.rng, b, rs.first[1]);
@@ -120,7 +189,14 @@
                          second ? pj.adj2 : pj.adj, second ? i - pj.blocks : i, pj.blocks);
     } else if (b < rs.first[3]) {
         kl_mix_body(rs.mix.z_pre, rs.mix.k, rs.mix.h, rs.mix.mix, b - rs.first[2], rs.first[3] - rs.first[2]);
-    }
-}
-
-}
+    } else if (b < rs.first[4]) {
+        prior_sample_body(rs.prior.z_pre, rs.prior.eps, rs.prior.out, rs.prior.s, rs.prior.k, rs.prior.h, b - rs.first[3],
+                          rs.first[4] - rs.first[3]);
+    } else if (b < rs.first[5]) {
+        kl_mix_final_body(rs.klfin, b - rs.first[4], sm);
+    } else if (b < rs.first[6]) {
+        colsum_final_body(rs.colsum, b - rs.first[5], sm);
+    }
+}
+
+}
diff --git a/gcn-vae_amd/encoders.py b/gcn-vae_amd/encoders.py
--- a/gcn-vae_amd/encoders.py
+++ b/gcn-vae_amd/encoders.py
@@ -95,7 +95,7 @@
     def get_kl(self, z):
         return ops.kl_to_mixture(z, self.z_mean, self.z_sigma, self.z_pre.squeeze(0), self.flow_log_prob)
 
-    def _prior_draw(self, device, dtype):
+    def _prior_draw(self, device, dtype, riders=None):
         num_sample = 200
         rows = (num_sample // self.k) * self.k if num_sample // self.k > 1 else self.k
         if self.mmd_eps_override is not None:
@@ -105,7 +105,7 @@
         else:
             eps = torch.empty(rows, self.h_dim, device=device, dtype=dtype)
             ops.device_rng(device).fill([(eps, ops.RNG_NORMAL, 0.0, self.rng_stream_prior)])
-        return ops.prior_sample(self.z_pre.squeeze(0), eps)
+        return ops.prior_sample(self.z_pre.squeeze(0), eps, riders)
 
     def _prior_rows(self):
         num_sample = 200
@@ -230,12 +230,16 @@
         if box2 is not None and fuse_kl and ops.FUSE_REPARAM_KL:
             kl_ws = ops.KLWorkspace(self.z_pre.squeeze(0), h.shape[0])
             box2.mix = (kl_ws.z_pre, kl_ws.ws)
+        z_pri = None
+        if (box2 is not None and self.n_flows == 0 and self._prior_eps_next is not None and ops.rider_kind('prior')
+                and ops.MMD_FUSED and self.h_dim % 4 == 0 and self.h_dim <= 256):
+            z_pri = self._prior_draw(h.device, h.dtype, box2)
         h = self.rconv_layer_2(g, h, r, norm, sole_consumer=fuse_kl, riders=box2)
         if box2 is not None and not box2.done:
             raise RuntimeError('KGVAE.forward: layer 2 dropped its RiderBox (weight packing / KL mixture table never launched)')
         z, self.z_mean, self.z_sigma = ops.reparam(h, eps, self.z_pre.squeeze(0) if fuse_kl else None,
                                                    getattr(h, '_gv_epi_link', None) if fuse_kl else None, kl_ws)
-        self._z_pri_flowed = None
+        self._z_pri_flowed = z_pri
         if self.n_flows > 0:
             z, self.flow_log_prob = self._apply_flows(z, want_mean=True)
             ops.made_prepare_finish()
diff --git a/gcn-vae_amd/lib.py b/gcn-vae_amd/lib.py
--- a/gcn-vae_amd/lib.py
+++ b/gcn-vae_amd/lib.py
@@ -53,6 +53,11 @@
     'gv_gemm_workspace_bytes': (_L, [_I, _I, _I, _I]),
     'gv_gemm_f32': (_I, [_I, _I, _I, _I, _I, _P, _I, _P, _I, _P, _I, _P, _I, _I, _I, _P, _P, _L, _P]),
     'gv_gemm_f32_riders': (_I, [_I, _I, _I, _I, _I, _P, _I, _P, _I, _P, _I, _P, _I, _I, _I, _P, _P, _L, _P, _P]),
+    'gv_gemm_f32_riders_fin': (_I, [_I, _I, _I, _I, _I, _P, _I, _P, _I, _P, _I, _P, _I, _I, _I, _P, _P, _L, _P, _P, _P]),
+    'gv_reparam_kl_bwd_fold_sweep': (_I, [_P, _P, _P, _P, _P, _P, _P, _F, _F, _P, _P, _P, _P, _F, _P, _P, _L, _I, _I, _P]),
+    'gv_kl_bwd_part_offset': (_L, [_I, _I]),
+    'gv_kl_bwd_slices': (_I, []),
+    'gv_kl_bwd_mix_final': (_I, [_P, _I, _P, _P, _F, _P, _I, _P, _I, _L, _I, _I, _P]),
     'gv_gemm_f32_live_rows': (_I, [_I, _I, _I, _I, _I, _P, _I, _P, _I, _P, _I, _P, _I, _I, _I, _P, _P, _L, _P, _P]),
     'gv_gemm_f32_sparse': (_I, [_I, _I, _I, _I, _I, _P, _I, _P, _I, _P, _I, _P, _I, _I, _I, _P, _P, _L, _P, _P, _P, _I, _P]),
     'gv_gemm_bf16': (_I, [_I, _I, _I, _I, _I, _P, _I, _P, _I, _P, _I, _P, _I, _I, _I, _P, _P, _L, _P]),
diff --git a/gcn-vae_amd/ops.py b/gcn-vae_amd/ops.py
--- a/gcn-vae_amd/ops.py
+++ b/gcn-vae_amd/ops.py
@@ -353,7 +353,16 @@
 
 
 GEMM_RIDERS = _os.environ.get('GV_GEMM_RIDERS', '1') == '1'
-GEMM_RIDER_KINDS = set(_os.environ.get('GV_GEMM_RIDER_KINDS', 'rng,pack,mix').split(','))
+RIDER_KINDS_ALL = ('rng', 'pack', 'mix', 'prior', 'klfin', 'colsum')
+GEMM_RIDER_KINDS = set(_os.environ.get('GV_GEMM_RIDER_KINDS', ','.join(RIDER_KINDS_ALL)).split(','))
+
+
+def rider_kind(kind):
+    return GEMM_RIDERS and kind in GEMM_RIDER_KINDS
+
+
+def _dist_active():
+    return torch.distributed.is_available() and torch.distributed.is_initialized()
 
 
 class _Riders(_ct.Structure):
@@ -365,16 +374,30 @@
                 ('mix_k', _ct.c_int32), ('mix_h', _ct.c_int32)]
 
 
+class _RidersFin(_ct.Structure):
+    _fields_ = [('prior_z_pre', _ct.c_void_p), ('prior_eps', _ct.c_void_p), ('prior_out', _ct.c_void_p), ('kl_part', _ct.c_void_p),
+                ('kl_z_pre', _ct.c_void_p), ('kl_gkl', _ct.c_void_p), ('kl_g_zpre', _ct.c_void_p), ('kl_g_bias', _ct.c_void_p),
+                ('cs_part', _ct.c_void_p), ('cs_out', _ct.c_void_p), ('kl_n', _ct.c_int64), ('kl_gscale', _ct.c_float),
+                ('prior_s', _ct.c_int32), ('prior_k', _ct.c_int32), ('prior_h', _ct.c_int32), ('kl_slices', _ct.c_int32),
+                ('kl_h', _ct.c_int32), ('kl_k', _ct.c_int32), ('kl_accumulate', _ct.c_int32), ('kl_accumulate_bias', _ct.c_int32),
+                ('cs_n', _ct.c_int32), ('cs_slices', _ct.c_int32), ('cs_accumulate', _ct.c_int32)]
+
+
 class RiderBox:
-    __slots__ = ('rng', 'pack', 'mix', 'done', 'rode')
+    __slots__ = ('rng', 'pack', 'mix', 'prior', 'klfin', 'colsum', 'done', 'rode')
 
     def __init__(self):
-        self.rng = self.pack = self.mix = None
+        self.rng = self.pack = self.mix = self.prior = self.klfin = self.colsum = None
         self.done = False
         self.rode = ()
 
     def empty(self):
-        return self.rng is None and self.pack is None and self.mix is None
+        return all(getattr(self, k) is None for k in RIDER_KINDS_ALL)
+
+    def _kl_part(self):
+        ws, h, k = self.klfin[0], self.klfin[9], self.klfin[10]
+        l = lib.load()
+        return ws.data_ptr() + 4 * int(l.gv_kl_bwd_part_offset(h, k)), int(l.gv_kl_bwd_slices())
 
     def _launch_alone(self, kinds):
         if 'rng' in kinds and self.rng is not None:
@@ -388,20 +411,32 @@
         if 'mix' in kinds and self.mix is not None:
             z_pre, ws = self.mix
             lib.call('gv_kl_mix', ptr(z_pre), z_pre.shape[0] // 2, z_pre.shape[1], ptr(ws), lib.stream())
+        if 'prior' in kinds and self.prior is not None:
+            z_pre, eps, out = self.prior
+            lib.call('gv_prior_sample_fwd', ptr(z_pre), ptr(eps), ptr(out), eps.shape[0], z_pre.shape[0] // 2, z_pre.shape[1],
+                     lib.stream())
+        if 'klfin' in kinds and self.klfin is not None:
+            _, z_pre, gkl, gscale, gzp, acc, g_bias, acc_b, n, h, k = self.klfin
+            part, slices = self._kl_part()
+            lib.call('gv_kl_bwd_mix_final', part, slices, ptr(z_pre), ptr(gkl), float(gscale), ptr(gzp), 1 if acc else 0, ptr(g_bias),
+                     1 if acc_b else 0, n, h, k, lib.stream())
+        if 'colsum' in kinds and self.colsum is not None:
+            part, n, slices, out, acc = self.colsum
+            lib.call('gv_colsum_finish', ptr(part), n, slices, ptr(out), 1 if acc else 0, lib.stream())
 
     def flush(self):
         if self.done:
             raise RuntimeError('RiderBox: its jobs were already launched')
-        self._launch_alone(('rng', 'pack', 'mix'))
+        self._launch_alone(RIDER_KINDS_ALL)
         self.done = True
 
     def ride(self, gemm_args):
         if self.done:
             raise RuntimeError('RiderBox: its jobs were already launched')
-        ride = {k for k in ('rng', 'pack', 'mix') if getattr(self, k) is not None and k in GEMM_RIDER_KINDS}
+        ride = {k for k in RIDER_KINDS_ALL if getattr(self, k) is not None and k in GEMM_RIDER_KINDS}
         if 'rng' in ride and len(self.rng[1]) > 8:
             ride.discard('rng')
-        self._launch_alone({'rng', 'pack', 'mix'} - ride)
+        self._launch_alone(set(RIDER_KINDS_ALL) - ride)
         d = _Riders()
         if 'rng' in ride:
             rng, jobs = self.rng
@@ -415,7 +450,24 @@
         if 'mix' in ride:
             z_pre, ws = self.mix
             d.mix_z_pre, d.mix, d.mix_k, d.mix_h = z_pre.data_ptr(), ws.data_ptr(), z_pre.shape[0] // 2, z_pre.shape[1]
-        lib.call('gv_gemm_f32_riders', *gemm_args, _ct.addressof(d), lib.stream())
+        if gemm_args[1] or ride & {'prior', 'klfin', 'colsum'}:
+            f = _RidersFin()
+            if 'prior' in ride:
+                z_pre, eps, out = self.prior
+                f.prior_z_pre, f.prior_eps, f.prior_out = z_pre.data_ptr(), eps.data_ptr(), out.data_ptr()
+                f.prior_s, f.prior_k, f.prior_h = eps.shape[0], z_pre.shape[0] // 2, z_pre.shape[1]
+            if 'klfin' in ride:
+                _, z_pre, gkl, gscale, gzp, acc, g_bias, acc_b, n, h, k = self.klfin
+                f.kl_part, f.kl_slices = self._kl_part()
+                f.kl_z_pre, f.kl_gkl, f.kl_g_zpre, f.kl_g_bias = z_pre.data_ptr(), ptr(gkl), gzp.data_ptr(), ptr(g_bias)
+                f.kl_gscale, f.kl_n, f.kl_h, f.kl_k = float(gscale), n, h, k
+                f.kl_accumulate, f.kl_accumulate_bias = 1 if acc else 0, 1 if acc_b else 0
+            if 'colsum' in ride:
+                part, n, slices, out, acc = self.colsum
+                f.cs_part, f.cs_out, f.cs_n, f.cs_slices, f.cs_accumulate = part.data_ptr(), out.data_ptr(), n, slices, 1 if acc else 0
+            lib.call('gv_gemm_f32_riders_fin', *gemm_args, _ct.addressof(d), _ct.addressof(f), lib.stream())
+        else:
+            lib.call('gv_gemm_f32_riders', *gemm_args, _ct.addressof(d), lib.stream())
         self.rode = tuple(sorted(ride))
         self.done = True
 
@@ -456,10 +508,10 @@
     entry = 'gv_gemm_bf16' if (precision or GEMM_PRECISION) == 'bf16' else 'gv_gemm_f32'
     live = LIVE_ROWS
     if riders is not None:
-        plain = (entry == 'gv_gemm_f32' and b_k_chunks is None and c_tiles is None and not trans_a and not trans_b and split_k <= 1
+        plain = (entry == 'gv_gemm_f32' and b_k_chunks is None and c_tiles is None and not trans_a and split_k <= 1
                  and m > 0 and n > 0 and not (live is not None and a.shape[0] == live[1] and a.device == live[0].device))
         if GEMM_RIDERS and plain and not riders.empty():
-            riders.ride((0, 0, m, n, k, ptr(a), lda, ptr(b), ldb, ptr(out), out.stride(0) if m > 1 else n, ptr(bias), act,
+            riders.ride((0, 1 if trans_b else 0, m, n, k, ptr(a), lda, ptr(b), ldb, ptr(out), out.stride(0) if m > 1 else n, ptr(bias), act,
                          1 if accumulate else 0, 1, ptr(a_relu_mask), None, 0))
             return out
         riders.flush()
@@ -1543,7 +1595,7 @@
     return out
 
 
-def epilogue_bwd(out, grad_out, act, keep, keep_scale, colsum_out=None, colsum_accumulate=False):
+def epilogue_bwd(out, grad_out, act, keep, keep_scale, colsum_out=None, colsum_accumulate=False, riders=None):
     grad_out = _chk(grad_out.contiguous(), name='grad_out')
     g = torch.empty_like(grad_out)
     m, n = grad_out.shape
@@ -1551,7 +1603,9 @@
     part = torch.empty(EPILOGUE_COLSUM_SLICES * n, dtype=torch.float32, device=g.device) if fused else None
     lib.call('gv_rgcn_epilogue_bwd', ptr(out), ptr(grad_out), act, ptr(keep), float(keep_scale), ptr(g), m, n, ptr(part),
              lib.stream())
-    if fused:
+    if fused and riders is not None:
+        riders.colsum = (part, n, EPILOGUE_COLSUM_SLICES, colsum_out, bool(colsum_accumulate))
+    elif fused:
         lib.call('gv_colsum_finish', ptr(part), n, EPILOGUE_COLSUM_SLICES, ptr(colsum_out), 1 if colsum_accumulate else 0,
                  lib.stream())
     elif colsum_out is not None:
@@ -1803,11 +1857,11 @@
     return _Embedding.apply(table, ids, tick_rng)
 
 
-def _epilogue_grad(out, grad_out, act, keep, keep_scale, want_bias, d_b):
+def _epilogue_grad(out, grad_out, act, keep, keep_scale, want_bias, d_b, riders=None):
     if not want_bias:
         return epilogue_bwd(out, grad_out, act, keep, keep_scale), None
     grad_bias = d_b if d_b is not None else torch.empty(grad_out.shape[1], dtype=torch.float32, device=grad_out.device)
-    g = epilogue_bwd(out, grad_out, act, keep, keep_scale, colsum_out=grad_bias, colsum_accumulate=d_b is not None)
+    g = epilogue_bwd(out, grad_out, act, keep, keep_scale, colsum_out=grad_bias, colsum_accumulate=d_b is not None, riders=riders)
     return g, (None if d_b is not None else grad_bias)
 
 
@@ -1833,7 +1887,10 @@
     return addend
 
 
-def _loop_grads(x, g, loop_weight, d_l, want_loop, want_x, loop_bf=None):
+def _loop_grads(x, g, loop_weight, d_l, want_loop, want_x, loop_bf=None, riders=None):
+    if riders is not None and (loop_weight is None or not want_x or loop_bf is not None):
+        riders.flush()
+        riders = None
     if loop_weight is None:
         return None, None
     grad_loop = gx_loop = None
@@ -1846,7 +1903,7 @@
         if loop_bf is not None:
             gx_loop = dense_bf16(g, loop_bf[1], loop_weight.shape[0], loop_weight.shape[1])
         else:
-            gx_loop = gemm(g, loop_weight, trans_b=True)
+            gx_loop = gemm(g, loop_weight, trans_b=True, riders=riders)
     return grad_loop, gx_loop
 
 
@@ -1932,6 +1989,7 @@
                 reduce_hook, link_box=None, riders=None):
         x, _ = _row_major(x, 'x')
         n, in_feat = x.shape
+        ctx.bwd_riders = riders is not None and reduce_hook is None and not _dist_active()
         if riders is not None and (reduce_hook is not None or loop_weight is None):
             riders.flush()
             riders = None
@@ -1977,6 +2035,7 @@
         if link_box is not None and act == ACT_NONE and reduce_hook is None:
             ctx.epi_link = link_box[0] = EpilogueLink(keep, keep_scale, h_bias is not None and ctx.needs_input_grad[2],
                                                       ctx.direct[1], out_feat)
+            ctx.epi_link.carries_fin = ctx.bwd_riders
         return out
 
     @staticmethod
@@ -1986,10 +2045,16 @@
         _verify_direct(ctx)
         d_w, d_b, d_l = ctx.direct
         folded = ctx.epi_link.take(grad_out) if ctx.epi_link is not None else None
+        fin_box = ctx.epi_link.take_fin() if ctx.epi_link is not None else None
         if folded is not None:
             g, grad_bias = folded
         else:
-            g, grad_bias = _epilogue_grad(out, grad_out, act, keep, keep_scale, has_bias and ctx.needs_input_grad[2], d_b)
+            if fin_box is None and ctx.bwd_riders and rider_kind('colsum') and LIVE_ROWS is None and d_b is not None:
+                fin_box = RiderBox()
+            g, grad_bias = _epilogue_grad(out, grad_out, act, keep, keep_scale, has_bias and ctx.needs_input_grad[2], d_b, fin_box)
+        if fin_box is not None and fin_box.empty():
+            fin_box = None
+        ctx.fin_box = fin_box
         pending = None
         g_agg = g
         if reduce_hook is not None:
@@ -2006,7 +2071,9 @@
                 if gw_first:
                     _loop_grads(x, g, loop_weight, d_l, True, False)
         grad_loop, gx_loop = _loop_grads(x, g, loop_weight, d_l, ctx.needs_input_grad[3] and not side_w, ctx.needs_input_grad[0],
-                                         ctx.loop_bf)
+                                         ctx.loop_bf, fin_box)
+        if fin_box is not None and not fin_box.done:
+            raise RuntimeError('_RelGraphConvBdd.backward: the finishers\' RiderBox was dropped (a gradient was never finished)')
         if pending is not None:
             pending.wait()
         grad_x = None
@@ -2683,7 +2750,8 @@
 
 
 class EpilogueLink:
-    __slots__ = ('keep', 'keep_scale', 'want_bias', 'bias_target', 'n_bias', '_gv_direct_epoch', 'buf', 'buf_version', 'grad_bias')
+    __slots__ = ('keep', 'keep_scale', 'want_bias', 'bias_target', 'n_bias', '_gv_direct_epoch', 'buf', 'buf_version', 'grad_bias',
+                 'carries_fin', 'fin')
 
     def __init__(self, keep, keep_scale, want_bias, bias_target, n_bias):
         self.keep, self.keep_scale = keep, float(keep_scale)
@@ -2691,6 +2759,11 @@
         _stamp_direct(self)
         self.buf = self.grad_bias = None
         self.buf_version = 0
+        self.carries_fin, self.fin = False, None
+
+    def take_fin(self):
+        box, self.fin = self.fin, None
+        return box
 
     def record(self, buf, grad_bias):
         self.buf, self.buf_version, self.grad_bias = buf, buf._version, grad_bias
@@ -2774,10 +2847,19 @@
                     if d_b is not None:
                         _verify_direct(epi)
                     g_bias = d_b if d_b is not None else torch.empty(2 * h, dtype=torch.float32, device=h2.device)
-                lib.call('gv_reparam_kl_bwd_fold', ptr(z), ptr(h2), ptr(v), ptr(eps), ptr(z_pre), ptr(link.resp), ptr(link.gkl),
-                         float(link.gscale), float(link.z_extra), ptr(gz), ptr(gh2), ptr(gzp), 1 if d_zp is not None else 0,
-                         ptr(epi.keep), epi.keep_scale, ptr(g_bias), 1 if d_b is not None else 0, ptr(link.ws), n, h, k,
-                         lib.stream())
+                if (epi.carries_fin and epi.fin is None and rider_kind('klfin') and LIVE_ROWS is None and d_zp is not None
+                        and (g_bias is None or d_b is not None)):
+                    lib.call('gv_reparam_kl_bwd_fold_sweep', ptr(z), ptr(h2), ptr(v), ptr(eps), ptr(z_pre), ptr(link.resp),
+                             ptr(link.gkl), float(link.gscale), float(link.z_extra), ptr(gz), ptr(gh2), ptr(gzp), ptr(epi.keep),
+                             epi.keep_scale, ptr(g_bias), ptr(link.ws), n, h, k, lib.stream())
+                    epi.fin = RiderBox()
+                    epi.fin.klfin = (link.ws, z_pre, link.gkl, float(link.gscale), gzp, d_zp is not None, g_bias, d_b is not None,
+                                     n, h, k)
+                else:
+                    lib.call('gv_reparam_kl_bwd_fold', ptr(z), ptr(h2), ptr(v), ptr(eps), ptr(z_pre), ptr(link.resp), ptr(link.gkl),
+                             float(link.gscale), float(link.z_extra), ptr(gz), ptr(gh2), ptr(gzp), 1 if d_zp is not None else 0,
+                             ptr(epi.keep), epi.keep_scale, ptr(g_bias), 1 if d_b is not None else 0, ptr(link.ws), n, h, k,
+                             lib.stream())
                 link.gkl = None
                 epi.record(gh2, None if d_b is not None else g_bias)
                 return gh2, None, (None if d_zp is not None else gzp), None, None, None
@@ -3227,12 +3309,15 @@
 class _PriorSample(torch.autograd.Function):
 
     @staticmethod
-    def forward(ctx, z_pre, eps, link_box=None):
+    def forward(ctx, z_pre, eps, link_box=None, riders=None):
         z_pre, eps = _chk(z_pre.contiguous(), name='z_pre'), _chk(eps.contiguous(), name='eps')
         k, h = z_pre.shape[0] // 2, z_pre.shape[1]
         out = torch.empty_like(eps)
         ctx.set_materialize_grads(False)
-        lib.call('gv_prior_sample_fwd', ptr(z_pre), ptr(eps), ptr(out), eps.shape[0], k, h, lib.stream())
+        if riders is not None and riders.prior is None and not riders.done and rider_kind('prior'):
+            riders.prior = (z_pre, eps, out)
+        else:
+            lib.call('gv_prior_sample_fwd', ptr(z_pre), ptr(eps), ptr(out), eps.shape[0], k, h, lib.stream())
         ctx.save_for_backward(z_pre, eps)
         ctx.link = None
         if link_box is not None and eps.shape[0] % k == 0:
@@ -3246,22 +3331,22 @@
         if link is not None and link.claimed:
             folded = link.take(g)
             if folded is not None:
-                return folded[0], None, None
+                return folded[0], None, None, None
         if g is None:
-            return None, None, None
+            return None, None, None, None
         g = _chk(g.contiguous(), name='g')
         d_zp = _direct_flat(z_pre)
         gz = d_zp if d_zp is not None else torch.empty_like(z_pre)
         lib.call('gv_prior_sample_bwd', ptr(z_pre), ptr(eps), ptr(g), ptr(gz), 1 if d_zp is not None else 0, eps.shape[0],
                  z_pre.shape[0] // 2, z_pre.shape[1], lib.stream())
-        return (None if d_zp is not None else gz), None, None
-
-
-def prior_sample(z_pre, eps):
+        return (None if d_zp is not None else gz), None, None, None
+
+
+def prior_sample(z_pre, eps, riders=None):
     if not MMD_FUSED:
-        return _PriorSample.apply(z_pre, eps)
+        return _PriorSample.apply(z_pre, eps, None, riders)
     box = [None]
-    out = _PriorSample.apply(z_pre, eps, box)
+    out = _PriorSample.apply(z_pre, eps, box, riders)
     out._gv_prior_link = box[0]
     return out
 
diff --git a/include/gcnvae.h b/include/gcnvae.h
--- a/include/gcnvae.h
+++ b/include/gcnvae.h
@@ -457,6 +457,27 @@
 int gv_gemm_f32_riders(int trans_a, int trans_b, int m, int n, int k, const float* a, int lda, const float* b, int ldb, float* c,
                        int ldc, const float* bias, int act, int accumulate, int split_k, const float* a_relu_mask, void* workspace,
                        int64_t workspace_bytes, const gv_riders* riders, void* stream);
+typedef struct gv_riders_fin {
+    const float* prior_z_pre;
+    const float* prior_eps;
+    float* prior_out;
+    const float* kl_part;
+    const float* kl_z_pre;
+    const float* kl_gkl;
+    float* kl_g_zpre;
+    float* kl_g_bias;
+    const float* cs_part;
+    float* cs_out;
+    int64_t kl_n;
+    float kl_gscale;
+    int32_t prior_s, prior_k, prior_h;
+    int32_t kl_slices, kl_h, kl_k, kl_accumulate, kl_accumulate_bias;
+    int32_t cs_n, cs_slices, cs_accumulate;
+} gv_riders_fin;
+int gv_gemm_f32_riders_fin(int trans_a, int trans_b, int m, int n, int k, const float* a, int lda, const float* b, int ldb, float* c,
+                           int ldc, const float* bias, int act, int accumulate, int split_k, const float* a_relu_mask,
+                           void* workspace, int64_t workspace_bytes, const gv_riders* riders, const gv_riders_fin* fin,
+                           void* stream);
 int gv_gemm_f32_live_rows(int trans_a, int trans_b, int m, int n, int k, const float* a, int lda, const float* b, int ldb, float* c,
                           int ldc, const float* bias, int act, int accumulate, int split_k, const float* a_relu_mask, void* workspace,
                           int64_t workspace_bytes, const int32_t* rows_dev, void* stream);
@@ -532,6 +553,14 @@
                            const float* resp, const float* gkl, float gscale, float z_extra, const float* gz_up, float* gh2,
                            float* g_zpre, int accumulate_zpre, const uint8_t* keep, float keep_scale, float* g_bias,
                            int accumulate_bias, float* workspace, int64_t n, int h, int k, void* stream);
+int gv_reparam_kl_bwd_fold_sweep(const float* z, const float* h2, const float* v, const float* eps, const float* z_pre,
+                                 const float* resp, const float* gkl, float gscale, float z_extra, const float* gz_up, float* gh2,
+                                 float* g_zpre, const uint8_t* keep, float keep_scale, float* g_bias, float* workspace, int64_t n,
+                                 int h, int k, void* stream);
+int64_t gv_kl_bwd_part_offset(int h, int k);
+int gv_kl_bwd_slices(void);
+int gv_kl_bwd_mix_final(const float* part, int n_slices, const float* z_pre, const float* gkl, float gscale, float* g_zpre,
+                        int accumulate_zpre, float* g_bias, int accumulate_bias, int64_t n, int h, int k, void* stream);
 int gv_loss_combine_fold(const float* ws_pred, int64_t t, const float* w_rel, int64_t n_embed, int64_t n_wrel,
                          const float* ws_kl, int64_t n_nodes, int h, int k, const float* ws_mmd, int sx, int sy, float reg_w,
                          float kl_w, float mmd_w, float* scal , float* loss, void* stream);
```

Result: faster. 622.9 million edges/s, median of 6 (+1.9%).
